# Tacha-S/perception

Hardware: AMD Instinct MI355X
Metric: candidate poses rendered+scored/sec @640x480 (higher is better)
Workload: dtype f32; 1 GPU; C2: 1 YCB mesh (12,288 tris), 10k 6-DoF poses/GPU render+score, 640x480, stride 8, no ICP; poses_per_gpu=10000, width=640, height=480, stride=8, parallelism=pose-shard x1, batches_in_flight=2, ranks=1, devices=1, exchange=none (one process)

## Files before the change

### include/pcore.h

```cpp
#ifndef PCORE_H_
#define PCORE_H_

#include <stdint.h>

#ifdef __cplusplus
extern "C" {
#endif

#define PCORE_ABI_VERSION 7

enum pcore_status {
    PCORE_OK = 0,
    PCORE_E_INVALID_ARG = 1,
    PCORE_E_HIP = 2,
    PCORE_E_OOM = 3,
    PCORE_E_STATE = 4
};

enum pcore_cost_type { PCORE_COST_DEPTH_3DOF = 0, PCORE_COST_RGBD_3DOF = 1, PCORE_COST_DEPTH_6DOF = 2 };

typedef struct pcore_ctx pcore_ctx;
typedef void* pcore_stream;

typedef struct pcore_camera {
    int32_t width, height;
    float fx, fy, cx, cy;
    float proj[16];
} pcore_camera;

typedef struct pcore_eval_params {
    int32_t cost_type;
    int32_t calc_obs_cost;
    int32_t stride;
    float depth_factor;
    float sensor_resolution;
    float occlusion_threshold;
    float color_distance_threshold;
} pcore_eval_params;

int pcore_create(int device, pcore_ctx** out_ctx);
void pcore_destroy(pcore_ctx* ctx);
const char* pcore_last_error(const pcore_ctx* ctx);
int pcore_abi_version(void);

uint64_t pcore_generation(const pcore_ctx* ctx);

int pcore_upload_meshes(pcore_ctx* ctx, const float* tri_xyz, const uint8_t* tri_rgb, int32_t num_tris,
                        const int32_t* tris_model_count, int32_t num_models);

int pcore_set_camera(pcore_ctx* ctx, const pcore_camera* cam);

int pcore_observed_cloud(pcore_ctx* ctx, const int32_t* d_depth, const uint8_t* d_label_mask, int32_t width,
                         int32_t height, int32_t stride, float depth_factor, float* d_out_xyz,
                         int32_t* d_out_label, int32_t cap, int32_t* out_count, pcore_stream stream);

int pcore_observed_cloud_bounded(pcore_ctx* ctx, const int32_t* d_depth, const uint8_t* d_rgb, int32_t width,
                                 int32_t height, int32_t stride, float depth_factor, const float* cam_to_world,
                                 const double* bounds, float* d_out_xyz, uint8_t* d_out_rgb, int32_t cap,
                                 int32_t* out_count, pcore_stream stream);

int pcore_set_observation(pcore_ctx* ctx, const int32_t* d_src_depth_cm, const uint8_t* d_src_mask,
                          const float* d_obs_xyz, const int32_t* d_obs_label, int32_t num_obs,
                          float sensor_resolution, pcore_stream stream);

int pcore_set_observation_colors(pcore_ctx* ctx, const uint8_t* d_obs_rgb, int32_t num_obs, pcore_stream stream);

int pcore_evaluate(pcore_ctx* ctx, const float* d_poses, const int32_t* d_pose_model,
                   const int32_t* d_pose_label, const float* d_pose_obs_total, int32_t num_poses,
                   const pcore_eval_params* params, float* d_out_rc, float* d_out_oc, float* d_out_diff,
                   int32_t* d_dbg_zs, pcore_stream stream);

#define PCORE_GICP_CYCLE_WINDOW 8
typedef struct pcore_icp_params {
    int32_t k_correspondences;
    int32_t max_iterations;
    double rotation_epsilon;
    double transformation_epsilon;
    int32_t cycle_exit_window;
} pcore_icp_params;

int pcore_evaluate_select(pcore_ctx* ctx, const float* d_poses, const int32_t* d_pose_model,
                          const int32_t* d_pose_label, const float* d_pose_obs_total, int32_t num_poses,
                          const pcore_eval_params* params, float* d_out_rc, float* d_out_oc, float* d_out_diff,
                          int64_t index_base, int32_t num_models, int64_t* d_keys, pcore_stream stream);

int pcore_evaluate_icp(pcore_ctx* ctx, const float* d_poses, const int32_t* d_pose_model,
                       const int32_t* d_pose_label, const float* d_pose_obs_total, int32_t num_poses,
                       const pcore_eval_params* params, const pcore_icp_params* icp, float* d_out_poses,
                       int32_t* d_out_iters, float* d_out_rc, float* d_out_oc, float* d_out_diff,
                       pcore_stream stream);

typedef struct pcore_planar_icp_params {
    int32_t max_iterations;
    float   max_correspondence;
    double  transformation_epsilon;
    double  fitness_epsilon;
} pcore_planar_icp_params;

int pcore_icp_planar(pcore_ctx* ctx, const float* d_poses, const int32_t* d_pose_model, int32_t num_poses,
                     const pcore_eval_params* params, const float* world_from_cam,
                     const pcore_planar_icp_params* icp, double* d_out_xform, int32_t* d_out_iters,
                     int32_t* d_out_status, double* d_out_mse, pcore_stream stream);

int pcore_debug_planar_step(const double* d_sums, double* d_out, int32_t n, pcore_stream stream);

typedef struct pcore_p2p_icp_params {
    int32_t max_iterations;
    float   relative_fitness;
    float   relative_rmse;
    float   max_dist_diff;
} pcore_p2p_icp_params;

int pcore_scene_projective(pcore_ctx* ctx, const int32_t* d_depth_cm, int32_t width, int32_t height, float fx, float fy,
                           float cx, float cy, float* d_out_pcd, float* d_out_normal, pcore_stream stream);

int pcore_icp_point2plane(pcore_ctx* ctx, const float* d_poses, const int32_t* d_pose_model,
                          const int32_t* d_pose_label, int32_t num_poses, const pcore_eval_params* params,
                          const pcore_p2p_icp_params* icp, float* d_out_T, float* d_out_fitness, float* d_out_rmse,
                          int32_t* d_out_iters, float* d_out_poses, pcore_stream stream);

int pcore_debug_p2p_clouds(const float* d_xyzw, const int32_t* d_seg_cnt, int32_t seg_stride, int32_t num_segs,
                           const float* d_scene_pcd4, const float* d_scene_normal4, int32_t width, int32_t height,
                           float fx, float fy, float cx, float cy, const pcore_p2p_icp_params* icp, float* d_out_T,
                           float* d_out_fitness, float* d_out_rmse, int32_t* d_out_iters, pcore_stream stream);

int pcore_render(pcore_ctx* ctx, const float* d_poses, const int32_t* d_pose_model, const int32_t* d_pose_label,
                 int32_t num_poses, float occlusion_threshold, int32_t* d_out_depth, uint8_t* d_out_color,
                 pcore_stream stream);

typedef struct pcore_gpu_stats {
    float icp_runtime;
    double peak_memory_usage;
    float gicp_ms;
    int32_t icp_chunks;
    int64_t gicp_iterations;
    int64_t gicp_iterations_run;
    int64_t gicp_cycle_exits;
} pcore_gpu_stats;
int pcore_get_stats(pcore_ctx* ctx, pcore_gpu_stats* out, int32_t reset);

#define PCORE_MAX_TILE_TIERS 8
typedef struct pcore_tile_info {
    int32_t num_tiers;
    int32_t tier;
    int32_t tcap;
    int32_t seq;
    int32_t edge[PCORE_MAX_TILE_TIERS];
    int32_t wgs_per_cu[PCORE_MAX_TILE_TIERS];
    int32_t hist[PCORE_MAX_TILE_TIERS + 1];
    int32_t chunked;
} pcore_tile_info;
int pcore_get_tile_info(pcore_ctx* ctx, pcore_tile_info* out);

int pcore_debug_lm_solve(const double* d_sys, const double* d_lambda, double* d_out, int32_t n, pcore_stream stream);

int pcore_debug_covariances(const float* d_xyzw, const int32_t* d_seg_off, const int32_t* d_seg_cnt, int32_t num_segs,
                            int32_t k, double* d_out_cov6, pcore_stream stream);
int pcore_debug_covariances_cloud(const float* d_xyzw, const int32_t* d_seg_cnt, int32_t seg_stride, int32_t num_segs,
                                  float fx, float fy, float cx, float cy, int32_t stride, double* d_out_cov6,
                                  pcore_stream stream);
int pcore_debug_gicp_help_stats(pcore_ctx* c, int64_t* out4);

int pcore_count_within(pcore_ctx* ctx, const float* d_queries, const int32_t* d_labels, const float* d_radius_sq,
                       int32_t n, int32_t* d_out_counts, pcore_stream stream);
int pcore_state_poses(pcore_ctx* ctx, const double* d_states, const int32_t* d_model, const double* cam_from_world,
                      const double* d_preprocess, int32_t num_models, int32_t n, float* d_out_poses,
                      pcore_stream stream);

int pcore_depth_to_cloud(pcore_ctx* ctx, const int32_t* d_depth, int32_t num_poses, int32_t width, int32_t height,
                         int32_t stride, float depth_factor, const uint8_t* d_label_mask,
                         const int32_t* d_pose_label, float* d_out_xyz, int32_t* d_out_pose, int32_t* d_out_label,
                         int32_t cap, int32_t* out_count, pcore_stream stream);

int pcore_depth_to_cloud_ex(pcore_ctx* ctx, const int32_t* d_depth, int32_t num_poses, int32_t width, int32_t height,
                            int32_t stride, float depth_factor, const uint8_t* d_label_mask, const int32_t* d_pose_label,
                            const uint8_t* d_color_planes, float* d_out_xyz, int32_t* d_out_pose, int32_t* d_out_label,
                            uint8_t* d_out_color, int32_t* d_out_dc_index, int32_t cap, int32_t* out_count,
                            pcore_stream stream);

#define PCORE_KEY_NONE ((int64_t)0x7fffffffffffffffLL)
int pcore_select(pcore_ctx* ctx, const float* d_rc, const float* d_oc, const int32_t* d_pose_model,
                 int32_t num_poses, int64_t index_base, int32_t num_models, int64_t* d_keys, pcore_stream stream);

int pcore_pose_distances(pcore_ctx* ctx, const float* d_pts, int32_t n, const double* d_T_gt, const double* d_T_est,
                         int32_t num_pairs, double* d_add, double* d_adds, pcore_stream stream);

#ifdef __cplusplus
}
#endif
#endif
```

### perception_amd/_native.py

```python
from __future__ import annotations

import ctypes
import os

import numpy as np

from . import build as _build

PCORE_OK = 0
PCORE_E_INVALID_ARG = 1
PCORE_E_HIP = 2
PCORE_E_OOM = 3
PCORE_E_STATE = 4
PCORE_KEY_NONE = 0x7FFFFFFFFFFFFFFF

COST_DEPTH_3DOF = 0
COST_RGBD_3DOF = 1
COST_DEPTH_6DOF = 2

EXPORTED_SYMBOLS = (
    "pcore_create", "pcore_destroy", "pcore_last_error", "pcore_abi_version", "pcore_upload_meshes",
    "pcore_set_camera", "pcore_observed_cloud", "pcore_set_observation", "pcore_evaluate", "pcore_evaluate_icp",
    "pcore_render",
    "pcore_depth_to_cloud", "pcore_select", "pcore_pose_distances",
    "pcore_observed_cloud_bounded", "pcore_set_observation_colors", "pcore_generation", "pcore_get_stats",
    "pcore_count_within", "pcore_state_poses", "pcore_evaluate_select", "pcore_get_tile_info", "pcore_debug_lm_solve",
    "pcore_debug_covariances", "pcore_debug_covariances_cloud", "pcore_debug_gicp_help_stats", "pcore_depth_to_cloud_ex",
    "pcore_icp_planar", "pcore_debug_planar_step",
    "pcore_scene_projective",
)
EXPORTED_SYMBOLS_WITH_DIGITS = ("pcore_icp_point2plane", "pcore_debug_p2p_clouds")


class PcoreError(RuntimeError):
    def __init__(self, code: int, msg: str):
        super().__init__(f"pcore error {code}: {msg}")
        self.code = code


class Camera(ctypes.Structure):
    _fields_ = [("width", ctypes.c_int32), ("height", ctypes.c_int32), ("fx", ctypes.c_float),
                ("fy", ctypes.c_float), ("cx", ctypes.c_float), ("cy", ctypes.c_float),
                ("proj", ctypes.c_float * 16)]


class EvalParams(ctypes.Structure):
    _fields_ = [("cost_type", ctypes.c_int32), ("calc_obs_cost", ctypes.c_int32), ("stride", ctypes.c_int32),
                ("depth_factor", ctypes.c_float), ("sensor_resolution", ctypes.c_float),
                ("occlusion_threshold", ctypes.c_float), ("color_distance_threshold", ctypes.c_float)]


class GpuStats(ctypes.Structure):
    _fields_ = [("icp_runtime", ctypes.c_float), ("peak_memory_usage", ctypes.c_double), ("gicp_ms", ctypes.c_float),
                ("icp_chunks", ctypes.c_int32), ("gicp_iterations", ctypes.c_int64),
                ("gicp_iterations_run", ctypes.c_int64), ("gicp_cycle_exits", ctypes.c_int64)]


MAX_TILE_TIERS = 8


class TileInfo(ctypes.Structure):
    _fields_ = [("num_tiers", ctypes.c_int32), ("tier", ctypes.c_int32), ("tcap", ctypes.c_int32),
                ("seq", ctypes.c_int32), ("edge", ctypes.c_int32 * MAX_TILE_TIERS),
                ("wgs_per_cu", ctypes.c_int32 * MAX_TILE_TIERS), ("hist", ctypes.c_int32 * (MAX_TILE_TIERS + 1)),
                ("chunked", ctypes.c_int32)]


class IcpParams(ctypes.Structure):
    _fields_ = [("k_correspondences", ctypes.c_int32), ("max_iterations", ctypes.c_int32),
                ("rotation_epsilon", ctypes.c_double), ("transformation_epsilon", ctypes.c_double),
                ("cycle_exit_window", ctypes.c_int32)]


class PlanarIcpParams(ctypes.Structure):
    _fields_ = [("max_iterations", ctypes.c_int32), ("max_correspondence", ctypes.c_float),
                ("transformation_epsilon", ctypes.c_double), ("fitness_epsilon", ctypes.c_double)]


class P2pIcpParams(ctypes.Structure):
    _fields_ = [("max_iterations", ctypes.c_int32), ("relative_fitness", ctypes.c_float),
                ("relative_rmse", ctypes.c_float), ("max_dist_diff", ctypes.c_float)]


P2P_MAX_ITER = 30
P2P_REL_FITNESS = 1e-5
P2P_REL_RMSE = 1e-5
P2P_MAX_DIST_DIFF = 0.1

PLANAR_MAX_ITER = 20
PLANAR_MAX_CORRESPONDENCE = 0.05
PLANAR_TRANS_EPS = 1e-8
PLANAR_FIT_EPS = 1e-5
PLANAR_ITERATION_CAP, PLANAR_TRANSFORM, PLANAR_ABS_MSE, PLANAR_REL_MSE, PLANAR_NO_CORRESPONDENCES, PLANAR_EMPTY_RENDER = \
    range(6)

ICP_K = 10
ICP_MAX_ITER = 150
ICP_ROT_EPS = float(np.float32(2e-3))
ICP_TRANS_EPS = float(np.float32(5e-4))
ICP_CYCLE_WINDOW = 8

_lib = None


def library_path() -> str:
    return _build.LIB


def load(auto_build: bool = True) -> ctypes.CDLL:
    global _lib
    if _lib is not None:
        return _lib
    override = os.environ.get("PCORE_LIB")
    if override:
        auto_build = False
    if auto_build:
        try:
            if _build.needs_build():
                _build.build()
        except (RuntimeError, OSError) as e:
            if not os.path.exists(_build.LIB):
                raise RuntimeError(f"libpcore.so is missing and cannot be built: {e}") from e
    path = override or _build.LIB
    if not os.path.exists(path):
        raise RuntimeError(f"libpcore.so not found at {path}; run `python -m perception_amd.build`")
    L = ctypes.CDLL(path)
    vp, i32, i64, f32 = ctypes.c_void_p, ctypes.c_int32, ctypes.c_int64, ctypes.c_float
    L.pcore_create.argtypes = [ctypes.c_int, ctypes.POINTER(vp)]
    L.pcore_destroy.argtypes = [vp]
    L.pcore_destroy.restype = None
    L.pcore_last_error.argtypes = [vp]
    L.pcore_last_error.restype = ctypes.c_char_p
    L.pcore_abi_version.argtypes = []
    L.pcore_upload_meshes.argtypes = [vp, vp, vp, i32, vp, i32]
    L.pcore_set_camera.argtypes = [vp, ctypes.POINTER(Camera)]
    L.pcore_observed_cloud.argtypes = [vp, vp, vp, i32, i32, i32, f32, vp, vp, i32, ctypes.POINTER(i32), vp]
    L.pcore_set_observation.argtypes = [vp, vp, vp, vp, vp, i32, f32, vp]
    L.pcore_evaluate.argtypes = [vp, vp, vp, vp, vp, i32, ctypes.POINTER(EvalParams), vp, vp, vp, vp, vp]
    L.pcore_evaluate_icp.argtypes = [vp, vp, vp, vp, vp, i32, ctypes.POINTER(EvalParams), ctypes.POINTER(IcpParams),
                                     vp, vp, vp, vp, vp, vp]
    L.pcore_render.argtypes = [vp, vp, vp, vp, i32, f32, vp, vp, vp]
    L.pcore_get_stats.argtypes = [vp, ctypes.POINTER(GpuStats), i32]
    if hasattr(L, "pcore_get_tile_info"):
        L.pcore_get_tile_info.argtypes = [vp, ctypes.POINTER(TileInfo)]
    if hasattr(L, "pcore_debug_lm_solve"):
        L.pcore_debug_lm_solve.argtypes = [vp, vp, vp, i32, vp]
    if hasattr(L, "pcore_debug_covariances"):
        L.pcore_debug_covariances.argtypes = [vp, vp, vp, i32, i32, vp, vp]
    if hasattr(L, "pcore_debug_gicp_help_stats"):
        L.pcore_debug_gicp_help_stats.argtypes = [vp, vp]
    if hasattr(L, "pcore_debug_covariances_cloud"):
        f32 = ctypes.c_float
        L.pcore_debug_covariances_cloud.argtypes = [vp, vp, i32, i32, f32, f32, f32, f32, i32, vp, vp]
    if hasattr(L, "pcore_depth_to_cloud_ex"):
        L.pcore_depth_to_cloud_ex.argtypes = [vp, vp, i32, i32, i32, i32, f32, vp, vp, vp, vp, vp, vp, vp, vp, i32,
                                              ctypes.POINTER(i32), vp]
    L.pcore_depth_to_cloud.argtypes = [vp, vp, i32, i32, i32, i32, f32, vp, vp, vp, vp, vp, i32,
                                       ctypes.POINTER(i32), vp]
    if hasattr(L, "pcore_icp_planar"):
        L.pcore_icp_planar.argtypes = [vp, vp, vp, i32, ctypes.POINTER(EvalParams), ctypes.POINTER(ctypes.c_float),
                                       ctypes.POINTER(PlanarIcpParams), vp, vp, vp, vp, vp]
    if hasattr(L, "pcore_debug_planar_step"):
        L.pcore_debug_planar_step.argtypes = [vp, vp, i32, vp]
    if hasattr(L, "pcore_icp_point2plane"):
        L.pcore_scene_projective.argtypes = [vp, vp, i32, i32, f32, f32, f32, f32, vp, vp, vp]
        L.pcore_icp_point2plane.argtypes = [vp, vp, vp, vp, i32, ctypes.POINTER(EvalParams),
                                            ctypes.POINTER(P2pIcpParams), vp, vp, vp, vp, vp, vp]
        L.pcore_debug_p2p_clouds.argtypes = [vp, vp, i32, i32, vp, vp, i32, i32, f32, f32, f32, f32,
                                             ctypes.POINTER(P2pIcpParams), vp, vp, vp, vp, vp]
    L.pcore_select.argtypes = [vp, vp, vp, vp, i32, i64, i32, vp, vp]
    L.pcore_pose_distances.argtypes = [vp, vp, i32, vp, vp, i32, vp, vp, vp]
    L.pcore_set_observation_colors.argtypes = [vp, vp, i32, vp]
    L.pcore_observed_cloud_bounded.argtypes = [vp, vp, vp, i32, i32, i32, f32, vp, vp, vp, vp, i32,
                                               ctypes.POINTER(i32), vp]
    L.pcore_generation.argtypes = [vp]
    L.pcore_evaluate_select.argtypes = [vp, vp, vp, vp, vp, i32, ctypes.POINTER(EvalParams), vp, vp, vp, i64, i32,
                                        vp, vp]
    L.pcore_count_within.argtypes = [vp, vp, vp, vp, i32, vp, vp]
    L.pcore_state_poses.argtypes = [vp, vp, vp, ctypes.POINTER(ctypes.c_double), vp, i32, i32, vp, vp]
    for name in EXPORTED_SYMBOLS + EXPORTED_SYMBOLS_WITH_DIGITS:
        if name not in ("pcore_destroy", "pcore_last_error", "pcore_generation") and hasattr(L, name):
            getattr(L, name).restype = ctypes.c_int
    L.pcore_generation.restype = ctypes.c_uint64
    _lib = L
    return L
```

### perception_amd/build.py

```python
from __future__ import annotations

import os
import shutil
import subprocess
import sys

HERE = os.path.dirname(os.path.abspath(__file__))
CSRC = os.path.join(HERE, "csrc")
LIB = os.path.join(HERE, "libpcore.so")
SOURCES = ["pcore_kernels.hip", "pcore_gicp.hip", "pcore_metrics.hip", "pcore_states.hip", "pcore_icp2d.hip", "pcore_p2p.hip",
           "pcore_api.hip"]
HEADERS = ["pcore_internal.h", "pcore_cov.h", "pcore_gicp_math.h", "pcore_icp2d_math.h", "pcore_p2p_math.h", "pcore_dmath.h", "pcore_colour.h", "pcore_fdiv.h", "pcore_streams.h", os.path.join("..", "..", "include", "pcore.h")]
ARCH = os.environ.get("PCORE_OFFLOAD_ARCH", "gfx950")


def hipcc() -> str:
    for cand in (os.environ.get("HIPCC"), shutil.which("hipcc"), "/opt/rocm/bin/hipcc"):
        if cand and os.path.exists(cand):
            return cand
    raise RuntimeError("hipcc not found: cannot build libpcore.so")


def flags() -> list:
    return [f"--offload-arch={ARCH}", "-O2", "-std=c++17", "-fPIC", "-shared", "-ffp-contract=off",
            "-fno-fast-math", "-fno-slp-vectorize", "-Wall", "-Wno-unused-function"]


def kernel_source_digest() -> str:
    import hashlib

    h = hashlib.sha256(" ".join(flags()).encode())
    for f in ("pcore_kernels.hip", "pcore_internal.h", "pcore_cov.h", "pcore_colour.h", "pcore_fdiv.h", "pcore_streams.h"):
        with open(os.path.join(CSRC, f), "rb") as fh:
            h.update(fh.read())
    return h.hexdigest()[:16]


def gicp_source_digest() -> str:
    import hashlib

    h = hashlib.sha256(" ".join(flags()).encode())
    for f in ("pcore_gicp.hip", "pcore_cov.h", "pcore_gicp_math.h", "pcore_icp2d_math.h", "pcore_dmath.h", "pcore_internal.h"):
        with open(os.path.join(CSRC, f), "rb") as fh:
            h.update(fh.read())
    return h.hexdigest()[:16]


def needs_build() -> bool:
    if not os.path.exists(LIB):
        return True
    t = os.path.getmtime(LIB)
    deps = [os.path.join(CSRC, f) for f in SOURCES + HEADERS] + [os.path.abspath(__file__)]
    return any(os.path.getmtime(d) > t for d in deps if os.path.exists(d))


def build(force: bool = False, verbose: bool = False) -> str:
    if not force and not needs_build():
        return LIB
    cmd = [hipcc()] + flags() + [os.path.join(CSRC, f) for f in SOURCES] + ["-o", LIB + ".tmp"]
    if verbose:
        print(" ".join(cmd), file=sys.stderr)
    subprocess.run(cmd, check=True, cwd=CSRC)
    os.replace(LIB + ".tmp", LIB)
    return LIB


def build_checkers(verbose: bool = False) -> list:
    root = os.path.dirname(HERE)
    out_dir = os.path.join(root, "tools", "bin")
    os.makedirs(out_dir, exist_ok=True)
    built = []
    for name in ("fdiv_check",):
        src = os.path.join(root, "tools", name + ".hip")
        out = os.path.join(out_dir, name)
        cmd = [hipcc(), f"--offload-arch={ARCH}", "-O3", "-std=c++17", "-ffp-contract=off", "-fno-fast-math", src,
               "-o", out]
        if verbose:
            print(" ".join(cmd), file=sys.stderr)
        subprocess.run(cmd, check=True, cwd=root)
        built.append(out)
    return built


if __name__ == "__main__":
    print(build(force="--force" in sys.argv, verbose=True))
```

### perception_amd/core.py

```python
from __future__ import annotations

import ctypes
from typing import Optional, Sequence, Tuple

import numpy as np
import torch

from . import _native
from ._native import Camera, EvalParams, IcpParams, P2pIcpParams, PcoreError, PlanarIcpParams


def _ptr(t: Optional[torch.Tensor], dtype: torch.dtype, name: str):
    if t is None:
        return None
    if not isinstance(t, torch.Tensor) or not t.is_cuda:
        raise TypeError(f"{name}: expected a GPU torch tensor")
    if t.dtype != dtype:
        raise TypeError(f"{name}: expected {dtype}, got {t.dtype}")
    if not t.is_contiguous():
        raise ValueError(f"{name}: tensor must be contiguous")
    return ctypes.c_void_p(t.data_ptr())


def _stream(stream: Optional[torch.cuda.Stream]):
    s = stream if stream is not None else torch.cuda.current_stream()
    return ctypes.c_void_p(s.cuda_stream)


class PoseCore:

    def __init__(self, device: int = 0):
        self.lib = _native.load()
        self.device = int(device)
        h = ctypes.c_void_p()
        rc = self.lib.pcore_create(self.device, ctypes.byref(h))
        if rc != _native.PCORE_OK:
            raise PcoreError(rc, f"pcore_create(device={device}) failed")
        self._h = h
        self.width = self.height = 0
        self.num_models = 0

    def close(self):
        if getattr(self, "_h", None) is not None and self._h.value:
            self.lib.pcore_destroy(self._h)
            self._h = None

    def __del__(self):
        try:
            self.close()
        except Exception:
            pass

    def _check(self, rc: int):
        if rc != _native.PCORE_OK:
            msg = self.lib.pcore_last_error(self._h)
            raise PcoreError(rc, msg.decode() if msg else "")

    def upload_meshes(self, tris: np.ndarray, tris_model_count, colors: Optional[np.ndarray] = None):
        tris = np.ascontiguousarray(tris, dtype=np.float32).reshape(-1, 9)
        cnt = np.ascontiguousarray(tris_model_count, dtype=np.int32)
        col = None if colors is None else np.ascontiguousarray(colors, dtype=np.uint8).reshape(-1, 3)
        self._check(self.lib.pcore_upload_meshes(
            self._h, tris.ctypes.data_as(ctypes.c_void_p),
            None if col is None else col.ctypes.data_as(ctypes.c_void_p), tris.shape[0],
            cnt.ctypes.data_as(ctypes.c_void_p), cnt.shape[0]))
        self.num_models = int(cnt.shape[0])

    def set_camera(self, width: int, height: int, fx: float, fy: float, cx: float, cy: float, proj: np.ndarray):
        cam = Camera()
        cam.width, cam.height = int(width), int(height)
        cam.fx, cam.fy, cam.cx, cam.cy = float(fx), float(fy), float(cx), float(cy)
        pj = np.asarray(proj, dtype=np.float32).reshape(16)
        for i in range(16):
            cam.proj[i] = float(pj[i])
        self._check(self.lib.pcore_set_camera(self._h, ctypes.byref(cam)))
        self.width, self.height = int(width), int(height)

    def observed_cloud(self, depth: torch.Tensor, label_mask: Optional[torch.Tensor], stride: int,
                       depth_factor: float, stream=None) -> Tuple[torch.Tensor, torch.Tensor]:
        h, w = depth.shape[-2:]
        cap = ((w + stride - 1) // stride) * ((h + stride - 1) // stride)
        xyz = torch.empty((max(cap, 1), 3), dtype=torch.float32, device=depth.device)
        lab = torch.empty((max(cap, 1),), dtype=torch.int32, device=depth.device)
        cnt = ctypes.c_int32(0)
        self._check(self.lib.pcore_observed_cloud(
            self._h, _ptr(depth, torch.int32, "depth"), _ptr(label_mask, torch.uint8, "label_mask"), w, h, stride,
            float(depth_factor), _ptr(xyz, torch.float32, "xyz"), _ptr(lab, torch.int32, "label"), cap,
            ctypes.byref(cnt), _stream(stream)))
        n = cnt.value
        return xyz[:n], lab[:n]

    def observed_cloud_bounded(self, depth: torch.Tensor, stride: int, depth_factor: float,
                               cam_to_world: Optional[np.ndarray] = None, bounds: Optional[Sequence[float]] = None,
                               rgb: Optional[torch.Tensor] = None, stream=None
                               ) -> Tuple[torch.Tensor, Optional[torch.Tensor]]:
        h, w = depth.shape[-2:]
        cap = ((w + stride - 1) // stride) * ((h + stride - 1) // stride)
        xyz = torch.empty((max(cap, 1), 3), dtype=torch.float32, device=depth.device)
        out_rgb = torch.empty((max(cap, 1), 3), dtype=torch.uint8, device=depth.device) if rgb is not None else None
        M = None if cam_to_world is None else (ctypes.c_float * 16)(*np.asarray(cam_to_world, np.float32).reshape(16))
        B = None if bounds is None else (ctypes.c_double * 6)(*np.asarray(bounds, np.float64).reshape(6))
        cnt = ctypes.c_int32(0)
        self._check(self.lib.pcore_observed_cloud_bounded(
            self._h, _ptr(depth, torch.int32, "depth"), _ptr(None if rgb is None else rgb.contiguous(), torch.uint8, "rgb"),
            w, h, stride, float(depth_factor), M, B, _ptr(xyz, torch.float32, "xyz"),
            _ptr(out_rgb, torch.uint8, "out_rgb"), cap, ctypes.byref(cnt), _stream(stream)))
        n = cnt.value
        return xyz[:n], (out_rgb[:n] if out_rgb is not None else None)

    def set_observation(self, src_depth_cm: torch.Tensor, src_mask: Optional[torch.Tensor],
                        obs_xyz: torch.Tensor, obs_label: Optional[torch.Tensor], sensor_resolution: float,
                        stream=None):
        obs_xyz = obs_xyz.contiguous()
        n = int(obs_xyz.shape[0])
        self._check(self.lib.pcore_set_observation(
            self._h, _ptr(src_depth_cm.contiguous(), torch.int32, "src_depth"),
            _ptr(None if src_mask is None else src_mask.contiguous(), torch.uint8, "src_mask"),
            _ptr(obs_xyz, torch.float32, "obs_xyz") if n else None,
            _ptr(None if obs_label is None else obs_label.contiguous(), torch.int32, "obs_label") if n else None,
            n, float(sensor_resolution), _stream(stream)))

    def set_observation_colors(self, obs_rgb: torch.Tensor, stream=None):
        rgb = obs_rgb.contiguous()
        n = int(rgb.shape[0])
        self._check(self.lib.pcore_set_observation_colors(
            self._h, _ptr(rgb, torch.uint8, "obs_rgb") if n else None, n, _stream(stream)))

    def evaluate(self, poses: torch.Tensor, pose_model: torch.Tensor, pose_label: Optional[torch.Tensor],
                 pose_obs_total: Optional[torch.Tensor], cost_type: int = _native.COST_DEPTH_6DOF,
                 calc_obs_cost: bool = True, stride: int = 8, depth_factor: float = 100.0,
                 sensor_resolution: float = 0.01, occlusion_threshold: float = 1.0,
                 out: Optional[Tuple[torch.Tensor, torch.Tensor, torch.Tensor]] = None,
                 dbg_zs: Optional[torch.Tensor] = None, color_distance_threshold: float = 15.0, stream=None,
                 select: Optional[Tuple[torch.Tensor, int, int]] = None):
        n = int(poses.shape[0])
        dev = poses.device
        if out is None:
            out = tuple(torch.empty(n, dtype=torch.float32, device=dev) for _ in range(3))
        rc, oc, df = out
        p = EvalParams(int(cost_type), int(bool(calc_obs_cost)), int(stride), float(depth_factor),
                       float(sensor_resolution), float(occlusion_threshold), float(color_distance_threshold))
        if select is not None:
            keys, index_base, num_models = select
            if dbg_zs is not None:
                raise ValueError("evaluate: dbg_zs and select are exclusive")
            self._check(self.lib.pcore_evaluate_select(
                self._h, _ptr(poses, torch.float32, "poses"), _ptr(pose_model, torch.int32, "pose_model"),
                _ptr(pose_label, torch.int32, "pose_label"), _ptr(pose_obs_total, torch.float32, "pose_obs_total"),
                n, ctypes.byref(p), _ptr(rc, torch.float32, "rc"), _ptr(oc, torch.float32, "oc"),
                _ptr(df, torch.float32, "diff"), int(index_base), int(num_models), _ptr(keys, torch.int64, "keys"),
                _stream(stream)))
            return rc, oc, df
        self._check(self.lib.pcore_evaluate(
            self._h, _ptr(poses, torch.float32, "poses"), _ptr(pose_model, torch.int32, "pose_model"),
            _ptr(pose_label, torch.int32, "pose_label"), _ptr(pose_obs_total, torch.float32, "pose_obs_total"),
            n, ctypes.byref(p), _ptr(rc, torch.float32, "rc"), _ptr(oc, torch.float32, "oc"),
            _ptr(df, torch.float32, "diff"), _ptr(dbg_zs, torch.int32, "dbg_zs"), _stream(stream)))
        return rc, oc, df

    def capture_evaluate(self, poses: torch.Tensor, pose_model: torch.Tensor, pose_label: Optional[torch.Tensor],
                         pose_obs_total: Optional[torch.Tensor], **kw):
        n = int(poses.shape[0])
        out = tuple(torch.empty(n, dtype=torch.float32, device=poses.device) for _ in range(3))
        self.evaluate(poses, pose_model, pose_label, pose_obs_total, out=out, **kw)
        torch.cuda.synchronize()
        graph = torch.cuda.CUDAGraph()
        with torch.cuda.graph(graph):
            self.evaluate(poses, pose_model, pose_label, pose_obs_total, out=out, **kw)
        gen = self.generation()

        def replay():
            if self.generation() != gen:
                raise PcoreError(_native.PCORE_E_STATE, "captured evaluate graph is stale: the context changed "
                                 "(setup call, new stride or scratch reallocation) since the capture")
            graph.replay()

        return replay, out

    def generation(self) -> int:
        return int(self.lib.pcore_generation(self._h))

    def evaluate_icp(self, poses: torch.Tensor, pose_model: torch.Tensor, pose_label: Optional[torch.Tensor],
                     pose_obs_total: Optional[torch.Tensor], cost_type: int = _native.COST_DEPTH_6DOF,
                     calc_obs_cost: bool = True, stride: int = 8, depth_factor: float = 100.0,
                     sensor_resolution: float = 0.01, occlusion_threshold: float = 1.0,
                     k: int = _native.ICP_K, max_iterations: int = _native.ICP_MAX_ITER,
                     rotation_epsilon: float = _native.ICP_ROT_EPS,
                     transformation_epsilon: float = _native.ICP_TRANS_EPS, out=None,
                     color_distance_threshold: float = 15.0, stream=None,
                     cycle_exit_window: int = _native.ICP_CYCLE_WINDOW):
        n = int(poses.shape[0])
        dev = poses.device
        if out is None:
            out = (torch.empty((n, 16), dtype=torch.float32, device=dev), torch.empty(n, dtype=torch.int32, device=dev),
                   *(torch.empty(n, dtype=torch.float32, device=dev) for _ in range(3)))
        adj, iters, rc, oc, df = out
        p = EvalParams(int(cost_type), int(bool(calc_obs_cost)), int(stride), float(depth_factor),
                       float(sensor_resolution), float(occlusion_threshold), float(color_distance_threshold))
        ip = IcpParams(int(k), int(max_iterations), float(rotation_epsilon), float(transformation_epsilon),
                       int(cycle_exit_window))
        self._check(self.lib.pcore_evaluate_icp(
            self._h, _ptr(poses, torch.float32, "poses"), _ptr(pose_model, torch.int32, "pose_model"),
            _ptr(pose_label, torch.int32, "pose_label"), _ptr(pose_obs_total, torch.float32, "pose_obs_total"),
            n, ctypes.byref(p), ctypes.byref(ip), _ptr(adj, torch.float32, "adjusted_poses"),
            _ptr(iters, torch.int32, "iterations"), _ptr(rc, torch.float32, "rc"), _ptr(oc, torch.float32, "oc"),
            _ptr(df, torch.float32, "diff"), _stream(stream)))
        return adj, iters, rc, oc, df

    def icp_planar(self, poses: torch.Tensor, pose_model: torch.Tensor, world_from_cam: np.ndarray,
                   cost_type: int = _native.COST_DEPTH_3DOF, stride: int = 4, depth_factor: float = 100.0,
                   occlusion_threshold: float = 1.0, max_iterations: int = _native.PLANAR_MAX_ITER,
                   max_correspondence: float = _native.PLANAR_MAX_CORRESPONDENCE,
                   transformation_epsilon: float = _native.PLANAR_TRANS_EPS,
                   fitness_epsilon: float = _native.PLANAR_FIT_EPS, out=None, stream=None):
        n = int(poses.shape[0])
        dev = poses.device
        if out is None:
            out = (torch.empty((n, 4), dtype=torch.float64, device=dev), torch.empty(n, dtype=torch.int32, device=dev),
                   torch.empty(n, dtype=torch.int32, device=dev), torch.empty(n, dtype=torch.float64, device=dev))
        xform, iters, status, mse = out
        p = EvalParams(int(cost_type), 0, int(stride), float(depth_factor), 0.0, float(occlusion_threshold), 0.0)
        pp = PlanarIcpParams(int(max_iterations), float(max_correspondence), float(transformation_epsilon),
                             float(fitness_epsilon))
        M = (ctypes.c_float * 16)(*np.asarray(world_from_cam, np.float32).reshape(16))
        self._check(self.lib.pcore_icp_planar(
            self._h, _ptr(poses, torch.float32, "poses"), _ptr(pose_model, torch.int32, "pose_model"), n,
            ctypes.byref(p), M, ctypes.byref(pp), _ptr(xform, torch.float64, "xform"),
            _ptr(iters, torch.int32, "iterations"), _ptr(status, torch.int32, "status"),
            _ptr(mse, torch.float64, "mse"), _stream(stream)))
        return xform, iters, status, mse

    def planar_step(self, sums: torch.Tensor, stream=None) -> torch.Tensor:
        sums = sums.contiguous()
        n = int(sums.shape[0])
        out = torch.empty((n, 4), dtype=torch.float64, device=sums.device)
        rc = self.lib.pcore_debug_planar_step(_ptr(sums, torch.float64, "sums"), _ptr(out, torch.float64, "out"), n,
                                              _stream(stream))
        if rc != _native.PCORE_OK:
            raise PcoreError(rc, "pcore_debug_planar_step failed")
        return out

    def scene_projective(self, depth_cm: torch.Tensor, fx: float, fy: float, cx: float, cy: float, stream=None
                         ) -> Tuple[torch.Tensor, torch.Tensor]:
        h, w = depth_cm.shape[-2:]
        pcd = torch.empty((h, w, 3), dtype=torch.float32, device=depth_cm.device)
        nrm = torch.empty((h, w, 3), dtype=torch.float32, device=depth_cm.device)
        self._check(self.lib.pcore_scene_projective(
            self._h, _ptr(depth_cm, torch.int32, "depth_cm"), int(w), int(h), float(fx), float(fy), float(cx),
            float(cy), _ptr(pcd, torch.float32, "pcd"), _ptr(nrm, torch.float32, "normal"), _stream(stream)))
        return pcd, nrm

    def icp_point2plane(self, poses: torch.Tensor, pose_model: torch.Tensor, pose_label: Optional[torch.Tensor] = None,
                        cost_type: int = _native.COST_DEPTH_6DOF, stride: int = 8, depth_factor: float = 100.0,
                        occlusion_threshold: float = 1.0, max_iterations: int = _native.P2P_MAX_ITER,
                        relative_fitness: float = _native.P2P_REL_FITNESS,
                        relative_rmse: float = _native.P2P_REL_RMSE, max_dist_diff: float = _native.P2P_MAX_DIST_DIFF,
                        out=None, out_poses: Optional[torch.Tensor] = None, stream=None):
        n = int(poses.shape[0])
        dev = poses.device
        if out is None:
            out = (torch.empty((n, 16), dtype=torch.float32, device=dev), torch.empty(n, dtype=torch.float32, device=dev),
                   torch.empty(n, dtype=torch.float32, device=dev), torch.empty(n, dtype=torch.int32, device=dev))
        T, fitness, rmse, iters = out
        p = EvalParams(int(cost_type), 0, int(stride), float(depth_factor), 0.0, float(occlusion_threshold), 0.0)
        ip = P2pIcpParams(int(max_iterations), float(relative_fitness), float(relative_rmse), float(max_dist_diff))
        self._check(self.lib.pcore_icp_point2plane(
            self._h, _ptr(poses, torch.float32, "poses"), _ptr(pose_model, torch.int32, "pose_model"),
            _ptr(pose_label, torch.int32, "pose_label"), n, ctypes.byref(p), ctypes.byref(ip),
            _ptr(T, torch.float32, "T"), _ptr(fitness, torch.float32, "fitness"), _ptr(rmse, torch.float32, "rmse"),
            _ptr(iters, torch.int32, "iterations"), _ptr(out_poses, torch.float32, "out_poses"), _stream(stream)))
        return T, fitness, rmse, iters

    def p2p_clouds(self, xyzw: torch.Tensor, seg_cnt: torch.Tensor, scene_pcd4: torch.Tensor,
                   scene_normal4: torch.Tensor, fx: float, fy: float, cx: float, cy: float,
                   max_iterations: int = _native.P2P_MAX_ITER, relative_fitness: float = _native.P2P_REL_FITNESS,
                   relative_rmse: float = _native.P2P_REL_RMSE, max_dist_diff: float = _native.P2P_MAX_DIST_DIFF,
                   stream=None):
        s, cap = int(xyzw.shape[0]), int(xyzw.shape[1])
        h, w = int(scene_pcd4.shape[0]), int(scene_pcd4.shape[1])
        dev = xyzw.device
        T = torch.empty((s, 16), dtype=torch.float32, device=dev)
        fitness = torch.empty(s, dtype=torch.float32, device=dev)
        rmse = torch.empty(s, dtype=torch.float32, device=dev)
        iters = torch.empty(s, dtype=torch.int32, device=dev)
        ip = P2pIcpParams(int(max_iterations), float(relative_fitness), float(relative_rmse), float(max_dist_diff))
        rc = self.lib.pcore_debug_p2p_clouds(
            _ptr(xyzw, torch.float32, "xyzw"), _ptr(seg_cnt, torch.int32, "seg_cnt"), cap, s,
            _ptr(scene_pcd4, torch.float32, "scene_pcd4"), _ptr(scene_normal4, torch.float32, "scene_normal4"), w, h,
            float(fx), float(fy), float(cx), float(cy), ctypes.byref(ip), _ptr(T, torch.float32, "T"),
            _ptr(fitness, torch.float32, "fitness"), _ptr(rmse, torch.float32, "rmse"),
            _ptr(iters, torch.int32, "iterations"), _stream(stream))
        if rc != _native.PCORE_OK:
            raise PcoreError(rc, "pcore_debug_p2p_clouds failed")
        return T, fitness, rmse, iters

    def evaluate_p2p(self, poses: torch.Tensor, pose_model: torch.Tensor, pose_label: Optional[torch.Tensor],
                     pose_obs_total: Optional[torch.Tensor], cost_type: int = _native.COST_DEPTH_6DOF,
                     calc_obs_cost: bool = True, stride: int = 8, depth_factor: float = 100.0,
                     sensor_resolution: float = 0.01, occlusion_threshold: float = 1.0,
                     max_iterations: int = _native.P2P_MAX_ITER, relative_fitness: float = _native.P2P_REL_FITNESS,
                     relative_rmse: float = _native.P2P_REL_RMSE, max_dist_diff: float = _native.P2P_MAX_DIST_DIFF,
                     color_distance_threshold: float = 15.0, stream=None):
        n = int(poses.shape[0])
        adj = torch.empty((n, 16), dtype=torch.float32, device=poses.device)
        label = pose_label if cost_type == _native.COST_DEPTH_6DOF else None
        _, fitness, rmse, iters = self.icp_point2plane(
            poses, pose_model, label, cost_type=cost_type, stride=stride, depth_factor=depth_factor,
            occlusion_threshold=occlusion_threshold, max_iterations=max_iterations,
            relative_fitness=relative_fitness, relative_rmse=relative_rmse, max_dist_diff=max_dist_diff,
            out_poses=adj, stream=stream)
        rc, oc, df = self.evaluate(adj, pose_model, pose_label, pose_obs_total, cost_type=cost_type,
                                   calc_obs_cost=calc_obs_cost, stride=stride, depth_factor=depth_factor,
                                   sensor_resolution=sensor_resolution, occlusion_threshold=occlusion_threshold,
                                   color_distance_threshold=color_distance_threshold, stream=stream)
        return adj, iters, rc, oc, df, fitness, rmse

    def render(self, poses: torch.Tensor, pose_model: torch.Tensor, pose_label: Optional[torch.Tensor],
               occlusion_threshold: float = 1.0, out: Optional[torch.Tensor] = None, color: bool = False,
               out_color: Optional[torch.Tensor] = None, stream=None):
        n = int(poses.shape[0])
        if out is None:
            out = torch.empty((n, self.height, self.width), dtype=torch.int32, device=poses.device)
        if color and out_color is None:
            out_color = torch.empty((3, n, self.height, self.width), dtype=torch.uint8, device=poses.device)
        self._check(self.lib.pcore_render(
            self._h, _ptr(poses, torch.float32, "poses"), _ptr(pose_model, torch.int32, "pose_model"),
            _ptr(pose_label, torch.int32, "pose_label"), n, float(occlusion_threshold),
            _ptr(out, torch.int32, "out"), _ptr(out_color, torch.uint8, "out_color") if color else None,
            _stream(stream)))
        return (out, out_color) if color else out

    def stats(self, reset: bool = False) -> dict:
        st = _native.GpuStats()
        self._check(self.lib.pcore_get_stats(self._h, ctypes.byref(st), int(bool(reset))))
        return {"icp_runtime": st.icp_runtime, "peak_memory_usage": st.peak_memory_usage, "gicp_ms": st.gicp_ms,
                "icp_chunks": st.icp_chunks, "gicp_iterations": st.gicp_iterations,
                "gicp_iterations_run": st.gicp_iterations_run, "gicp_cycle_exits": st.gicp_cycle_exits}

    def gicp_help_stats(self) -> dict:
        out = (ctypes.c_int64 * 4)()
        self._check(self.lib.pcore_debug_gicp_help_stats(self._h, out))
        return {"helper_rounds": int(out[0]), "owner_timeouts": int(out[1]), "helper_giveups": int(out[2]),
                "poses_enlisted": int(out[3])}

    def tile_info(self) -> dict:
        ti = _native.TileInfo()
        self._check(self.lib.pcore_get_tile_info(self._h, ctypes.byref(ti)))
        n = ti.num_tiers
        return {"tier": ti.tier, "tcap": ti.tcap, "seq": ti.seq, "edge": list(ti.edge[:n]),
                "wgs_per_cu": list(ti.wgs_per_cu[:n]), "hist": list(ti.hist[:n + 1]), "chunked": ti.chunked}

    def depth_to_cloud(self, depth: torch.Tensor, stride: int, depth_factor: float,
                       label_mask: Optional[torch.Tensor] = None, pose_label: Optional[torch.Tensor] = None,
                       stream=None, color_planes: Optional[torch.Tensor] = None, dc_index: bool = False):
        if depth.dim() == 2:
            depth = depth.unsqueeze(0)
        n, h, w = depth.shape
        cap = n * ((w + stride - 1) // stride) * ((h + stride - 1) // stride)
        dev = depth.device
        xyz = torch.empty((max(cap, 1), 3), dtype=torch.float32, device=dev)
        pose = torch.empty((max(cap, 1),), dtype=torch.int32, device=dev)
        lab = torch.empty((max(cap, 1),), dtype=torch.int32, device=dev)
        cnt = ctypes.c_int32(0)
        extra = color_planes is not None or dc_index
        if not extra:
            self._check(self.lib.pcore_depth_to_cloud(
                self._h, _ptr(depth.contiguous(), torch.int32, "depth"), n, w, h, stride, float(depth_factor),
                _ptr(label_mask, torch.uint8, "label_mask"), _ptr(pose_label, torch.int32, "pose_label"),
                _ptr(xyz, torch.float32, "xyz"), _ptr(pose, torch.int32, "pose"), _ptr(lab, torch.int32, "label"),
                cap, ctypes.byref(cnt), _stream(stream)))
            k = cnt.value
            return xyz[:k], pose[:k], lab[:k]
        planes = None
        col = None
        if color_planes is not None:
            planes = color_planes.contiguous()
            if tuple(planes.shape) != (3, n, h, w):
                raise ValueError(f"color_planes must be (3, {n}, {h}, {w}), got {tuple(planes.shape)}")
            col = torch.empty((3, max(cap, 1)), dtype=torch.uint8, device=dev)
        dc = torch.empty((n, h, w), dtype=torch.int32, device=dev) if dc_index else None
        self._check(self.lib.pcore_depth_to_cloud_ex(
            self._h, _ptr(depth.contiguous(), torch.int32, "depth"), n, w, h, stride, float(depth_factor),
            _ptr(label_mask, torch.uint8, "label_mask"), _ptr(pose_label, torch.int32, "pose_label"),
            _ptr(planes, torch.uint8, "color_planes"), _ptr(xyz, torch.float32, "xyz"), _ptr(pose, torch.int32, "pose"),
            _ptr(lab, torch.int32, "label"), _ptr(col, torch.uint8, "color"), _ptr(dc, torch.int32, "dc_index"),
            max(cap, 1) if col is not None else cap, ctypes.byref(cnt), _stream(stream)))
        k = cnt.value
        out = [xyz[:k], pose[:k], lab[:k]]
        if col is not None:
            out.append(col[:, :k])
        if dc is not None:
            out.append(dc)
        return tuple(out)

    def select(self, rc: torch.Tensor, oc: torch.Tensor, pose_model: torch.Tensor, num_models: int,
               index_base: int = 0, keys: Optional[torch.Tensor] = None, stream=None) -> torch.Tensor:
        if keys is None:
            keys = torch.full((num_models,), _native.PCORE_KEY_NONE, dtype=torch.int64, device=rc.device)
        self._check(self.lib.pcore_select(
            self._h, _ptr(rc, torch.float32, "rc"), _ptr(oc, torch.float32, "oc"),
            _ptr(pose_model, torch.int32, "pose_model"), int(rc.shape[0]), int(index_base), int(num_models),
            _ptr(keys, torch.int64, "keys"), _stream(stream)))
        return keys

    def count_within(self, queries: torch.Tensor, labels: torch.Tensor, radius_sq: torch.Tensor,
                     out: Optional[torch.Tensor] = None, stream=None) -> torch.Tensor:
        n = int(queries.shape[0])
        if out is None:
            out = torch.empty(n, dtype=torch.int32, device=queries.device)
        self._check(self.lib.pcore_count_within(
            self._h, _ptr(queries.contiguous(), torch.float32, "queries"), _ptr(labels.contiguous(), torch.int32, "labels"),
            _ptr(radius_sq.contiguous(), torch.float32, "radius_sq"), n, _ptr(out, torch.int32, "counts"),
            _stream(stream)))
        return out

    def state_poses(self, states: torch.Tensor, model: torch.Tensor, cam_from_world, preprocess: torch.Tensor,
                    out: Optional[torch.Tensor] = None, stream=None) -> torch.Tensor:
        n = int(states.shape[0])
        if out is None:
            out = torch.empty((n, 16), dtype=torch.float32, device=states.device)
        cam = (ctypes.c_double * 16)(*[float(v) for v in np.asarray(cam_from_world, np.float64).reshape(16)])
        k = int(preprocess.shape[0])
        self._check(self.lib.pcore_state_poses(
            self._h, _ptr(states.contiguous(), torch.float64, "states"), _ptr(model.contiguous(), torch.int32, "model"),
            cam, _ptr(preprocess.contiguous(), torch.float64, "preprocess"), k, n, _ptr(out, torch.float32, "poses"),
            _stream(stream)))
        return out


class PoseLanes:

    def __init__(self, device: int = 0, lanes: int = 2):
        if lanes < 1:
            raise ValueError("lanes must be >= 1")
        self.cores = [PoseCore(device) for _ in range(lanes)]
        dev = torch.device("cuda", int(device))
        self.streams = [torch.cuda.Stream(device=dev) for _ in range(lanes)]

    def __len__(self):
        return len(self.cores)

    def __getitem__(self, i: int) -> Tuple[PoseCore, torch.cuda.Stream]:
        return self.cores[i], self.streams[i]

    def upload_meshes(self, *a, **kw):
        for c in self.cores:
            c.upload_meshes(*a, **kw)

    def set_camera(self, *a, **kw):
        for c in self.cores:
            c.set_camera(*a, **kw)

    def set_observation(self, *a, **kw):
        for c in self.cores:
            c.set_observation(*a, **kw)

    def set_observation_colors(self, *a, **kw):
        for c in self.cores:
            c.set_observation_colors(*a, **kw)

    @classmethod
    def replicate(cls, core: "PoseCore", scene_setup, lanes: int = 2) -> "PoseLanes":
        if lanes < 1:
            raise ValueError("lanes must be >= 1")
        self = cls.__new__(cls)
        self.cores = [core] + [PoseCore(core.device) for _ in range(lanes - 1)]
        dev = torch.device("cuda", core.device)
        self.streams = [torch.cuda.Stream(device=dev) for _ in range(lanes)]
        for c in self.cores[1:]:
            scene_setup(c)
        return self


def decode_keys(keys) -> Tuple[np.ndarray, np.ndarray]:
    k = np.asarray(keys.cpu() if isinstance(keys, torch.Tensor) else keys, dtype=np.int64)
    none = k == _native.PCORE_KEY_NONE
    hi = (k >> 31).astype(np.uint64).astype(np.uint32)
    cost = (hi ^ np.uint32(0x80000000)).view(np.int32).astype(np.int32)
    idx = (k & 0x7FFFFFFF).astype(np.int64)
    cost = np.where(none, np.int32(2**31 - 1), cost)
    idx = np.where(none, -1, idx)
    return cost, idx


def encode_key(cost: int, index: int) -> int:
    if cost == 2**31 - 1 and index < 0:
        return _native.PCORE_KEY_NONE
    hi = (int(cost) & 0xFFFFFFFF) ^ 0x80000000
    return (hi << 31) | (int(index) & 0x7FFFFFFF)
```

### perception_amd/csrc/pcore_api.hip

```cpp
#include "../../include/pcore.h"
#include "pcore_internal.h"
#include "pcore_streams.h"
#include "pcore_gicp_math.h"
#include "pcore_icp2d_math.h"
#include "pcore_p2p_math.h"

#include <algorithm>
#include <climits>
#include <cmath>
#include <cstdio>
#include <cstdlib>
#include <cstring>
#include <string>
#include <unordered_map>
#include <vector>

using namespace pcore;

namespace {

template <typename T>
struct DevBuf {
    T* p = nullptr;
    size_t n = 0;
// ... 1051 lines not shown
            HIPC(c, hipMemcpyAsync(c->icp_iter_stats_host, c->icp_iter_stats.p, 8 * sizeof(unsigned long long),
                                   hipMemcpyDeviceToHost, s));
        if (ev) {
            HIPC(c, hipEventRecord(ev[2], s));
            c->icp_ev_used++;
        }
    }
    return pcore_evaluate(c, d_out_poses, d_pose_model, d_pose_label, d_pose_obs_total, num_poses, p, d_out_rc,
                          d_out_oc, d_out_diff, nullptr, stream);
}

int pcore_icp_planar(pcore_ctx* c, const float* d_poses, const int32_t* d_pose_model, int32_t num_poses,
                     const pcore_eval_params* p, const float* world_from_cam, const pcore_planar_icp_params* pp,
                     double* d_out_xform, int32_t* d_out_iters, int32_t* d_out_status, double* d_out_mse,
                     pcore_stream stream) {
    if (!c) return PCORE_E_INVALID_ARG;
    if (!p || !pp || !world_from_cam) return fail(c, PCORE_E_INVALID_ARG, "icp_planar: null parameters");
    if (!c->have_mesh || !c->have_cam || !c->have_obs)
        return fail(c, PCORE_E_STATE, "icp_planar: meshes, camera and observation must be set first");
    if (p->cost_type != PCORE_COST_DEPTH_3DOF && p->cost_type != PCORE_COST_RGBD_3DOF)
        return fail(c, PCORE_E_INVALID_ARG, "icp_planar: cost_type must be a 3-DoF one (0 or 1)");
    if (pp->max_iterations < 0) return fail(c, PCORE_E_INVALID_ARG, "icp_planar: max_iterations must be >= 0");
    if (!std::isfinite(pp->max_correspondence) || pp->max_correspondence < 0.0f)
        return fail(c, PCORE_E_INVALID_ARG, "icp_planar: max_correspondence must be finite and >= 0");
    if (std::isnan(pp->transformation_epsilon) || std::isnan(pp->fitness_epsilon))
        return fail(c, PCORE_E_INVALID_ARG, "icp_planar: NaN epsilon");
    for (int i = 0; i < 16; i++)
        if (!std::isfinite(world_from_cam[i])) return fail(c, PCORE_E_INVALID_ARG, "icp_planar: non-finite world_from_cam");
    if (num_poses < 0 || (num_poses > 0 && (!d_poses || !d_pose_model || !d_out_xform || !d_out_iters || !d_out_status)))
        return fail(c, PCORE_E_INVALID_ARG, "icp_planar: null pose / output pointer");
    const int W = c->cam.width, H = c->cam.height;
    if (p->stride <= 0 || W % p->stride != 0)
        return fail(c, PCORE_E_INVALID_ARG, "icp_planar: width must be a multiple of stride");
    const int ws = W / p->stride, hs = (H + p->stride - 1) / p->stride;
    if (ws > 4095 || hs > 4095) return fail(c, PCORE_E_INVALID_ARG, "icp_planar: sampled image too large");
    if (fused_lds_bytes(ws * hs, c->bitmap_words, false) > (size_t)c->prop.sharedMemPerBlock)
        return fail(c, PCORE_E_INVALID_ARG, "icp_planar: sampled z-buffer does not fit in LDS (use a larger stride)");
    if (num_poses == 0) return PCORE_OK;
    HIPC(c, hipSetDevice(c->device));
    hipStream_t s = (hipStream_t)stream;
    const int nsamp = ws * hs;
    const size_t per_pose = (size_t)nsamp * sizeof(float4) + sizeof(int32_t);
    size_t budget = (size_t)32 << 30;
    {
        size_t free_b = 0, total_b = 0;
        if (hipMemGetInfo(&free_b, &total_b) == hipSuccess && free_b > 0)
            budget = std::min(budget, std::max<size_t>((size_t)1 << 30, free_b / 5 * 2));
    }
    if (const char* e = getenv("PCORE_ICP2D_SCRATCH_BYTES")) budget = (size_t)std::max(1LL, atoll(e));
    const int max_chunk = (int)std::min<size_t>(std::max<size_t>(1, budget / per_pose), 0x7fffffff);
    const int nchunks = (num_poses + max_chunk - 1) / max_chunk;
    const int chunk = (num_poses + nchunks - 1) / nchunks;
    const bool grid_stale = c->planar_obs_serial != c->obs_serial ||
                            std::memcmp(c->planar_m, world_from_cam, sizeof(c->planar_m)) != 0 ||
                            std::memcmp(&c->planar_radius, &pp->max_correspondence, sizeof(float)) != 0;
    const bool setup = grid_stale || c->sampled_stride != p->stride || !c->icp_cloud.p || !c->icp_count.p ||
                       c->icp_cloud.n < (size_t)chunk * nsamp || c->icp_count.n < (size_t)chunk;
    hipStreamCaptureStatus cap_status = hipStreamCaptureStatusNone;
    if (hipStreamIsCapturing(s, &cap_status) != hipSuccess) {
        (void)hipGetLastError();
        cap_status = hipStreamCaptureStatusActive;
    }
    if (setup && cap_status != hipStreamCaptureStatusNone)
        return fail(c, PCORE_E_STATE, "icp_planar: the world-frame grid or the scratch would have to be built while the "
                                      "stream captures; run the call once before the capture");
    if (grid_stale) {
        const int n = (int)(c->obs_xyz_h.size() / 3);
        std::vector<float4> wp((size_t)n);
        for (int i = 0; i < n; i++) {
            float4 q;
            icp2d::to_world(world_from_cam, c->obs_xyz_h[3 * (size_t)i], c->obs_xyz_h[3 * (size_t)i + 1],
                            c->obs_xyz_h[3 * (size_t)i + 2], q.x, q.y, q.z);
            std::memcpy(&q.w, &i, 4);
            wp[i] = q;
        }
        std::vector<int32_t> cell_start;
        std::vector<float4> gpts;
        LabelGrid g;
        build_grid(wp, pp->max_correspondence, g, cell_start, gpts);
        if (gpts.empty()) gpts.push_back(make_float4(0.0f, 0.0f, 0.0f, 0.0f));
        HIPC(c, hipStreamSynchronize(s));
        c->planar_obs_serial = 0;
        c->generation++;
        HIPC(c, dev_upload(c->planar_cell_start, cell_start));
        HIPC(c, dev_upload(c->planar_pts, gpts));
        c->planar_grid = g;
        std::memcpy(c->planar_m, world_from_cam, sizeof(c->planar_m));
        c->planar_radius = pp->max_correspondence;
        c->planar_obs_serial = c->obs_serial;
    }
    int rc = ensure_sampled(c, p->stride, s);
    if (rc != PCORE_OK) return rc;
    HIPC(c, reserve_gen(c, c->icp_cloud, (size_t)chunk * nsamp));
    HIPC(c, reserve_gen(c, c->icp_count, (size_t)chunk));
    FusedArgs a{};
    fill_fused_args(c, p, a);
    PlanarArgs g{};
    g.src = c->icp_cloud.p;
    g.src_count = c->icp_count.p;
    g.src_cap = nsamp;
    for (int i = 0; i < 12; i++) g.m[i] = world_from_cam[i];
    g.grid = c->planar_grid;
    g.cell_start = c->planar_cell_start.p;
    g.grid_pts = c->planar_pts.p;
    g.r = pp->max_correspondence;
    g.r2 = pp->max_correspondence * pp->max_correspondence;
    g.max_iter = pp->max_iterations;
    g.eps_t = pp->transformation_epsilon;
    g.eps_fit = pp->fitness_epsilon;
    g.out_xform = d_out_xform;
    g.out_iters = d_out_iters;
    g.out_status = d_out_status;
    g.out_mse = d_out_mse;
    for (int base = 0; base < num_poses; base += chunk) {
        const int n = std::min(chunk, num_poses - base);
        a.poses = d_poses + (size_t)16 * base;
        a.pose_model = d_pose_model + base;
        a.pose_label = nullptr;
        a.num_poses = n;
        a.cloud_out = c->icp_cloud.p;
        a.cloud_count = c->icp_count.p;
        a.cloud_cap = nsamp;
        a.tcap = fused_tier_samples(0, a.ws, a.hs, 0, false, c->dinfo);
        if (const char* e = getenv("PCORE_FUSED_TCAP")) a.tcap = std::min(std::max(atoi(e), 1), a.ws * a.hs);
        if (a.tcap <= 0) a.tcap = a.ws * a.hs;
        HIPC(c, launch_render_cloud(a, s));
        g.pose_base = base;
        HIPC(c, launch_planar_icp(g, n, s));
    }
    return PCORE_OK;
}

int pcore_debug_planar_step(const double* d_sums, double* d_out, int32_t n, pcore_stream stream) {
    if (n < 0 || (n > 0 && (!d_sums || !d_out))) return PCORE_E_INVALID_ARG;
    return launch_planar_step_test(d_sums, d_out, n, (hipStream_t)stream) == hipSuccess ? PCORE_OK : PCORE_E_HIP;
}

int pcore_scene_projective(pcore_ctx* c, const int32_t* d_depth_cm, int32_t width, int32_t height, float fx, float fy,
                           float cx, float cy, float* d_out_pcd, float* d_out_normal, pcore_stream stream) {
    if (!c) return PCORE_E_INVALID_ARG;
    if (width <= 0 || height <= 0 || width > 16384 || height > 16384)
        return fail(c, PCORE_E_INVALID_ARG, "scene_projective: bad image size");
    if (!d_depth_cm || !d_out_pcd || !d_out_normal)
        return fail(c, PCORE_E_INVALID_ARG, "scene_projective: null pointer");
    HIPC(c, hipSetDevice(c->device));
    HIPC(c, launch_p2p_scene(d_depth_cm, width, height, fx, fy, cx, cy, nullptr, nullptr, d_out_pcd, d_out_normal,
                             (hipStream_t)stream));
    return PCORE_OK;
}

namespace {

const char* p2p_params_error(const pcore_p2p_icp_params* ip) {
    if (ip->max_iterations < 0) return "max_iterations must be >= 0";
    if (std::isnan(ip->relative_fitness) || ip->relative_fitness < 0.0f) return "relative_fitness must be >= 0";
    if (std::isnan(ip->relative_rmse) || ip->relative_rmse < 0.0f) return "relative_rmse must be >= 0";
    if (std::isnan(ip->max_dist_diff) || ip->max_dist_diff < 0.0f) return "max_dist_diff must be >= 0";
    return nullptr;
}

}

int pcore_icp_point2plane(pcore_ctx* c, const float* d_poses, const int32_t* d_pose_model, const int32_t* d_pose_label,
                          int32_t num_poses, const pcore_eval_params* p, const pcore_p2p_icp_params* ip,
                          float* d_out_T, float* d_out_fitness, float* d_out_rmse, int32_t* d_out_iters,
                          float* d_out_poses, pcore_stream stream) {
    if (!c) return PCORE_E_INVALID_ARG;
    if (!p || !ip) return fail(c, PCORE_E_INVALID_ARG, "icp_point2plane: null parameters");
    if (!c->have_mesh || !c->have_cam || !c->have_obs)
        return fail(c, PCORE_E_STATE, "icp_point2plane: meshes, camera and observation must be set first");
    if (p->cost_type != PCORE_COST_DEPTH_3DOF && p->cost_type != PCORE_COST_DEPTH_6DOF &&
        p->cost_type != PCORE_COST_RGBD_3DOF)
        return fail(c, PCORE_E_INVALID_ARG, "icp_point2plane: unknown cost_type");
    if (const char* e = p2p_params_error(ip)) return fail(c, PCORE_E_INVALID_ARG, std::string("icp_point2plane: ") + e);
    if (num_poses < 0 || (num_poses > 0 && (!d_poses || !d_pose_model || !d_out_T || !d_out_fitness || !d_out_rmse ||
                                            !d_out_iters)))
        return fail(c, PCORE_E_INVALID_ARG, "icp_point2plane: null pose / output pointer");
    if (d_pose_label && !c->obs_has_mask)
        return fail(c, PCORE_E_INVALID_ARG, "icp_point2plane: pose labels need a source mask");
    const int W = c->cam.width, H = c->cam.height;
    if (p->stride <= 0 || W % p->stride != 0)
        return fail(c, PCORE_E_INVALID_ARG, "icp_point2plane: width must be a multiple of stride");
    const int ws = W / p->stride, hs = (H + p->stride - 1) / p->stride;
    if (ws > 4095 || hs > 4095) return fail(c, PCORE_E_INVALID_ARG, "icp_point2plane: sampled image too large");
    if (fused_lds_bytes(ws * hs, c->bitmap_words, false) > (size_t)c->prop.sharedMemPerBlock)
        return fail(c, PCORE_E_INVALID_ARG,
                    "icp_point2plane: sampled z-buffer does not fit in LDS (use a larger stride)");
    if (num_poses == 0) return PCORE_OK;
    HIPC(c, hipSetDevice(c->device));
    hipStream_t s = (hipStream_t)stream;
    const int nsamp = ws * hs;
    const size_t per_pose = (size_t)nsamp * sizeof(float4) + sizeof(int32_t);
    size_t budget = (size_t)32 << 30;
    {
        size_t free_b = 0, total_b = 0;
        if (hipMemGetInfo(&free_b, &total_b) == hipSuccess && free_b > 0)
            budget = std::min(budget, std::max<size_t>((size_t)1 << 30, free_b / 5 * 2));
    }
    if (const char* e = getenv("PCORE_P2P_SCRATCH_BYTES")) budget = (size_t)std::max(1LL, atoll(e));
    const int max_chunk = (int)std::min<size_t>(std::max<size_t>(1, budget / per_pose), 0x7fffffff);
    const int nchunks = (num_poses + max_chunk - 1) / max_chunk;
    const int chunk = (num_poses + nchunks - 1) / nchunks;
    const pcore_camera& cam = c->cam;
    const bool scene_stale = c->p2p_obs_serial != c->obs_serial || c->p2p_cam.width != W || c->p2p_cam.height != H ||
                             std::memcmp(&c->p2p_cam.fx, &cam.fx, sizeof(float)) != 0 ||
                             std::memcmp(&c->p2p_cam.fy, &cam.fy, sizeof(float)) != 0 ||
                             std::memcmp(&c->p2p_cam.cx, &cam.cx, sizeof(float)) != 0 ||
                             std::memcmp(&c->p2p_cam.cy, &cam.cy, sizeof(float)) != 0;
    const bool setup = scene_stale || c->sampled_stride != p->stride || !c->icp_cloud.p || !c->icp_count.p ||
                       c->icp_cloud.n < (size_t)chunk * nsamp || c->icp_count.n < (size_t)chunk;
    hipStreamCaptureStatus cap_status = hipStreamCaptureStatusNone;
    if (hipStreamIsCapturing(s, &cap_status) != hipSuccess) {
        (void)hipGetLastError();
        cap_status = hipStreamCaptureStatusActive;
    }
    if (setup && cap_status != hipStreamCaptureStatusNone)
        return fail(c, PCORE_E_STATE, "icp_point2plane: the scene or the scratch would have to be built while the "
                                      "stream captures; run the call once before the capture");
    if (scene_stale) {
        const size_t npx = (size_t)W * H;
        HIPC(c, hipStreamSynchronize(s));
        c->p2p_obs_serial = 0;
        c->generation++;
        HIPC(c, dev_reserve(c->p2p_pcd, npx));
        HIPC(c, dev_reserve(c->p2p_normal, npx));
        HIPC(c, launch_p2p_scene(c->src_depth.p, W, H, cam.fx, cam.fy, cam.cx, cam.cy, c->p2p_pcd.p, c->p2p_normal.p,
                                 nullptr, nullptr, s));
        c->p2p_cam = cam;
        c->p2p_obs_serial = c->obs_serial;
    }
    int rc = ensure_sampled(c, p->stride, s);
    if (rc != PCORE_OK) return rc;
    HIPC(c, reserve_gen(c, c->icp_cloud, (size_t)chunk * nsamp));
    HIPC(c, reserve_gen(c, c->icp_count, (size_t)chunk));
    FusedArgs a{};
    fill_fused_args(c, p, a);
    P2pArgs g{};
    g.src = c->icp_cloud.p;
    g.src_count = c->icp_count.p;
    g.src_cap = nsamp;
    g.scene_pcd = c->p2p_pcd.p;
    g.scene_normal = c->p2p_normal.p;
    g.width = W;
    g.height = H;
    g.fx = cam.fx; g.fy = cam.fy; g.cx = cam.cx; g.cy = cam.cy;
    g.max_dist_diff = ip->max_dist_diff;
    g.rel_fitness = ip->relative_fitness;
    g.rel_rmse = ip->relative_rmse;
    g.max_iter = ip->max_iterations;
    g.poses_in = d_poses;
    g.poses_out = d_out_poses;
    g.out_T = d_out_T;
    g.out_fitness = d_out_fitness;
    g.out_rmse = d_out_rmse;
    g.out_iters = d_out_iters;
    for (int base = 0; base < num_poses; base += chunk) {
        const int n = std::min(chunk, num_poses - base);
        a.poses = d_poses + (size_t)16 * base;
        a.pose_model = d_pose_model + base;
        a.pose_label = d_pose_label ? d_pose_label + base : nullptr;
        a.num_poses = n;
        a.cloud_out = c->icp_cloud.p;
        a.cloud_count = c->icp_count.p;
        a.cloud_cap = nsamp;
        a.tcap = fused_tier_samples(0, a.ws, a.hs, 0, false, c->dinfo);
        if (const char* e = getenv("PCORE_FUSED_TCAP")) a.tcap = std::min(std::max(atoi(e), 1), a.ws * a.hs);
        if (a.tcap <= 0) a.tcap = a.ws * a.hs;
        HIPC(c, launch_render_cloud(a, s));
        g.pose_base = base;
        HIPC(c, launch_p2p_icp(g, n, s));
    }
    return PCORE_OK;
}

int pcore_debug_p2p_clouds(const float* d_xyzw, const int32_t* d_seg_cnt, int32_t seg_stride, int32_t num_segs,
                           const float* d_scene_pcd4, const float* d_scene_normal4, int32_t width, int32_t height,
                           float fx, float fy, float cx, float cy, const pcore_p2p_icp_params* ip, float* d_out_T,
                           float* d_out_fitness, float* d_out_rmse, int32_t* d_out_iters, pcore_stream stream) {
    if (!ip || p2p_params_error(ip) || num_segs < 0 || seg_stride < 0 || width <= 0 || height <= 0 || width > 16384 ||
        height > 16384 || !d_scene_pcd4 || !d_scene_normal4)
        return PCORE_E_INVALID_ARG;
    if (num_segs > 0 && (!d_xyzw || !d_seg_cnt || !d_out_T || !d_out_fitness || !d_out_rmse || !d_out_iters))
        return PCORE_E_INVALID_ARG;
    P2pArgs g{};
    g.src = (float4*)d_xyzw;
    g.src_count = d_seg_cnt;
    g.src_cap = seg_stride;
    g.scene_pcd = (const float4*)d_scene_pcd4;
    g.scene_normal = (const float4*)d_scene_normal4;
    g.width = width;
    g.height = height;
    g.fx = fx; g.fy = fy; g.cx = cx; g.cy = cy;
    g.max_dist_diff = ip->max_dist_diff;
    g.rel_fitness = ip->relative_fitness;
    g.rel_rmse = ip->relative_rmse;
    g.max_iter = ip->max_iterations;
    g.out_T = d_out_T;
    g.out_fitness = d_out_fitness;
    g.out_rmse = d_out_rmse;
    g.out_iters = d_out_iters;
    return launch_p2p_icp(g, num_segs, (hipStream_t)stream) == hipSuccess ? PCORE_OK : PCORE_E_HIP;
}

int pcore_render(pcore_ctx* c, const float* d_poses, const int32_t* d_pose_model, const int32_t* d_pose_label,
                 int32_t num_poses, float occlusion_threshold, int32_t* d_out_depth, uint8_t* d_out_color,
                 pcore_stream stream) {
    if (!c) return PCORE_E_INVALID_ARG;
    if (!c->have_mesh || !c->have_cam || !c->have_obs)
        return fail(c, PCORE_E_STATE, "render: meshes, camera and observation must be set first");
    if (num_poses < 0 || (num_poses > 0 && (!d_poses || !d_pose_model || !d_out_depth)))
        return fail(c, PCORE_E_INVALID_ARG, "render: null pointer");
    if (d_pose_label && !c->obs_has_mask)
        return fail(c, PCORE_E_INVALID_ARG, "render: pose labels need a source mask");
    if (num_poses == 0) return PCORE_OK;
    HIPC(c, hipSetDevice(c->device));
    hipStream_t s = (hipStream_t)stream;
    const int W = c->cam.width, H = c->cam.height;
    HIPC(c, launch_fill_i32(d_out_depth, INT_MAX, (size_t)num_poses * W * H, s));
    HIPC(c, launch_render_full(c->tris.p, c->num_tris, c->tri_lo.p, c->tri_hi.p, d_poses, d_pose_model, num_poses, W,
                               H, c->proj.p, d_out_depth, s));
    int32_t* tri_min = nullptr;
    if (d_out_color) {
        const size_t npx = (size_t)num_poses * W * H;
        HIPC(c, dev_reserve(c->render_tri, npx));
        tri_min = c->render_tri.p;
        HIPC(c, launch_fill_i32(tri_min, INT_MAX, npx, s));
        HIPC(c, launch_render_full_tri(c->tris.p, c->num_tris, c->tri_lo.p, c->tri_hi.p, d_poses, d_pose_model,
                                       num_poses, W, H, c->proj.p, d_out_depth, tri_min, s));
    }
    HIPC(c, launch_render_finalize(d_out_depth, c->src_depth.p, c->src_mask.p, d_pose_label, num_poses, W, H,
                                   occlusion_threshold, s, tri_min, d_out_color ? c->tri_rgb.p : nullptr, d_out_color));
    return PCORE_OK;
}

int pcore_get_stats(pcore_ctx* c, pcore_gpu_stats* out, int32_t reset) {
    if (!c || !out) return PCORE_E_INVALID_ARG;
    HIPC(c, hipSetDevice(c->device));
    double icp_ms = 0.0, gicp_ms = 0.0;
    for (int i = 0; i < c->icp_ev_used; i++) {
        hipEvent_t* ev = c->icp_ev.data() + 3 * i;
        HIPC(c, hipEventSynchronize(ev[2]));
        float a = 0.0f, b = 0.0f;
        HIPC(c, hipEventElapsedTime(&a, ev[0], ev[2]));
        HIPC(c, hipEventElapsedTime(&b, ev[1], ev[2]));
        icp_ms += a;
        gicp_ms += b;
    }
    out->icp_runtime = (float)(icp_ms * 1e-3);
    out->peak_memory_usage = c->peak_mem_mb;
    out->gicp_ms = (float)gicp_ms;
    out->icp_chunks = c->icp_ev_used;
    unsigned long long it[4] = {0ull, 0ull, 0ull, 0ull};
    if (c->icp_ev_used > 0 && c->icp_iter_stats_host)
        for (int i = 0; i < 4; i++) it[i] = c->icp_iter_stats_host[i];
    if (it[3] != 0)
        return fail(c, PCORE_E_HIP, "evaluate_icp: " + std::to_string(it[3]) +
                                        " poses needed the grid search in the GICP instance without it");
    out->gicp_iterations = (int64_t)it[0];
    out->gicp_iterations_run = (int64_t)it[1];
    out->gicp_cycle_exits = (int64_t)it[2];
    if (reset) c->peak_mem_mb = 0.0;
    return PCORE_OK;
}

int pcore_debug_gicp_help_stats(pcore_ctx* c, int64_t* out4) {
    if (!c || !out4) return PCORE_E_INVALID_ARG;
    HIPC(c, hipSetDevice(c->device));
    for (int i = 0; i < 4; i++) out4[i] = 0;
    if (c->icp_ev_used <= 0 || !c->icp_iter_stats_host) return PCORE_OK;
    HIPC(c, hipEventSynchronize(c->icp_ev[3 * (c->icp_ev_used - 1) + 2]));
    for (int i = 0; i < 4; i++) out4[i] = (int64_t)c->icp_iter_stats_host[4 + i];
    return PCORE_OK;
}

int pcore_get_tile_info(pcore_ctx* c, pcore_tile_info* out) {
    if (!c || !out) return PCORE_E_INVALID_ARG;
    static_assert(kTileTiers <= PCORE_MAX_TILE_TIERS, "pcore_tile_info holds the tiers");
    std::memset(out, 0, sizeof(*out));
    out->num_tiers = kTileTiers;
    out->tier = c->tile_tier;
    out->tcap = c->tile_tcap;
    out->seq = -1;
    for (int t = 0; t < kTileTiers; t++) {
        out->edge[t] = c->tile_edge[t];
        out->wgs_per_cu[t] = tier_wgs(t);
    }
    if (c->fb_host) {
        const volatile int32_t* fb = c->fb_host;
        for (int b = 0; b <= kTileTiers; b++) out->hist[b] = fb[b];
        out->chunked = fb[kTileTiers + 1];
        out->seq = fb[kTileTiers + 2];
    }
    return PCORE_OK;
}

int pcore_debug_lm_solve(const double* d_sys, const double* d_lambda, double* d_out, int32_t n, pcore_stream stream) {
    if (n < 0 || (n > 0 && (!d_sys || !d_lambda || !d_out))) return PCORE_E_INVALID_ARG;
    return launch_lm_solve_test(d_sys, d_lambda, d_out, n, (hipStream_t)stream) == hipSuccess ? PCORE_OK : PCORE_E_HIP;
}

int pcore_debug_covariances(const float* d_xyzw, const int32_t* d_seg_off, const int32_t* d_seg_cnt, int32_t num_segs,
                            int32_t k, double* d_out_cov6, pcore_stream stream) {
    if (num_segs < 0 || k <= 0 || k > 16 || (num_segs > 0 && (!d_xyzw || !d_seg_off || !d_seg_cnt || !d_out_cov6)))
        return PCORE_E_INVALID_ARG;
    return launch_covariances(reinterpret_cast<const float4*>(d_xyzw), d_seg_off, d_seg_cnt, 0, num_segs, k, d_out_cov6,
                              (hipStream_t)stream, INT_MAX) == hipSuccess ? PCORE_OK : PCORE_E_HIP;
}

int pcore_debug_covariances_cloud(const float* d_xyzw, const int32_t* d_seg_cnt, int32_t seg_stride, int32_t num_segs,
                                  float fx, float fy, float cx, float cy, int32_t stride, double* d_out_cov6,
                                  pcore_stream stream) {
    if (num_segs < 0 || seg_stride < 0 || stride <= 0 || (num_segs > 0 && (!d_xyzw || !d_seg_cnt || !d_out_cov6)))
        return PCORE_E_INVALID_ARG;
    return launch_covariances_cloud(reinterpret_cast<const float4*>(d_xyzw), d_seg_cnt, seg_stride, num_segs, fx, fy, cx,
                                    cy, stride, d_out_cov6, (hipStream_t)stream) == hipSuccess ? PCORE_OK : PCORE_E_HIP;
}

int pcore_depth_to_cloud(pcore_ctx* c, const int32_t* d_depth, int32_t num_poses, int32_t width, int32_t height,
                         int32_t stride, float depth_factor, const uint8_t* d_label_mask, const int32_t* d_pose_label,
                         float* d_out_xyz, int32_t* d_out_pose, int32_t* d_out_label, int32_t cap, int32_t* out_count,
                         pcore_stream stream) {
    return pcore_depth_to_cloud_ex(c, d_depth, num_poses, width, height, stride, depth_factor, d_label_mask,
                                   d_pose_label, nullptr, d_out_xyz, d_out_pose, d_out_label, nullptr, nullptr, cap,
                                   out_count, stream);
}

int pcore_depth_to_cloud_ex(pcore_ctx* c, const int32_t* d_depth, int32_t num_poses, int32_t width, int32_t height,
                            int32_t stride, float depth_factor, const uint8_t* d_label_mask, const int32_t* d_pose_label,
                            const uint8_t* d_color_planes, float* d_out_xyz, int32_t* d_out_pose, int32_t* d_out_label,
                            uint8_t* d_out_color, int32_t* d_out_dc_index, int32_t cap, int32_t* out_count,
                            pcore_stream stream) {
    if (!c) return PCORE_E_INVALID_ARG;
    if (!c->have_cam) return fail(c, PCORE_E_STATE, "depth_to_cloud: camera not set");
    if (num_poses < 0 || width <= 0 || height <= 0 || stride <= 0 || !d_depth || cap < 0 ||
        (cap > 0 && !d_out_xyz) || !out_count || (d_out_color && !d_color_planes))
        return fail(c, PCORE_E_INVALID_ARG, "depth_to_cloud: bad arguments");
    if (width % stride != 0) return fail(c, PCORE_E_INVALID_ARG, "depth_to_cloud: width % stride != 0");
    if (d_label_mask && num_poses != 1)
        return fail(c, PCORE_E_INVALID_ARG, "depth_to_cloud: label mask needs num_poses == 1");
    *out_count = 0;
    if (num_poses == 0) return PCORE_OK;
    HIPC(c, hipSetDevice(c->device));
    hipStream_t s = (hipStream_t)stream;
    HIPC(c, dev_reserve(c->scratch_counts, num_poses));
    HIPC(c, dev_reserve(c->scratch_offsets, num_poses));
    HIPC(c, dev_reserve(c->scratch_total, 1));
    const CloudBounds no_bounds{};
    HIPC(c, launch_cloud_count(d_depth, num_poses, width, height, stride, d_label_mask, no_bounds,
                               c->scratch_counts.p, s));
    HIPC(c, launch_exclusive_scan(c->scratch_counts.p, c->scratch_offsets.p, num_poses, c->scratch_total.p, s));
    HIPC(c, launch_cloud_write(d_depth, num_poses, width, height, stride, c->cam.cx, c->cam.cy, c->cam.fx, c->cam.fy,
                               depth_factor, d_label_mask, d_pose_label, c->scratch_offsets.p, d_out_xyz, d_out_pose,
                               d_out_label, cap, no_bounds, nullptr, nullptr, s, d_out_color ? d_color_planes : nullptr,
                               d_out_color));
    if (d_out_dc_index) {
        const size_t samples = (size_t)((width + stride - 1) / stride) * ((height + stride - 1) / stride);
        HIPC(c, dev_reserve(c->scratch_dc_pre, (size_t)num_poses * (samples + 1)));
        HIPC(c, launch_cloud_dc_index(d_depth, num_poses, width, height, stride, d_label_mask, c->scratch_offsets.p,
                                      c->scratch_dc_pre.p, d_out_dc_index, s));
    }
    int32_t total = 0;
    HIPC(c, hipMemcpyAsync(&total, c->scratch_total.p, 4, hipMemcpyDeviceToHost, s));
    HIPC(c, hipStreamSynchronize(s));
    *out_count = total;
    return PCORE_OK;
}

int pcore_select(pcore_ctx* c, const float* d_rc, const float* d_oc, const int32_t* d_pose_model, int32_t num_poses,
                 int64_t index_base, int32_t num_models, int64_t* d_keys, pcore_stream stream) {
    if (!c) return PCORE_E_INVALID_ARG;
    if (num_poses < 0 || num_models <= 0 || index_base < 0 || index_base + num_poses > 0x7fffffffLL ||
        (num_poses > 0 && (!d_rc || !d_oc || !d_pose_model || !d_keys)))
        return fail(c, PCORE_E_INVALID_ARG, "select: bad arguments");
    if (num_poses == 0) return PCORE_OK;
    HIPC(c, hipSetDevice(c->device));
    HIPC(c, launch_select(d_rc, d_oc, d_pose_model, num_poses, index_base, num_models, d_keys, (hipStream_t)stream));
    return PCORE_OK;
}

int pcore_count_within(pcore_ctx* c, const float* d_queries, const int32_t* d_labels, const float* d_radius_sq,
                       int32_t n, int32_t* d_out_counts, pcore_stream stream) {
    if (!c) return PCORE_E_INVALID_ARG;
    if (n < 0 || (n > 0 && (!d_queries || !d_labels || !d_radius_sq || !d_out_counts)))
        return fail(c, PCORE_E_INVALID_ARG, "count_within: null pointer");
    if (!c->have_obs) return fail(c, PCORE_E_STATE, "count_within: the observation must be set first");
    if (n == 0) return PCORE_OK;
    HIPC(c, hipSetDevice(c->device));
    HIPC(c, launch_count_within(d_queries, d_labels, d_radius_sq, n, c->tgt.p, c->seg_lo.p, c->seg_hi.p,
                                c->num_obs > 0 ? c->num_grids : 0, d_out_counts, (hipStream_t)stream));
    return PCORE_OK;
}

int pcore_state_poses(pcore_ctx* c, const double* d_states, const int32_t* d_model, const double* cam_from_world,
                      const double* d_preprocess, int32_t num_models, int32_t n, float* d_out_poses,
                      pcore_stream stream) {
    if (!c) return PCORE_E_INVALID_ARG;
    if (n < 0 || !cam_from_world || num_models <= 0 ||
        (n > 0 && (!d_states || !d_model || !d_preprocess || !d_out_poses)))
        return fail(c, PCORE_E_INVALID_ARG, "state_poses: bad arguments");
    if (n == 0) return PCORE_OK;
    HIPC(c, hipSetDevice(c->device));
    HIPC(c, launch_state_poses(d_states, d_model, d_preprocess, cam_from_world, num_models, n, d_out_poses,
                               (hipStream_t)stream));
    return PCORE_OK;
}

int pcore_pose_distances(pcore_ctx* c, const float* d_pts, int32_t n, const double* d_T_gt, const double* d_T_est,
                         int32_t num_pairs, double* d_add, double* d_adds, pcore_stream stream) {
    if (!c) return PCORE_E_INVALID_ARG;
    if (n <= 0 || num_pairs < 0 || (num_pairs > 0 && (!d_pts || !d_T_gt || !d_T_est)))
        return fail(c, PCORE_E_INVALID_ARG, "pose_distances: need n > 0 points and pose pointers");
    if (num_pairs == 0 || (!d_add && !d_adds)) return PCORE_OK;
    if (num_pairs > 65535) return fail(c, PCORE_E_INVALID_ARG, "pose_distances: at most 65535 pairs per call");
    HIPC(c, hipSetDevice(c->device));
    HIPC(c, dev_reserve(c->metric_part, (size_t)2 * num_pairs * pose_dist_blocks(n)));
    HIPC(c, launch_pose_distances(d_pts, n, d_T_gt, d_T_est, num_pairs, c->metric_part.p, d_add, d_adds,
                                  (hipStream_t)stream));
    return PCORE_OK;
}

}
```

### perception_amd/csrc/pcore_fdiv.h

```cpp
#pragma once
#include <hip/hip_runtime.h>
#include <stdint.h>

namespace pcore {

__device__ __forceinline__ float recip_refined(float b) {
    const float r = __builtin_amdgcn_rcpf(b);
    const float e = __builtin_fmaf(-b, r, 1.0f);
    return __builtin_fmaf(e, r, r);
}

__device__ __forceinline__ float quot_refined(float a, float b, float r1) {
    const float q0 = a * r1;
    const float e1 = __builtin_fmaf(-b, q0, a);
    const float q1 = __builtin_fmaf(e1, r1, q0);
    const float e2 = __builtin_fmaf(-b, q1, a);
    return __builtin_fmaf(e2, r1, q1);
}

__device__ __forceinline__ uint32_t fexp_bits(float x) { return (__float_as_uint(x) >> 23) & 0xffu; }

__device__ __forceinline__ bool fdiv_range_ok(uint32_t emin, uint32_t emax) { return emin >= 87u && emax <= 167u; }

__device__ __forceinline__ float fdiv_exact(float a, float b) {
    const uint32_t ea = fexp_bits(a), eb = fexp_bits(b);
    float q = quot_refined(a, b, recip_refined(b));
    if (!fdiv_range_ok(min(ea, eb), max(ea, eb))) {
        asm volatile("");
        q = a / b;
    }
    return q;
}

__device__ __forceinline__ int32_t cvt_i32_rz_sat(float f) {
    int32_t r;
    asm("v_cvt_i32_f32 %0, %1" : "=v"(r) : "v"(f));
    return r;
}

__device__ __forceinline__ uint32_t absbits_zero_as_one(float x) {
    const uint32_t u = __float_as_uint(x) & 0x7fffffffu;
    return u == 0u ? 0x3f800000u : u;
}
__device__ __forceinline__ bool absbits_range_ok(uint32_t umin, uint32_t umax) {
    return umin >= (87u << 23) && umax < (168u << 23);
}

__device__ __forceinline__ int32_t frag_depth_ieee(float alpha, float beta, float gamma, float z0, float z1, float z2) {
    const float ox = alpha / z0, oy = beta / z1, oz = gamma / z2;
    return cvt_i32_rz_sat((alpha + beta + gamma) / (ox + oy + oz) + 0.5f);
}

__device__ __forceinline__ int32_t frag_depth_certified(float alpha, float beta, float gamma, float z0, float z1,
                                                        float z2, bool z_known_ok = false, bool active = true) {
    const float num = alpha + beta + gamma;
    const float oxa = alpha * __builtin_amdgcn_rcpf(z0), oya = beta * __builtin_amdgcn_rcpf(z1),
                oza = gamma * __builtin_amdgcn_rcpf(z2);
    const float f = num * __builtin_amdgcn_rcpf(oxa + oya + oza);
    const float e = fabsf(f) * 0x1p-19f;
    int32_t d = cvt_i32_rz_sat((f - e) + 0.5f);
    const int32_t dh = cvt_i32_rz_sat((f + e) + 0.5f);
    bool z_ok = z_known_ok;
    if (!z_known_ok) {
        const float zmin = fminf(fminf(z0, z1), z2), zmax = fmaxf(fmaxf(z0, z1), z2), zs = z0 + z1 + z2;
        z_ok = zmin >= 0x1p-100f && zmax <= 0x1p100f && zs == zs;
    }
    if (active && (!z_ok || num != num || d != dh)) {
        asm volatile("");
        d = frag_depth_ieee(alpha, beta, gamma, z0, z1, z2);
    }
    return d;
}

__device__ __forceinline__ void fdiv2_exact(float a0, float a1, float b, float& q0, float& q1) {
    const uint32_t e0 = fexp_bits(a0), e1 = fexp_bits(a1), eb = fexp_bits(b);
    const uint32_t emin = min(min(e0, e1), eb), emax = max(max(e0, e1), eb);
    const float r1 = recip_refined(b);
    q0 = quot_refined(a0, b, r1);
    q1 = quot_refined(a1, b, r1);
    if (!fdiv_range_ok(emin, emax)) {
        asm volatile("");
        q0 = a0 / b;
        q1 = a1 / b;
    }
}

}
```

### perception_amd/csrc/pcore_kernels.hip

```cpp
#include "pcore_internal.h"
#include "pcore_colour.h"
#include "pcore_cov.h"
#include "pcore_fdiv.h"

#include <algorithm>
#include <climits>
#include <cfloat>
#include <cstdlib>

#pragma clang fp contract(off)

#ifndef PCORE_FRAG_FDIV
#define PCORE_FRAG_FDIV 3
#endif
#ifndef PCORE_STEP_UNROLL
#define PCORE_STEP_UNROLL 1
#endif

namespace pcore {

constexpr int kWave = 64;
constexpr int kWaves = kFusedWaves;
constexpr int kThreads = kWaves * kWave;
constexpr int kRecCap = 128;
constexpr int kRecStride = kRecCap + 2;
constexpr int64_t PCORE_KEY_NONE_DEV = 0x7fffffffffffffffLL;
constexpr int kSmallK = 4;


__device__ __forceinline__ int32_t cvt_i32_x86(float f) {
    if (!(f == f) || f >= 2147483648.0f || f < -2147483648.0f) return INT_MIN;
    return (int32_t)f;
}

__device__ __forceinline__ int32_t iabs_wrap(int32_t a, int32_t b) {
    int32_t d = (int32_t)((uint32_t)a - (uint32_t)b);
    return d < 0 ? (int32_t)(0u - (uint32_t)d) : d;
}

__device__ __forceinline__ float ref_max(float a, float b) { return (a > b) ? a : b; }
__device__ __forceinline__ float ref_min(float a, float b) { return (a < b) ? a : b; }

__device__ __forceinline__ float row4(float m0, float m1, float m2, float m3, float x, float y, float z) {
    return m0 * x + m1 * y + m2 * z + m3;
}

__device__ __forceinline__ int32_t occlusion_rule(int32_t z, int32_t src, int lab, bool use_seg, int32_t pl,
                                                  float occlusion_threshold) {
    if (z == INT_MAX) return 0;
    bool cond;
    if (use_seg) cond = (pl != lab - 1) && ((float)iabs_wrap(z, src) > 0.5f);
    else cond = (float)iabs_wrap(z, src) > occlusion_threshold;
    if (cond && z > src && src > 0) return 0;
    return z;
}

__device__ __forceinline__ void bbox_ref(const float (&p)[3][2], float cmax0, float cmax1, float (&bmin)[2],
                                         float (&bmax)[2]) {
    bmin[0] = FLT_MAX; bmin[1] = FLT_MAX;
    bmax[0] = -FLT_MAX; bmax[1] = -FLT_MAX;
    const float cmax[2] = {cmax0, cmax1};
#pragma unroll
    for (int i = 0; i < 3; i++)
#pragma unroll
        for (int j = 0; j < 2; j++) {
            bmin[j] = ref_max(0.0f, ref_min(bmin[j], p[i][j]));
            bmax[j] = ref_min(cmax[j], ref_max(bmax[j], p[i][j]));
        }
}

__device__ __forceinline__ bool loop_bounds(float bmin, float bmax, int& lo, int& hi) {
    if (!(bmax >= 0.0f)) return false;
    const float st = bmin + 0.5f;
    int start;
    if (!(st > 0.0f)) start = 0;
    else if (st >= 1.0e9f) return false;
    else start = (int)st;
    hi = (int)floorf(bmax);
    lo = start;
    return lo <= hi;
}

__device__ __forceinline__ bool fragment(float A0, float A1, float B0, float B1, float C0, float C1, float z0,
                                         float z1, float z2, float P0, float P1, int32_t& depth, bool z_ok = false) {
    const float area = 0.5f * ((C0 - A0) * (B1 - A1) - (B0 - A0) * (C1 - A1));
    const float base_inv = 1.0f / area;
    const float beta = 0.5f * ((C0 - A0) * (P1 - A1) - (P0 - A0) * (C1 - A1)) * base_inv;
    const float gamma = 0.5f * ((P0 - A0) * (B1 - A1) - (B0 - A0) * (P1 - A1)) * base_inv;
    const float alpha = 1.0f - beta - gamma;
    float mn, mx;
    asm("v_min3_f32 %0, %1, %2, %3" : "=v"(mn) : "v"(alpha), "v"(beta), "v"(gamma));
    asm("v_max3_f32 %0, %1, %2, %3" : "=v"(mx) : "v"(alpha), "v"(beta), "v"(gamma));
    const bool inside = !(mn < -0.0f) && !(mx > 1.0f);
#if PCORE_FRAG_FDIV == 3
    depth = frag_depth_certified(alpha, beta, gamma, z0, z1, z2, z_ok, inside);
#else
    (void)z_ok;
    depth = 0;
    if (inside) {
        const float ox = alpha / z0, oy = beta / z1, oz = gamma / z2;
        depth = cvt_i32_rz_sat((alpha + beta + gamma) / (ox + oy + oz) + 0.5f);
    }
#endif
    return inside;
}

__device__ __forceinline__ void wave_sync() {
    __builtin_amdgcn_fence(__ATOMIC_RELEASE, "wavefront");
    __builtin_amdgcn_wave_barrier();
    __builtin_amdgcn_fence(__ATOMIC_ACQUIRE, "wavefront");
}

__device__ __forceinline__ int lane_id() { return __builtin_amdgcn_mbcnt_hi(~0u, __builtin_amdgcn_mbcnt_lo(~0u, 0)); }

__device__ __forceinline__ int mbcnt64(uint64_t mask) {
    return __builtin_amdgcn_mbcnt_hi((uint32_t)(mask >> 32), __builtin_amdgcn_mbcnt_lo((uint32_t)mask, 0));
}


struct TriRec {
    float a0, a1, b0, b1, c0, c1, z0, z1, z2;
};

template <int STRIDE>
__device__ __forceinline__ int sdiv(int v, int s) {
    if constexpr (STRIDE > 0) return v / STRIDE;
    else return v / s;
}

template <int STRIDE>
__device__ __forceinline__ int sample_window(const float (&bmin)[2], const float (&bmax)[2], int s, int H, int& kx0,
                                             int& ky0, int& nx, int& ny) {
    int lo0, hi0, lo1, hi1;
    if (!loop_bounds(bmin[0], bmax[0], lo0, hi0)) return 0;
    if (!loop_bounds(bmin[1], bmax[1], lo1, hi1)) return 0;
    const int ss = STRIDE > 0 ? STRIDE : s;
    kx0 = sdiv<STRIDE>(lo0 + ss - 1, s);
    const int kx1 = sdiv<STRIDE>(hi0, s);
    ky0 = sdiv<STRIDE>(H - 1 - hi1 + ss - 1, s);
    const int ky1 = sdiv<STRIDE>(H - 1 - lo1, s);
    nx = kx1 - kx0 + 1;
    ny = ky1 - ky0 + 1;
    if (nx <= 0 || ny <= 0) return 0;
    return nx * ny;
}

struct FusedSmem {
    int32_t* zbuf;
    float2* vxy;
    float* vz;
    uint2* vbd;
    uint2* ring;
    uint32_t* ring_id;
    uint32_t* bitmap;
    int32_t* counters;
};
constexpr int kRingSlots = kVRing * kWave;
static_assert(kRingSlots <= (1 << kRingSlotBits), "vertex ring slots must fit the 9-bit triangle indices");
static_assert(kVRing > kRefPasses, "the ring must hold the referenced passes and the one being written");
static_assert(kRecCap >= 128 && (kRecCap & (kRecCap - 1)) == 0, "record ring: >= 128 records, a power of two");

struct SampleWin {
    int x0, y0, nx, ny;
    int fastdiv;
};

template <bool IDPASS = false>
__device__ __forceinline__ void raster_sample(const TriRec& r, int kx, int ky, int s, int H, const SampleWin& w,
                                              int32_t* zbuf, int32_t* cid = nullptr, uint32_t id = 0) {
    const float P0 = (float)(kx * s);
    const float P1 = (float)(H - 1 - ky * s);
    int32_t d;
    const bool in = fragment(r.a0, r.a1, r.b0, r.b1, r.c0, r.c1, r.z0, r.z1, r.z2, P0, P1, d, w.fastdiv != 0);
    const int k = (int)__umul24((uint32_t)(ky - w.y0), (uint32_t)w.nx) + (kx - w.x0);
    if constexpr (IDPASS) {
        if (in && d == zbuf[k]) atomicMin(&cid[k], (int32_t)id);
    } else {
        if (in) atomicMin(&zbuf[k], d);
    }
}

size_t fused_lds_bytes(int tile_samples, int bitmap_words, bool colour) {
    auto al = [](size_t b) { return (b + 15) & ~size_t(15); };
    size_t b = al((size_t)tile_samples * 4);
    b += al((size_t)kWaves * kRingSlots * 8);
    b += al((size_t)kWaves * kRingSlots * 4);
    b += al((size_t)kWaves * 2 * kWave * 8);
    b += al((size_t)kWaves * kRecStride * 8);
    if (colour) b += al((size_t)kWaves * kRecStride * 4);
    b += al((size_t)bitmap_words * 4);
    b += 48;
    return b;
}

__device__ __forceinline__ FusedSmem carve_smem(unsigned char* smem_raw, int nsamp, int bitmap_words,
                                                bool colour = false) {
    auto al = [](size_t b) { return (b + 15) & ~size_t(15); };
    FusedSmem sm;
    unsigned char* p = smem_raw;
    sm.zbuf = (int32_t*)p; p += al((size_t)nsamp * 4);
    sm.vxy = (float2*)p; p += al((size_t)kWaves * kRingSlots * 8);
    sm.vz = (float*)p; p += al((size_t)kWaves * kRingSlots * 4);
    sm.vbd = (uint2*)p; p += al((size_t)kWaves * 2 * kWave * 8);
    sm.ring = (uint2*)p; p += al((size_t)kWaves * kRecStride * 8);
    sm.ring_id = nullptr;
    if (colour) { sm.ring_id = (uint32_t*)p; p += al((size_t)kWaves * kRecStride * 4); }
    sm.bitmap = (uint32_t*)p; p += al((size_t)bitmap_words * 4);
    sm.counters = (int32_t*)p;
    return sm;
}

template <int STRIDE>
__device__ __forceinline__ int floor_div(int v, int s) {
    if constexpr (STRIDE == 8) return v >> 3;
    else {
        const int q = v / s;
        return (v % s != 0 && v < 0) ? q - 1 : q;
    }
}

__device__ __forceinline__ int cvt_rpi(float v) {
    int r;
    asm("v_cvt_rpi_i32_f32 %0, %1" : "=v"(r) : "v"(v));
    return r;
}
__device__ __forceinline__ int cvt_flr(float v) {
    int r;
    asm("v_cvt_flr_i32_f32 %0, %1" : "=v"(r) : "v"(v));
    return r;
}

typedef short short2v __attribute__((ext_vector_type(2)));
__device__ __forceinline__ short2v as_s2(uint32_t v) { return __builtin_bit_cast(short2v, v); }
constexpr uint32_t kNanBounds = 0x80008000u;

template <int STRIDE>
__device__ __forceinline__ uint2 vertex_bounds(float sx, float sy, int s, float cmax0, float cmax1, int H,
                                              bool finite = false) {
    if (!finite && __builtin_isunordered(sx, sy)) return make_uint2(kNanBounds, 0u);
    const int ss = STRIDE > 0 ? STRIDE : s;
    const int lo0 = cvt_rpi(__builtin_amdgcn_fmed3f(sx, 0.0f, 65536.0f));
    const int lo1 = cvt_rpi(__builtin_amdgcn_fmed3f(sy, 0.0f, 65536.0f));
    const int hi0 = cvt_flr(__builtin_amdgcn_fmed3f(sx, -65536.0f, cmax0));
    const int hi1 = cvt_flr(__builtin_amdgcn_fmed3f(sy, -65536.0f, cmax1));
    int A0 = floor_div<STRIDE>(lo0 + ss - 1, s), A1 = floor_div<STRIDE>(hi0, s);
    int B0 = floor_div<STRIDE>(H - 1 - hi1 + ss - 1, s), B1 = floor_div<STRIDE>(H - 1 - lo1, s);
    if constexpr (STRIDE == 0) {
        A0 = min(A0, 32767);
        B0 = min(B0, 32767);
        A1 = max(A1, -32767);
        B1 = max(B1, -32767);
    }
    return make_uint2(((uint32_t)A0 & 0xffffu) | ((uint32_t)B0 << 16), ((uint32_t)A1 & 0xffffu) | ((uint32_t)B1 << 16));
}

#ifdef PCORE_FUSED_PROFILE
__device__ unsigned long long g_fprof[8];
extern "C" int pcore_debug_fused_profile(unsigned long long* out, int reset) {
    hipError_t e = hipMemcpyFromSymbol(out, HIP_SYMBOL(g_fprof), sizeof(unsigned long long) * 8);
    if (e == hipSuccess && reset) {
        const unsigned long long z[8] = {0, 0, 0, 0, 0, 0, 0, 0};
        e = hipMemcpyToSymbol(HIP_SYMBOL(g_fprof), z, sizeof(z));
    }
    return e == hipSuccess ? 0 : 1;
}
struct FProf {
    unsigned long long acc[8] = {0, 0, 0, 0, 0, 0, 0, 0};
    unsigned long long last = __builtin_amdgcn_s_memtime();
    __device__ __forceinline__ void mark(int k) {
        const unsigned long long t = __builtin_amdgcn_s_memtime();
        acc[k] += t - last;
        last = t;
    }
    __device__ __forceinline__ void flush() {
        if ((threadIdx.x & 63) == 0)
            for (int k = 0; k < 8; k++) atomicAdd(&g_fprof[k], acc[k]);
    }
};
#else
struct FProf {
    __device__ __forceinline__ void mark(int) {}
    __device__ __forceinline__ void flush() {}
};
#endif

#ifdef PCORE_FLUSH_STATS
__device__ unsigned long long pcore_flush_stats[9];
extern "C" int pcore_debug_flush_stats(unsigned long long* host) {
    return (int)hipMemcpyFromSymbol(host, HIP_SYMBOL(pcore_flush_stats), sizeof(unsigned long long) * 9);
}
#endif

template <int STRIDE, bool IDPASS = false, int FD = -1>
__device__ __forceinline__ void raster_phase(const FusedArgs& a, const FusedSmem& sm, int pose, const SampleWin& sw_in,
                                             int32_t* cid, FProf& fp) {
    SampleWin sw = sw_in;
    if constexpr (FD >= 0) sw.fastdiv = FD;
    const int tid = threadIdx.x;
    const int wave = __builtin_amdgcn_readfirstlane(tid >> 6);
    const int lane = tid & 63;
    const int s = STRIDE > 0 ? STRIDE : a.stride;
    const int W = a.width, H = a.height;
    const float* P = a.poses + (size_t)16 * pose;
    const float m00 = P[0], m01 = P[1], m02 = P[2], m03 = P[3];
    const float m10 = P[4], m11 = P[5], m12 = P[6], m13 = P[7];
    const float m20 = P[8], m21 = P[9], m22 = P[10], m23 = P[11];
    const int model = a.pose_model[pose];
    bool proj_sparse = false;
    if (a.proj_sparse && model >= 0 && model < a.num_models) {
        const float4 lo = a.model_box[2 * model], hi = a.model_box[2 * model + 1];
        const float ax = fmaxf(fabsf(lo.x), fabsf(hi.x)), ay = fmaxf(fabsf(lo.y), fabsf(hi.y));
        const float az = fmaxf(fabsf(lo.z), fabsf(hi.z));
        const float Bx = fabsf(m00) * ax + fabsf(m01) * ay + fabsf(m02) * az + fabsf(m03);
        const float By = fabsf(m10) * ax + fabsf(m11) * ay + fabsf(m12) * az + fabsf(m13);
        proj_sparse = lo.w != 0.0f && Bx < 1.0e30f && By < 1.0e30f;
    }
    __syncthreads();

    const float Wf = (float)W, Hf = (float)H;
    const float hw = Wf / 2.0f, hh = Hf / 2.0f;
    const float cmax0 = (float)(W - 1), cmax1 = (float)(H - 1);
    float2* vxy = sm.vxy + wave * kRingSlots;
    float* vz = sm.vz + wave * kRingSlots;
    uint2* vbd = sm.vbd + wave * 2 * kWave;
    const short2v wfirst = {(short)sw.x0, (short)sw.y0};
    const short2v wlast = {(short)(sw.x0 + sw.nx - 1), (short)(sw.y0 + sw.ny - 1)};
    uint2* ring = sm.ring + wave * kRecStride;
    uint32_t* ring_id = IDPASS ? sm.ring_id + wave * kRecStride : nullptr;
    int rec_total = 0, rec_done = 0;

#if PCORE_DEBUG_SKIP_RT
    const int dbg = a.dbg_skip;
#else
    constexpr int dbg = 0;
#endif
    auto flush = [&](int count) {
        fp.mark(2);
        wave_sync();
        if (!(dbg & 1)) {
            for (int base = 0; base < count; base += kWave) {
#ifdef PCORE_FLUSH_STATS
                if (lane == 0) {
                    atomicAdd(&pcore_flush_stats[0], 1ull);
                    atomicAdd(&pcore_flush_stats[1], (unsigned long long)min(count - base, kWave));
                }
#endif
                if (base + lane < count) {
                    const int j = (rec_done + base + lane) & (kRecCap - 1);
                    const uint2 rec = ring[j];
                    const uint32_t id = IDPASS ? ring_id[j] : 0u;
                    const int i0 = rec.x & 511, i1 = (rec.x >> 9) & 511, i2 = (rec.x >> 18) & 511;
                    const float2 q0 = vxy[i0], q1 = vxy[i1], q2 = vxy[i2];
                    TriRec r;
                    r.a0 = q0.x; r.a1 = q0.y;
                    r.b0 = q1.x; r.b1 = q1.y;
                    r.c0 = q2.x; r.c1 = q2.y;
                    r.z0 = vz[i0]; r.z1 = vz[i1]; r.z2 = vz[i2];
                    asm volatile("" : "+v"(r.z0), "+v"(r.z1), "+v"(r.z2));
#ifdef PCORE_FLUSH_STATS
                    atomicAdd(&pcore_flush_stats[2], 1ull);
#endif
                    raster_sample<IDPASS>(r, (int)(rec.y & 0xffffu), (int)(rec.y >> 16), s, H, sw, sm.zbuf, cid, id);
                }
            }
        }
        rec_done += count;
        wave_sync();
        fp.mark(3);
    };

    if (model < 0 || model >= a.num_models) return;
    const int st_lo = a.model_st_lo[model], st_hi = a.model_st_hi[model];
    fp.mark(0);
    for (int st = st_lo + wave; st < st_hi; st += kWaves) {
        const int4 sd = a.streams[st];
        if (rec_total > rec_done) {
#ifdef PCORE_FLUSH_STATS
            if (lane == 0) atomicAdd(&pcore_flush_stats[3], 1ull);
#endif
            flush(rec_total - rec_done);
        }
        int hist[kVRing - kRefPasses];
#pragma unroll
        for (int k = 0; k < kVRing - kRefPasses; k++) hist[k] = rec_total;
        int buf = 0;
        const uint32_t* tp = a.stris + (size_t)sd.x * kStepSlots;
        const uint32_t* op = IDPASS ? a.stri_orig + (size_t)sd.x * kStepSlots : nullptr;
        const float4* vq = a.sverts + (size_t)sd.z * kStepSlots;
        auto run_step = [&](int step, const float4& cv, const uint32_t ct, const uint32_t cidt, float4& ncv,
                            uint32_t& nct, uint32_t& ncid) {
            (void)step;
            tp += kStepSlots;
            nct = tp[lane];
            if constexpr (IDPASS) {
                op += kStepSlots;
                ncid = op[lane];
            } else {
                ncid = 0u;
            }
            const bool vpass = (__builtin_amdgcn_readfirstlane((int)ct) >> 30) & 1;
            if (vpass) vq += kStepSlots;
            ncv = vq[lane];
            if (vpass) {
                if (rec_done < hist[kVRing - kRefPasses - 1]) {
#ifdef PCORE_FLUSH_STATS
                    if (lane == 0) atomicAdd(&pcore_flush_stats[3], 1ull);
#endif
                    flush(rec_total - rec_done);
                }
                if (!(dbg & 8)) {
                    const float lx = row4(m00, m01, m02, m03, cv.x, cv.y, cv.z);
                    const float ly = row4(m10, m11, m12, m13, cv.x, cv.y, cv.z);
                    const float lz = row4(m20, m21, m22, m23, cv.x, cv.y, cv.z);
                    float px, py;
                    if (proj_sparse) {
                        px = a.p00 * lx + a.p02 * lz;
                        py = a.p11 * ly + a.p12 * lz;
                    } else {
                        px = row4(a.p00, a.p01, a.p02, a.p03, lx, ly, lz);
                        py = row4(a.p10, a.p11, a.p12, a.p13, lx, ly, lz);
                    }
                    const float r1 = recip_refined(lz);
                    float qx = quot_refined(px, lz, r1), qy = quot_refined(py, lz, r1);
                    float sx = qx * hw + hw, sy = qy * hh + hh;
                    if (!sw.fastdiv) {
                        const uint32_t ex = fexp_bits(px), ey = fexp_bits(py), ez = fexp_bits(lz);
                        if (!fdiv_range_ok(min(min(ex, ey), ez), max(max(ex, ey), ez))) {
                            asm volatile("");
                            qx = px / lz;
                            qy = py / lz;
                            sx = qx * Wf / 2.0f + Wf / 2.0f;
                            sy = qy * Hf / 2.0f + Hf / 2.0f;
                        }
                    }
                    vxy[buf * kWave + lane] = make_float2(sx, sy);
                    vz[buf * kWave + lane] = lz;
                    uint2 vb;
                    if (sw.fastdiv) vb = vertex_bounds<STRIDE>(sx, sy, s, cmax0, cmax1, H, true);
                    else vb = vertex_bounds<STRIDE>(sx, sy, s, cmax0, cmax1, H, false);
                    vbd[(buf & 1) * kWave + lane] = vb;
                }
#pragma unroll
                for (int k = kVRing - kRefPasses - 1; k > 0; k--) hist[k] = hist[k - 1];
                hist[0] = rec_total;
                buf = buf + 1 == kVRing ? 0 : buf + 1;
#ifdef PCORE_FLUSH_STATS
                if (lane == 0) atomicAdd(&pcore_flush_stats[8], 1ull);
#endif
                wave_sync();
            }
            fp.mark(1);
            if (!(dbg & 2)) {
                uint32_t pos = 0u, nxy = 0u;
                int nk = 0;
                auto slot_of = [ct](int k) { return (int)((ct >> (9 * k)) & 511u); };
                const bool pad = ct >> 31;
                {
                    uint32_t i1, i2;
                    asm("v_bfe_u32 %0, %1, 9, 7" : "=v"(i1) : "v"(ct));
                    asm("v_bfe_u32 %0, %1, 18, 7" : "=v"(i2) : "v"(ct));
                    const uint2 w0 = vbd[ct & 127u], w1 = vbd[i1], w2 = vbd[i2];
                    short2v lo = __builtin_elementwise_min(__builtin_elementwise_min(as_s2(w0.x), as_s2(w1.x)), as_s2(w2.x));
                    short2v hi = __builtin_elementwise_max(__builtin_elementwise_max(as_s2(w0.y), as_s2(w1.y)), as_s2(w2.y));
                    const bool nan_tri = !sw.fastdiv && lo.x < 0 && !pad;
                    lo = __builtin_elementwise_max(lo, wfirst);
                    hi = __builtin_elementwise_min(hi, wlast);
                    const short2v d = hi - lo;
                    const short2v one = {1, 1};
                    pos = __builtin_bit_cast(uint32_t, lo);
                    nxy = __builtin_bit_cast(uint32_t, d + one);
                    const bool nonempty = (__builtin_bit_cast(uint32_t, d) & 0x80008000u) == 0u && !pad;
                    nk = nonempty ? (int)__umul24(nxy & 0xffffu, nxy >> 16) : 0;
                    if (nan_tri) {
                        const float2 q0 = vxy[slot_of(0)], q1 = vxy[slot_of(1)], q2 = vxy[slot_of(2)];
                        const float p[3][2] = {{q0.x, q0.y}, {q1.x, q1.y}, {q2.x, q2.y}};
                        float bmin[2], bmax[2];
                        bbox_ref(p, cmax0, cmax1, bmin, bmax);
                        int kx0 = 0, ky0 = 0, nx = 0, ny = 0;
                        nk = sample_window<STRIDE>(bmin, bmax, s, H, kx0, ky0, nx, ny);
                        if (nk > 0) {
                            const int kx1 = min(kx0 + nx, sw.x0 + sw.nx), ky1 = min(ky0 + ny, sw.y0 + sw.ny);
                            kx0 = max(kx0, sw.x0);
                            ky0 = max(ky0, sw.y0);
                            nx = kx1 - kx0;
                            ny = ky1 - ky0;
                            nk = (nx > 0 && ny > 0) ? nx * ny : 0;
                        }
                        pos = (uint32_t)kx0 | ((uint32_t)ky0 << 16);
                        nxy = (uint32_t)nx | ((uint32_t)ny << 16);
                    }
                }
                uint64_t big = __ballot(nk > kSmallK);
#ifdef PCORE_FLUSH_STATS
                {
                    const uint64_t btouch = __ballot(nk > 0), blanes = __ballot(!(ct >> 31));
                    if (lane == 0) {
                        atomicAdd(&pcore_flush_stats[4], (unsigned long long)__popcll(big));
                        atomicAdd(&pcore_flush_stats[5], (unsigned long long)__popcll(btouch));
                        atomicAdd(&pcore_flush_stats[6], (unsigned long long)__popcll(blanes));
                        atomicAdd(&pcore_flush_stats[7], 1ull);
                    }
                }
#endif
                if (big) {
                    float2 q0 = make_float2(0.f, 0.f), q1 = q0, q2 = q0;
                    float z0 = 0.0f, z1 = 0.0f, z2 = 0.0f;
                    if (nk > kSmallK) {
                        const int i0 = slot_of(0), i1 = slot_of(1), i2 = slot_of(2);
                        q0 = vxy[i0];
                        q1 = vxy[i1];
                        q2 = vxy[i2];
                        z0 = vz[i0];
                        z1 = vz[i1];
                        z2 = vz[i2];
                    }
                    do {
                        const int j = __ffsll((unsigned long long)big) - 1;
                        big &= big - 1;
                        auto rl = [&](float x) { return __int_as_float(__builtin_amdgcn_readlane(__float_as_int(x), j)); };
                        TriRec rb;
                        rb.a0 = rl(q0.x); rb.a1 = rl(q0.y);
                        rb.b0 = rl(q1.x); rb.b1 = rl(q1.y);
                        rb.c0 = rl(q2.x); rb.c1 = rl(q2.y);
                        rb.z0 = rl(z0); rb.z1 = rl(z1); rb.z2 = rl(z2);
                        const uint32_t bpos = (uint32_t)__builtin_amdgcn_readlane((int)pos, j);
                        const int bkx0 = (int)(bpos & 0xffffu), bky0 = (int)(bpos >> 16);
                        const int bnx = (int)((uint32_t)__builtin_amdgcn_readlane((int)nxy, j) & 0xffffu);
                        const int bnk = __builtin_amdgcn_readlane(nk, j);
                        const uint32_t bid = IDPASS ? (uint32_t)__builtin_amdgcn_readlane((int)cidt, j) : 0u;
                        const float inv_nx = 1.0f / (float)bnx;
                        for (int q = lane; q < bnk; q += kWave) {
                            int iy = (int)(((float)q + 0.5f) * inv_nx), ix = q - iy * bnx;
                            if (ix < 0) { iy--; ix += bnx; } else if (ix >= bnx) { iy++; ix -= bnx; }
                            raster_sample<IDPASS>(rb, bkx0 + ix, bky0 + iy, s, H, sw, sm.zbuf, cid, bid);
                        }
                    } while (big);
                }
                const bool qd = nk > 0 && nk <= kSmallK;
                const uint64_t bq = __ballot(qd);
#if PCORE_RING_DISCARD
                {
                    const int slot = qd ? (rec_total + mbcnt64(bq)) & (kRecCap - 1) : kRecCap;
                    ring[slot] = make_uint2(ct, pos);
                    if (IDPASS) ring_id[slot] = cidt;
                }
#else
                if (qd) {
                    const int slot = (rec_total + mbcnt64(bq)) & (kRecCap - 1);
                    ring[slot] = make_uint2(ct, pos);
                    if (IDPASS) ring_id[slot] = cidt;
                }
#endif
                rec_total += __popcll(bq);
                while (rec_total - rec_done >= kWave) flush(kWave);
                if (__ballot(qd && nk > 1)) {
                    for (int q = 1; q < kSmallK; q++) {
                        const bool qr = qd && nk > q;
                        const uint64_t br = __ballot(qr);
                        if (!br) break;
                        if (qr) {
                            const int nx = (int)(nxy & 0xffffu);
                            const int iy = nx == 1 ? q : (nx == 2 ? q >> 1 : 0), ix = q - iy * nx;
                            const int slot = (rec_total + mbcnt64(br)) & (kRecCap - 1);
                            ring[slot] = make_uint2(ct, pos + (uint32_t)ix + ((uint32_t)iy << 16));
                            if (IDPASS) ring_id[slot] = cidt;
                        }
                        rec_total += __popcll(br);
                        while (rec_total - rec_done >= kWave) flush(kWave);
                    }
                }
            }
            fp.mark(2);
        };
        float4 cvA = vq[lane], cvB;
        uint32_t ctA = tp[lane], ctB, cidA, cidB;
        cidA = IDPASS ? op[lane] : 0u;
#if PCORE_STEP_UNROLL
        for (int step = sd.x; step < sd.y; step += 2) {
            run_step(step, cvA, ctA, cidA, cvB, ctB, cidB);
            if (step + 1 < sd.y) run_step(step + 1, cvB, ctB, cidB, cvA, ctA, cidA);
        }
#else
        for (int step = sd.x; step < sd.y; step++) {
            run_step(step, cvA, ctA, cidA, cvB, ctB, cidB);
            cvA = cvB; ctA = ctB; cidA = cidB;
        }
#endif
    }
    if (rec_total > rec_done) flush(rec_total - rec_done);
}

__device__ SampleWin pose_window(const FusedArgs& a, int model, const float (&m)[12], int s) {
    const SampleWin whole = {0, 0, a.ws, a.hs, 0};
    const float4 lo = a.model_box[2 * model], hi = a.model_box[2 * model + 1];
    const int c = lane_id() & 7;
    const float x = (c & 1) ? hi.x : lo.x, y = (c & 2) ? hi.y : lo.y, z = (c & 4) ? hi.z : lo.z;
    const float Wf = (float)a.width, Hf = (float)a.height;
    const float lx = row4(m[0], m[1], m[2], m[3], x, y, z);
    const float ly = row4(m[4], m[5], m[6], m[7], x, y, z);
    const float lz = row4(m[8], m[9], m[10], m[11], x, y, z);
    const float px = row4(a.p00, a.p01, a.p02, a.p03, lx, ly, lz);
    const float py = row4(a.p10, a.p11, a.p12, a.p13, lx, ly, lz);
    const float sx = px / lz * Wf / 2.0f + Wf / 2.0f;
    const float sy = py / lz * Hf / 2.0f + Hf / 2.0f;
    const bool bad = !(fabsf(sx) < 1.0e7f) || !(fabsf(sy) < 1.0e7f) || !(lz > 0.0f);
    float lzmin = lz, sx0 = sx, sx1 = sx, sy0 = sy, sy1 = sy;
#pragma unroll
    for (int off = 1; off < 8; off <<= 1) {
        lzmin = fminf(lzmin, __shfl_xor(lzmin, off));
        sx0 = fminf(sx0, __shfl_xor(sx0, off));
        sx1 = fmaxf(sx1, __shfl_xor(sx1, off));
        sy0 = fminf(sy0, __shfl_xor(sy0, off));
        sy1 = fmaxf(sy1, __shfl_xor(sy1, off));
    }
    auto uni = [](float v) { return __int_as_float(__builtin_amdgcn_readfirstlane(__float_as_int(v))); };
    lzmin = uni(lzmin); sx0 = uni(sx0); sx1 = uni(sx1); sy0 = uni(sy0); sy1 = uni(sy1);
    if ((__ballot(bad) & 0xffull) || lo.w == 0.0f) return whole;
    const float ax = fmaxf(fabsf(lo.x), fabsf(hi.x)), ay = fmaxf(fabsf(lo.y), fabsf(hi.y));
    const float az = fmaxf(fabsf(lo.z), fabsf(hi.z));
    const float Bx = fabsf(m[0]) * ax + fabsf(m[1]) * ay + fabsf(m[2]) * az + fabsf(m[3]);
    const float By = fabsf(m[4]) * ax + fabsf(m[5]) * ay + fabsf(m[6]) * az + fabsf(m[7]);
    const float Bz = fabsf(m[8]) * ax + fabsf(m[9]) * ay + fabsf(m[10]) * az + fabsf(m[11]);
    if (!(lzmin > 0.05f * Bz)) return whole;
    const float eps = 5.9604645e-8f;
    const float Pbx = fabsf(a.p00) * Bx + fabsf(a.p01) * By + fabsf(a.p02) * Bz + fabsf(a.p03);
    const float Pby = fabsf(a.p10) * Bx + fabsf(a.p11) * By + fabsf(a.p12) * Bz + fabsf(a.p13);
    const float mgx = 2.0f + 256.0f * eps * (0.5f * Wf) * Pbx / lzmin + 8.0f * eps * (fmaxf(fabsf(sx0), fabsf(sx1)) + Wf);
    const float mgy = 2.0f + 256.0f * eps * (0.5f * Hf) * Pby / lzmin + 8.0f * eps * (fmaxf(fabsf(sy0), fabsf(sy1)) + Hf);
    if (!(mgx < 1.0e6f) || !(mgy < 1.0e6f)) return whole;
    const float xlo = sx0 - mgx, xhi = sx1 + mgx, ylo = sy0 - mgy, yhi = sy1 + mgy;
    const float sf = (float)s;
    const int X0 = max(0, (int)floorf((xlo - 1.0f) / sf)), X1 = min(a.ws - 1, (int)floorf(xhi / sf));
    const int Y0 = max(0, (int)floorf((Hf - 1.0f - yhi) / sf)), Y1 = min(a.hs - 1, (int)floorf((Hf - ylo) / sf));
    const bool fastdiv = lzmin - 1.0e-5f * Bz >= 1.0f && Bz < 0x1p40f && Pbx < 0x1p40f && Pby < 0x1p40f;
    return SampleWin{X0, Y0, max(0, X1 - X0 + 1), max(0, Y1 - Y0 + 1), fastdiv ? 1 : 0};
}

__device__ __forceinline__ int64_t select_key(float rc, float oc, int m, int num_models, int64_t gidx) {
    const int32_t target = cvt_i32_x86(rc);
    const int32_t source = cvt_i32_x86(oc);
    const int32_t cost = (target < 0) ? -1 : cvt_i32_x86(rc + oc);
    const int32_t adiff = iabs_wrap(target, source);
    const bool ok = !(cost == -1 || cost == -2) && adiff < 30 && cost != INT_MAX && m >= 0 && m < num_models;
    if (!ok) return PCORE_KEY_NONE_DEV;
    const uint64_t hi = (uint64_t)((uint32_t)cost ^ 0x80000000u);
    return (int64_t)((hi << 31) | ((uint64_t)gidx & 0x7fffffffull));
}

template <int STRIDE, bool COLOUR>
__device__ __forceinline__ void fused_pose(const FusedArgs& a, const FusedSmem& sm, int pose, const SampleWin& pw,
                                           int cap) {
    const int tid = threadIdx.x;
    const int wave = __builtin_amdgcn_readfirstlane(tid >> 6);
    const int lane = tid & 63;
    const int s = STRIDE > 0 ? STRIDE : a.stride;
    const int ws = a.ws, nsamp = a.ws * a.hs;

    for (int i = tid; i < a.bitmap_words; i += kThreads) sm.bitmap[i] = 0u;
    if (tid < 4) sm.counters[tid] = 0;
    if (a.dbg_zs)
        for (int i = tid; i < nsamp; i += kThreads) a.dbg_zs[(size_t)pose * nsamp + i] = 0;

    const bool use_seg = a.pose_label != nullptr;
    const int32_t pl = use_seg ? a.pose_label[pose] : 0;
    FProf fp;
    int wave_bad = 0, wave_pts = 0;
    int32_t* cid = nullptr;
    if constexpr (COLOUR) cid = a.cid + (size_t)pose * nsamp;
    auto chunk = [&](const SampleWin& sw) __attribute__((always_inline)) {
    const int tn = sw.nx * sw.ny;
    for (int i = tid; i < tn; i += kThreads) sm.zbuf[i] = INT_MAX;
    if (sw.fastdiv) raster_phase<STRIDE, false, 1>(a, sm, pose, sw, nullptr, fp);
    else raster_phase<STRIDE, false, 0>(a, sm, pose, sw, nullptr, fp);
    fp.mark(2);
    __syncthreads();
    fp.mark(4);
    if constexpr (COLOUR) {
        for (int i = tid; i < tn; i += kThreads) cid[i] = INT_MAX;
        __syncthreads();
        raster_phase<STRIDE, true>(a, sm, pose, sw, cid, fp);
        __syncthreads();
    }

    int32_t* queue = reinterpret_cast<int32_t*>(sm.ring + wave * kRecStride);
    int qcount = 0;
    const int grid_id = use_seg ? pl : a.num_grids;
    const bool grid_ok = use_seg ? (pl >= 0 && pl < a.num_grids) : true;
    LabelGrid g;
    if (grid_ok) g = a.grids[grid_id];
    const float r_eff = sqrtf(a.r2) * 1.0001f + 1e-7f;
    int my_bad = 0;

    auto process_points = [&](int count) {
        wave_sync();
        for (int base = 0; base < count; base += kWave) {
            const int j = base + lane;
            bool is_bad = false;
            if (j < count) {
                const int k = queue[2 * j];
                const int kxy = queue[2 * j + 1];
                const int32_t Z = sm.zbuf[k];
                const int kx = kxy & 0xffff, ky = kxy >> 16;
                const float zp = (float)Z / a.depth_factor;
                const float xp = ((float)(kx * s) - a.cx) / a.fx * zp;
                const float yp = ((float)(ky * s) - a.cy) / a.fy * zp;
                float best = INFINITY;
                int bidx = 0x7fffffff;
                if (grid_ok) {
                    const float rc = r_eff * g.inv_c;
                    const float fx0 = (xp - g.ox) * g.inv_c, fy0 = (yp - g.oy) * g.inv_c, fz0 = (zp - g.oz) * g.inv_c;
                    const float lx = fx0 - rc, hx = fx0 + rc, ly = fy0 - rc, hy = fy0 + rc, lz = fz0 - rc, hz = fz0 + rc;
                    if (hx >= 0.0f && lx < (float)g.nx && hy >= 0.0f && ly < (float)g.ny && hz >= 0.0f && lz < (float)g.nz) {
                        const int ix0 = (int)floorf(fmaxf(lx, 0.0f)), ix1 = min(g.nx - 1, (int)floorf(hx));
                        const int iy0 = (int)floorf(fmaxf(ly, 0.0f)), iy1 = min(g.ny - 1, (int)floorf(hy));
                        const int iz0 = (int)floorf(fmaxf(lz, 0.0f)), iz1 = min(g.nz - 1, (int)floorf(hz));
                        int cb[4], ce[4];
#pragma unroll
                        for (int q = 0; q < 4; q++) {
                            const int iy = iy0 + (q & 1), iz = iz0 + (q >> 1);
                            const bool ok = iy <= iy1 && iz <= iz1;
                            const int c = g.cell_base + (iz * g.ny + iy) * g.nx + ix0;
                            cb[q] = ok ? a.cell_start[c] : 0;
                            ce[q] = ok ? a.cell_start[c + 1 + (ix1 - ix0)] : 0;
                        }
                        const int l0 = ce[0] - cb[0], l1 = l0 + (ce[1] - cb[1]), l2 = l1 + (ce[2] - cb[2]);
                        const int ltot = l2 + (ce[3] - cb[3]);
                        for (int k0 = 0; k0 < ltot; k0 += 4) {
                            float4 o[4];
#pragma unroll
                            for (int u = 0; u < 4; u++) {
                                const int k = min(k0 + u, ltot - 1);
                                const int pi = k < l0 ? cb[0] + k : k < l1 ? cb[1] + (k - l0)
                                             : k < l2 ? cb[2] + (k - l1) : cb[3] + (k - l2);
                                o[u] = a.grid_pts[pi];
                            }
#pragma unroll
                            for (int u = 0; u < 4; u++) {
                                const float dx = xp - o[u].x, dy = yp - o[u].y, dz = zp - o[u].z;
                                const float d = dx * dx + dy * dy + dz * dz;
                                const int oi = __float_as_int(o[u].w);
                                const bool take = k0 + u < ltot && (d < best || (d == best && oi < bidx));
                                best = take ? d : best;
                                bidx = take ? oi : bidx;
                            }
                        }
                    }
                }
                if (best > a.r2) {
                    is_bad = true;
                } else if (bidx != 0x7fffffff) {
                    bool expl = true;
                    if constexpr (COLOUR) {
                        const int id = cid[k];
                        const float4 lr = a.tri_lab[id == INT_MAX ? 0 : id];
                        const float4 lo = a.obs_lab[bidx];
                        const double cd = colour::colour_distance(lo.x, lo.y, lo.z, lr.x, lr.y, lr.z);
                        expl = !(cd > (double)a.colour_thr);
                    }
                    if (expl) atomicOr(&sm.bitmap[bidx >> 5], 1u << (bidx & 31));
                    else is_bad = true;
                }
            }
            my_bad += is_bad ? 1 : 0;
        }
        wave_sync();
    };

    const float inv_nx = tn > 0 ? 1.0f / (float)sw.nx : 0.0f;
    for (int base = wave * kWave; base < tn; base += kThreads) {
        const int k = base + lane;
        bool valid = false;
        int kx = 0, ky = 0;
#if PCORE_DEBUG_SKIP_RT
        if (k < tn && !(a.dbg_skip & 4)) {
#else
        if (k < tn) {
#endif
            int iy = (int)(((float)k + 0.5f) * inv_nx), ix = k - iy * sw.nx;
            if (ix < 0) { iy--; ix += sw.nx; } else if (ix >= sw.nx) { iy++; ix -= sw.nx; }
            kx = sw.x0 + ix;
            ky = sw.y0 + iy;
            const int gk = ky * ws + kx;
            const int32_t z = sm.zbuf[k];
            const int32_t zf = z == INT_MAX ? 0
                                            : occlusion_rule(z, a.src_s[gk], use_seg ? (int)a.lab_s[gk] : 0, use_seg,
                                                             pl, a.occlusion_threshold);
            if (zf != z) sm.zbuf[k] = zf;
            if (a.dbg_zs) a.dbg_zs[(size_t)pose * nsamp + gk] = zf;
            valid = zf > 0;
        }
        const uint64_t bv = __ballot(valid);
        if (valid) {
            const int q = qcount + mbcnt64(bv);
            queue[2 * q] = k;
            queue[2 * q + 1] = kx | (ky << 16);
        }
        qcount += __popcll(bv);
        wave_pts += __popcll(bv);
        if (qcount >= kWave) {
            process_points(qcount);
            qcount = 0;
        }
    }
    if (qcount > 0) process_points(qcount);
    fp.mark(5);
    for (int off = 32; off > 0; off >>= 1) my_bad += __shfl_xor(my_bad, off);
    wave_bad += __builtin_amdgcn_readfirstlane(my_bad);
    };
    if (pw.nx * pw.ny <= cap) {
        chunk(pw);
    } else {
        const int cw = min(pw.nx, cap), ch = max(1, cap / max(cw, 1));
        for (int r0 = 0; r0 < pw.ny; r0 += ch)
            for (int c0 = 0; c0 < pw.nx; c0 += cw) {
                if (r0 > 0 || c0 > 0) __syncthreads();
                chunk(SampleWin{pw.x0 + c0, pw.y0 + r0, min(cw, pw.nx - c0), min(ch, pw.ny - r0), pw.fastdiv});
            }
    }
    __syncthreads();
    if (lane == 0) atomicAdd(&sm.counters[0], wave_bad);
    int my_expl = 0;
    for (int w = tid; w < a.bitmap_words; w += kThreads) my_expl += __popc(sm.bitmap[w]);
    for (int off = 32; off > 0; off >>= 1) my_expl += __shfl_xor(my_expl, off);
    if (lane == 0) {
        atomicAdd(&sm.counters[1], my_expl);
        atomicAdd(&sm.counters[2], wave_pts);
    }
    __syncthreads();

    if (tid == 0) {
        const float num = (float)sm.counters[2];
        const float badf = (float)sm.counters[0];
        const float rendered_explained = num - badf;
        float rc = (num == 0.0f) ? -1.0f : badf / num;
        rc = (rc == -1.0f) ? -1.0f : rc * 100.0f;
        a.out_rc[pose] = rc;
        float ocw = 0.0f;
        if (a.calc_obs) {
            const float expl = (float)sm.counters[1];
            const float tot = a.pose_obs_total[pose];
            a.out_diff[pose] = rendered_explained - expl;
            float oc = tot - expl;
            oc = oc / tot;
            ocw = oc * 100.0f;
            a.out_oc[pose] = ocw;
        } else {
            if (a.out_oc) a.out_oc[pose] = 0.0f;
            if (a.out_diff) a.out_diff[pose] = 0.0f;
        }
        if (a.sel_keys) {
            const int m = a.pose_model[pose];
            const int64_t key = select_key(rc, ocw, m, a.sel_models, a.sel_base + pose);
            if (key != PCORE_KEY_NONE_DEV) atomicMin((unsigned long long*)&a.sel_keys[m], (unsigned long long)key);
        }
    }
    fp.mark(6);
    fp.flush();
}

__device__ __forceinline__ void load_pose_rows(const float* poses, int pose, float (&m)[12]) {
    const float* P = poses + (size_t)16 * pose;
#pragma unroll
    for (int i = 0; i < 12; i++) m[i] = P[i];
}

#ifdef PCORE_WG_TIMING
__device__ unsigned long long pcore_wg_clock[2 * 1048576];
extern "C" int pcore_debug_wg_clock(unsigned long long* host, int n) {
    return (int)hipMemcpyFromSymbol(host, HIP_SYMBOL(pcore_wg_clock), sizeof(unsigned long long) * 2 * (size_t)n);
}
#endif

#ifndef PCORE_FUSED_WAVES_PER_EU
#define PCORE_FUSED_WAVES_PER_EU PCORE_TIER_MAX
#endif
template <int STRIDE, bool COLOUR = false>
__global__ void __launch_bounds__(kThreads) __attribute__((amdgpu_waves_per_eu(COLOUR ? 1 : PCORE_FUSED_WAVES_PER_EU)))
fused_cost_kernel(FusedArgs a) {
    extern __shared__ __attribute__((aligned(16))) unsigned char smem_raw[];
    const int pose = blockIdx.x;
#ifdef PCORE_WG_TIMING
    if (threadIdx.x == 0) pcore_wg_clock[2 * pose] = wall_clock64();
    struct End {
        int pose;
        __device__ ~End() {
            __syncthreads();
            if (threadIdx.x == 0) pcore_wg_clock[2 * pose + 1] = wall_clock64();
        }
    } end_clock{pose};
#endif
    const FusedSmem sm = carve_smem(smem_raw, a.tcap, a.bitmap_words, COLOUR);
    if (threadIdx.x < kWave) {
        const int model = a.pose_model[pose];
        SampleWin w = {0, 0, 0, 0, 0};
        if (model >= 0 && model < a.num_models) {
            float m[12];
            load_pose_rows(a.poses, pose, m);
            w = pose_window(a, model, m, STRIDE > 0 ? STRIDE : a.stride);
        }
        if (threadIdx.x == 0) {
            sm.counters[4] = w.x0;
            sm.counters[5] = w.y0;
            sm.counters[6] = w.nx;
            sm.counters[7] = w.ny;
            sm.counters[8] = w.fastdiv;
        }
    }
    __syncthreads();
    const SampleWin sw = {__builtin_amdgcn_readfirstlane(sm.counters[4]), __builtin_amdgcn_readfirstlane(sm.counters[5]),
                          __builtin_amdgcn_readfirstlane(sm.counters[6]), __builtin_amdgcn_readfirstlane(sm.counters[7]),
                          __builtin_amdgcn_readfirstlane(sm.counters[8])};
    const int tn = sw.nx * sw.ny;
    if (threadIdx.x == 0) {
        const int par = a.fb_par;
        int b = 0;
#pragma unroll
        for (int t = 0; t < kTileTiers; t++) b += tn > a.hist_edge[t] ? 1 : 0;
        atomicAdd(&a.win_hist[par * (kTileTiers + 1) + b], 1);
        if (tn > a.tcap) atomicAdd(&a.fb_ctr[par], 1);
        if (blockIdx.x == 0 && a.fb_host) {
            const int o = (1 - par) * (kTileTiers + 1);
            for (int k = 0; k <= kTileTiers; k++) a.fb_host[k] = atomicExch(&a.win_hist[o + k], 0);
            a.fb_host[kTileTiers + 1] = atomicExch(&a.fb_ctr[1 - par], 0);
            a.fb_host[kTileTiers + 2] = a.fb_seq - 1;
        }
    }
    fused_pose<STRIDE, COLOUR>(a, sm, pose, sw, a.tcap);
}

constexpr int kProbeBlocks = 2048;
__global__ void __launch_bounds__(kThreads) window_probe_kernel(FusedArgs a, int32_t* hist) {
    constexpr int kWaves = kThreads / kWave;
    int cnt[kTileTiers + 1] = {};
    for (int pose = blockIdx.x * kWaves + (int)(threadIdx.x / kWave); pose < a.num_poses;
         pose += gridDim.x * kWaves) {
        const int model = a.pose_model[pose];
        int tn = 0;
        if (model >= 0 && model < a.num_models) {
            float m[12];
            load_pose_rows(a.poses, pose, m);
            const SampleWin w = pose_window(a, model, m, a.stride);
            tn = w.nx * w.ny;
        }
        int b = 0;
#pragma unroll
        for (int t = 0; t < kTileTiers; t++) b += tn > a.hist_edge[t] ? 1 : 0;
#pragma unroll
        for (int k = 0; k <= kTileTiers; k++) cnt[k] += b == k ? 1 : 0;
    }
    __shared__ int32_t wg_cnt[kTileTiers + 1];
    if (threadIdx.x <= kTileTiers) wg_cnt[threadIdx.x] = 0;
    __syncthreads();
    if (lane_id() == 0) {
#pragma unroll
        for (int k = 0; k <= kTileTiers; k++)
            if (cnt[k]) atomicAdd(&wg_cnt[k], cnt[k]);
    }
    __syncthreads();
    if (threadIdx.x <= kTileTiers && wg_cnt[threadIdx.x]) atomicAdd(&hist[threadIdx.x], wg_cnt[threadIdx.x]);
}

hipError_t launch_window_probe(const FusedArgs& a, int32_t* hist, hipStream_t s) {
    if (a.num_poses <= 0) return hipSuccess;
    const int per_wg = kThreads / kWave;
    const int blocks = std::min(kProbeBlocks, (a.num_poses + per_wg - 1) / per_wg);
    hipLaunchKernelGGL(window_probe_kernel, dim3(blocks), dim3(kThreads), 0, s, a, hist);
    return hipGetLastError();
}

template <int STRIDE>
__global__ void __launch_bounds__(kThreads) render_cloud_kernel(FusedArgs a) {
    extern __shared__ __attribute__((aligned(16))) unsigned char smem_raw[];
    __shared__ int wsum[kWaves];
    __shared__ int carry_s;
    const int pose = blockIdx.x;
    const int tid = threadIdx.x, wave = tid >> 6, lane = tid & 63;
    const int s = STRIDE > 0 ? STRIDE : a.stride;
    const int ws = a.ws, nsamp = a.ws * a.hs;
    const int cap = a.tcap > 0 && a.tcap < nsamp ? a.tcap : nsamp;
    const FusedSmem sm = carve_smem(smem_raw, cap, 0);
    const int model = a.pose_model[pose];
    SampleWin sw = {0, 0, 0, 0, 0};
    if (model >= 0 && model < a.num_models) {
        float m[12];
        load_pose_rows(a.poses, pose, m);
        sw = pose_window(a, model, m, s);
    }
    if (tid == 0) carry_s = 0;
    const bool use_seg = a.pose_label != nullptr;
    const int32_t pl = use_seg ? a.pose_label[pose] : 0;
    FProf fp;
    float4* out = a.cloud_out + (size_t)pose * a.cloud_cap;
    auto chunk = [&](const SampleWin& cw) __attribute__((always_inline)) {
        const int tn = cw.nx * cw.ny;
        for (int i = tid; i < tn; i += kThreads) sm.zbuf[i] = INT_MAX;
        if (cw.fastdiv) raster_phase<STRIDE, false, 1>(a, sm, pose, cw, nullptr, fp);
        else raster_phase<STRIDE, false, 0>(a, sm, pose, cw, nullptr, fp);
        __syncthreads();
        const float inv_nx = tn > 0 ? 1.0f / (float)cw.nx : 0.0f;
        for (int base = 0; base < tn; base += kThreads) {
            const int k = base + tid;
            int32_t zf = 0;
            int kx = 0, ky = 0;
            if (k < tn) {
                int iy = (int)(((float)k + 0.5f) * inv_nx), ix = k - iy * cw.nx;
                if (ix < 0) { iy--; ix += cw.nx; } else if (ix >= cw.nx) { iy++; ix -= cw.nx; }
                kx = cw.x0 + ix;
                ky = cw.y0 + iy;
                const int gk = ky * ws + kx;
                zf = occlusion_rule(sm.zbuf[k], a.src_s[gk], use_seg ? (int)a.lab_s[gk] : 0, use_seg, pl,
                                    a.occlusion_threshold);
            }
            const bool valid = zf > 0;
            const uint64_t b = __ballot(valid);
            if (lane == 0) wsum[wave] = __popcll(b);
            __syncthreads();
            int woff = 0, tot = 0;
            for (int w = 0; w < kWaves; w++) {
                if (w < wave) woff += wsum[w];
                tot += wsum[w];
            }
            const int carry = carry_s;
            if (valid) {
                const int o = carry + woff + mbcnt64(b);
                const float zp = (float)zf / a.depth_factor;
                const float xp = ((float)(kx * s) - a.cx) / a.fx * zp;
                const float yp = ((float)(ky * s) - a.cy) / a.fy * zp;
                if (o < a.cloud_cap) out[o] = make_float4(xp, yp, zp, 0.0f);
            }
            __syncthreads();
            if (tid == 0) carry_s = carry + tot;
            __syncthreads();
        }
    };
    if (sw.nx * sw.ny <= cap) {
        chunk(sw);
    } else {
        const int cw = min(sw.nx, cap), ch = max(1, cap / max(cw, 1));
        for (int r0 = 0; r0 < sw.ny; r0 += ch)
            for (int c0 = 0; c0 < sw.nx; c0 += cw)
                chunk(SampleWin{sw.x0 + c0, sw.y0 + r0, min(cw, sw.nx - c0), min(ch, sw.ny - r0), sw.fastdiv});
    }
    if (tid == 0) a.cloud_count[pose] = carry_s < a.cloud_cap ? carry_s : a.cloud_cap;
    if (a.cloud_cov) {
        __syncthreads();
        const int n = carry_s < a.cloud_cap ? carry_s : a.cloud_cap;
        float4* tile = reinterpret_cast<float4*>(sm.vxy) + wave * kCovLanes;
        double* C = a.cloud_cov + (size_t)6 * pose * a.cloud_cap;
        for (int i0 = wave * kCovLanes; i0 < n; i0 += kThreads)
            cov_knn_round<10, true>(out, n, 10, i0, lane, tile, C);
    }
}

hipError_t launch_render_cloud(const FusedArgs& a, hipStream_t s) {
    const int nsamp = a.ws * a.hs;
    const size_t lds = fused_lds_bytes(a.tcap > 0 && a.tcap < nsamp ? a.tcap : nsamp, 0);
    if (a.num_poses <= 0) return hipSuccess;
    if (a.stride == 8)
        hipLaunchKernelGGL(render_cloud_kernel<8>, dim3(a.num_poses), dim3(kThreads), lds, s, a);
    else
        hipLaunchKernelGGL(render_cloud_kernel<0>, dim3(a.num_poses), dim3(kThreads), lds, s, a);
    return hipGetLastError();
}

int fused_tier_samples(int t, int ws, int hs, int bitmap_words, bool colour, const DeviceInfo& d) {
    const int nsamp = ws * hs;
    const size_t granule = d.lds_granule;
    const size_t per_wg = (d.lds_per_cu / tier_wgs(t)) / granule * granule;
    const size_t fixed = fused_lds_bytes(0, bitmap_words, colour);
    if (per_wg <= fixed + 64) return 0;
    const int cap = (int)((per_wg - fixed) / 4) & ~3;
    return cap >= nsamp ? nsamp : cap;
}

hipError_t launch_fused_cost(const FusedArgs& a0, hipStream_t s) {
    if (a0.num_poses <= 0) return hipSuccess;
    const bool colour = a0.cid != nullptr;
    const int nsamp = a0.ws * a0.hs;
    FusedArgs a = a0;
    if (a.tcap <= 0 || a.tcap > nsamp) a.tcap = nsamp;
    const size_t lds = fused_lds_bytes(a.tcap, a.bitmap_words, colour);
    if (colour)
        hipLaunchKernelGGL((fused_cost_kernel<0, true>), dim3(a.num_poses), dim3(kThreads), lds, s, a);
    else if (a.stride == 8)
        hipLaunchKernelGGL(fused_cost_kernel<8>, dim3(a.num_poses), dim3(kThreads), lds, s, a);
    else
        hipLaunchKernelGGL(fused_cost_kernel<0>, dim3(a.num_poses), dim3(kThreads), lds, s, a);
    return hipGetLastError();
}


__global__ void __launch_bounds__(256) render_full_kernel(const float* tris, int num_tris, const int32_t* tri_lo,
                                                          const int32_t* tri_hi, const float* poses,
                                                          const int32_t* pose_model, int width, int height,
                                                          const float* proj, int32_t* depth) {
    const int pose = blockIdx.y;
    const int t = blockIdx.x * blockDim.x + threadIdx.x;
    if (t >= num_tris) return;
    const int m = pose_model[pose];
    if (!(t >= tri_lo[m] && t < tri_hi[m])) return;
    const float* M = poses + (size_t)16 * pose;
    const float* tp = tris + (size_t)9 * t;
    const float Wf = (float)width, Hf = (float)height;
    float p[3][2], z[3];
#pragma unroll
    for (int k = 0; k < 3; k++) {
        const float x = tp[3 * k], y = tp[3 * k + 1], zz = tp[3 * k + 2];
        const float lx = row4(M[0], M[1], M[2], M[3], x, y, zz);
        const float ly = row4(M[4], M[5], M[6], M[7], x, y, zz);
        const float lz = row4(M[8], M[9], M[10], M[11], x, y, zz);
        const float px = row4(proj[0], proj[1], proj[2], proj[3], lx, ly, lz);
        const float py = row4(proj[4], proj[5], proj[6], proj[7], lx, ly, lz);
        p[k][0] = px / lz * Wf / 2.0f + Wf / 2.0f;
        p[k][1] = py / lz * Hf / 2.0f + Hf / 2.0f;
        z[k] = lz;
    }
    float bmin[2], bmax[2];
    bbox_ref(p, (float)(width - 1), (float)(height - 1), bmin, bmax);
    int lo0, hi0, lo1, hi1;
    if (!loop_bounds(bmin[0], bmax[0], lo0, hi0) || !loop_bounds(bmin[1], bmax[1], lo1, hi1)) return;
    int32_t* img = depth + (size_t)pose * width * height;
    for (int P1 = lo1; P1 <= hi1; P1++)
        for (int P0 = lo0; P0 <= hi0; P0++) {
            int32_t d;
            if (fragment(p[0][0], p[0][1], p[1][0], p[1][1], p[2][0], p[2][1], z[0], z[1], z[2], (float)P0, (float)P1, d))
                atomicMin(&img[P0 + (size_t)(height - 1 - P1) * width], d);
        }
}

__global__ void __launch_bounds__(256) render_full_tri_kernel(const float* tris, int num_tris, const int32_t* tri_lo,
                                                              const int32_t* tri_hi, const float* poses,
                                                              const int32_t* pose_model, int width, int height,
                                                              const float* proj, const int32_t* depth,
                                                              int32_t* tri_min) {
    const int pose = blockIdx.y;
    const int t = blockIdx.x * blockDim.x + threadIdx.x;
    if (t >= num_tris) return;
    const int m = pose_model[pose];
    if (!(t >= tri_lo[m] && t < tri_hi[m])) return;
    const float* M = poses + (size_t)16 * pose;
    const float* tp = tris + (size_t)9 * t;
    const float Wf = (float)width, Hf = (float)height;
    float p[3][2], z[3];
#pragma unroll
    for (int k = 0; k < 3; k++) {
        const float x = tp[3 * k], y = tp[3 * k + 1], zz = tp[3 * k + 2];
        const float lx = row4(M[0], M[1], M[2], M[3], x, y, zz);
        const float ly = row4(M[4], M[5], M[6], M[7], x, y, zz);
        const float lz = row4(M[8], M[9], M[10], M[11], x, y, zz);
        const float px = row4(proj[0], proj[1], proj[2], proj[3], lx, ly, lz);
        const float py = row4(proj[4], proj[5], proj[6], proj[7], lx, ly, lz);
        p[k][0] = px / lz * Wf / 2.0f + Wf / 2.0f;
        p[k][1] = py / lz * Hf / 2.0f + Hf / 2.0f;
        z[k] = lz;
    }
    float bmin[2], bmax[2];
    bbox_ref(p, (float)(width - 1), (float)(height - 1), bmin, bmax);
    int lo0, hi0, lo1, hi1;
    if (!loop_bounds(bmin[0], bmax[0], lo0, hi0) || !loop_bounds(bmin[1], bmax[1], lo1, hi1)) return;
    const size_t base = (size_t)pose * width * height;
    for (int P1 = lo1; P1 <= hi1; P1++)
        for (int P0 = lo0; P0 <= hi0; P0++) {
            int32_t d;
            if (fragment(p[0][0], p[0][1], p[1][0], p[1][1], p[2][0], p[2][1], z[0], z[1], z[2], (float)P0, (float)P1, d)) {
                const size_t i = base + P0 + (size_t)(height - 1 - P1) * width;
                if (d == depth[i]) atomicMin(&tri_min[i], t);
            }
        }
}

__global__ void render_finalize_kernel(int32_t* depth, const int32_t* src_depth, const uint8_t* src_mask,
                                       const int32_t* pose_label, int width, int height, float occlusion_threshold,
                                       const int32_t* tri_min, const uint32_t* rgb, uint8_t* color, int num_poses) {
    const int pose = blockIdx.y;
    const size_t npx = (size_t)width * height;
    const bool use_seg = pose_label != nullptr;
    const int32_t pl = use_seg ? pose_label[pose] : 0;
    int32_t* img = depth + npx * pose;
    const size_t plane = npx * (size_t)num_poses;
    for (size_t i = (size_t)blockIdx.x * blockDim.x + threadIdx.x; i < npx; i += (size_t)gridDim.x * blockDim.x) {
        const int32_t dmin = img[i];
        const int32_t z = occlusion_rule(dmin, src_depth[i], use_seg ? (int)src_mask[i] : 0, use_seg, pl, occlusion_threshold);
        img[i] = z;
        if (color) {
            const bool shown = dmin != INT_MAX && z == dmin;
            const uint32_t c = shown ? rgb[tri_min[npx * pose + i]] : 0u;
            uint8_t* px = color + npx * pose + i;
            px[0] = (uint8_t)(c & 0xff);
            px[plane] = (uint8_t)((c >> 8) & 0xff);
            px[2 * plane] = (uint8_t)((c >> 16) & 0xff);
        }
    }
}

__global__ void fill_i32_kernel(int32_t* p, int32_t v, size_t n) {
    for (size_t i = (size_t)blockIdx.x * blockDim.x + threadIdx.x; i < n; i += (size_t)gridDim.x * blockDim.x) p[i] = v;
}

hipError_t launch_fill_i32(int32_t* p, int32_t v, size_t n, hipStream_t s) {
    if (n == 0) return hipSuccess;
    size_t blocks = (n + 255) / 256;
    if (blocks > 4096) blocks = 4096;
    hipLaunchKernelGGL(fill_i32_kernel, dim3((unsigned)blocks), dim3(256), 0, s, p, v, n);
    return hipGetLastError();
}

hipError_t launch_render_full(const float* tris, int num_tris, const int32_t* tri_lo, const int32_t* tri_hi,
                              const float* poses, const int32_t* pose_model, int num_poses, int width, int height,
                              const float* proj, int32_t* depth, hipStream_t s) {
    if (num_poses <= 0 || num_tris <= 0) return hipSuccess;
    dim3 grid((num_tris + 255) / 256, num_poses);
    hipLaunchKernelGGL(render_full_kernel, grid, dim3(256), 0, s, tris, num_tris, tri_lo, tri_hi, poses, pose_model,
                       width, height, proj, depth);
    return hipGetLastError();
}

hipError_t launch_render_full_tri(const float* tris, int num_tris, const int32_t* tri_lo, const int32_t* tri_hi,
                                  const float* poses, const int32_t* pose_model, int num_poses, int width, int height,
                                  const float* proj, const int32_t* depth, int32_t* tri_min, hipStream_t s) {
    if (num_poses <= 0 || num_tris <= 0) return hipSuccess;
    dim3 grid((num_tris + 255) / 256, num_poses);
    hipLaunchKernelGGL(render_full_tri_kernel, grid, dim3(256), 0, s, tris, num_tris, tri_lo, tri_hi, poses,
                       pose_model, width, height, proj, depth, tri_min);
    return hipGetLastError();
}

hipError_t launch_render_finalize(int32_t* depth, const int32_t* src_depth, const uint8_t* src_mask,
                                  const int32_t* pose_label, int num_poses, int width, int height,
                                  float occlusion_threshold, hipStream_t s, const int32_t* tri_min,
                                  const uint32_t* rgb, uint8_t* color) {
    if (num_poses <= 0) return hipSuccess;
    const size_t npx = (size_t)width * height;
    unsigned bx = (unsigned)((npx + 255) / 256);
    if (bx > 256) bx = 256;
    hipLaunchKernelGGL(render_finalize_kernel, dim3(bx, num_poses), dim3(256), 0, s, depth, src_depth, src_mask,
                       pose_label, width, height, occlusion_threshold, tri_min, rgb, color, num_poses);
    return hipGetLastError();
}


__device__ __forceinline__ bool cloud_valid(const int32_t* depth, const uint8_t* label_mask, size_t idx, int x, int y,
                                            const CloudBounds& cb) {
    if (depth[idx] <= 0) return false;
    if (label_mask != nullptr && label_mask[idx] <= 0) return false;
    if (cb.on) {
        const float zc = (float)depth[idx] / cb.depth_factor;
        const float xc = ((float)x - cb.cx) / cb.fx * zc;
        const float yc = ((float)y - cb.cy) / cb.fy * zc;
        float w[3];
#pragma unroll
        for (int r = 0; r < 3; r++) {
            w[r] = cb.m[4 * r] * xc + cb.m[4 * r + 1] * yc + cb.m[4 * r + 2] * zc;
            w[r] = w[r] + cb.m[4 * r + 3];
        }
        if (w[0] > cb.b[0] || w[0] < cb.b[1]) return false;
        if (w[1] > cb.b[2] || w[1] < cb.b[3]) return false;
        if (w[2] > cb.b[4] || w[2] < cb.b[5]) return false;
    }
    return true;
}

__global__ void cloud_count_kernel(const int32_t* depth, int width, int height, int stride, const uint8_t* label_mask,
                                   CloudBounds cb, int32_t* counts) {
    const int n = blockIdx.x;
    const int ws = (width + stride - 1) / stride, hs = (height + stride - 1) / stride;
    const size_t npx = (size_t)width * height;
    int c = 0;
    for (int k = threadIdx.x; k < ws * hs; k += blockDim.x) {
        const int ky = k / ws, kx = k - ky * ws;
        c += cloud_valid(depth, label_mask, npx * n + (size_t)(kx * stride) + (size_t)(ky * stride) * width,
                         kx * stride, ky * stride, cb) ? 1 : 0;
    }
    for (int off = 32; off > 0; off >>= 1) c += __shfl_xor(c, off);
    __shared__ int part[16];
    if ((threadIdx.x & 63) == 0) part[threadIdx.x >> 6] = c;
    __syncthreads();
    if (threadIdx.x == 0) {
        int t = 0;
        for (int w = 0; w < (int)(blockDim.x >> 6); w++) t += part[w];
        counts[n] = t;
    }
}

__global__ void exclusive_scan_kernel(const int32_t* in, int32_t* out, int n, int32_t* total) {
    __shared__ int wsum[16];
    __shared__ int carry_s;
    const int lane = threadIdx.x & 63, wave = threadIdx.x >> 6, nw = blockDim.x >> 6;
    if (threadIdx.x == 0) carry_s = 0;
    __syncthreads();
    for (int base = 0; base < n; base += blockDim.x) {
        const int i = base + threadIdx.x;
        const int v = i < n ? in[i] : 0;
        int incl = v;
        for (int off = 1; off < 64; off <<= 1) {
            const int y = __shfl_up(incl, off);
            if (lane >= off) incl += y;
        }
        if (lane == 63) wsum[wave] = incl;
        __syncthreads();
        int woff = 0;
        for (int w = 0; w < wave; w++) woff += wsum[w];
        int chunk_total = 0;
        for (int w = 0; w < nw; w++) chunk_total += wsum[w];
        const int carry = carry_s;
        if (i < n) out[i] = carry + woff + incl - v;
        __syncthreads();
        if (threadIdx.x == 0) carry_s = carry + chunk_total;
        __syncthreads();
    }
    if (threadIdx.x == 0 && total) *total = carry_s;
}

__global__ void cloud_write_kernel(const int32_t* depth, int width, int height, int stride, float cx, float cy,
                                   float fx, float fy, float depth_factor, const uint8_t* label_mask,
                                   const int32_t* pose_label, const int32_t* offsets, float* xyz, int32_t* pose_out,
                                   int32_t* label_out, int cap, CloudBounds cb, const uint8_t* rgb_in,
                                   uint8_t* rgb_out, const uint8_t* planes_in, uint8_t* planes_out, int num_poses) {
    __shared__ int wsum[16];
    __shared__ int carry_s;
    const int n = blockIdx.x;
    const int lane = threadIdx.x & 63, wave = threadIdx.x >> 6, nw = blockDim.x >> 6;
    const int ws = (width + stride - 1) / stride, hs = (height + stride - 1) / stride;
    const size_t npx = (size_t)width * height;
    if (threadIdx.x == 0) carry_s = offsets[n];
    __syncthreads();
    for (int base = 0; base < ws * hs; base += blockDim.x) {
        const int k = base + threadIdx.x;
        bool v = false;
        int kx = 0, ky = 0;
        size_t idx = 0;
        if (k < ws * hs) {
            ky = k / ws; kx = k - ky * ws;
            idx = npx * n + (size_t)(kx * stride) + (size_t)(ky * stride) * width;
            v = cloud_valid(depth, label_mask, idx, kx * stride, ky * stride, cb);
        }
        const uint64_t b = __ballot(v);
        if (lane == 0) wsum[wave] = __popcll(b);
        __syncthreads();
        int woff = 0, tot = 0;
        for (int w = 0; w < nw; w++) {
            if (w < wave) woff += wsum[w];
            tot += wsum[w];
        }
        const int carry = carry_s;
// ... 176 lines not shown
```

### perception_amd/csrc/pcore_streams.h

```cpp
#pragma once
#include <algorithm>
#include <cmath>
#include <cstdint>
#include <cstring>
#include <vector>

namespace pcore {
namespace streams {

struct F4 {
    float x, y, z, w;
};
struct I4 {
    int32_t x, y, z, w;
};

struct Built {
    std::vector<F4> sverts;
    std::vector<uint32_t> stris;
    std::vector<uint32_t> sorig;
    std::vector<I4> streams;
    long long passes = 0, steps = 0, filled = 0;
};

inline std::vector<int> locality_order(const std::vector<int>& tv, int num_verts) {
    const int T = (int)tv.size() / 3;
    std::vector<std::vector<int>> adj(num_verts);
    for (int t = 0; t < T; t++)
        for (int k = 0; k < 3; k++) adj[tv[3 * t + k]].push_back(t);
    std::vector<char> done(T, 0);
    std::vector<int> order;
    order.reserve(T);
    std::vector<int> stamp(num_verts, -1);
    int next_seed = 0;
    const int window = 96;
    std::vector<int> cand;
    while ((int)order.size() < T) {
        while (next_seed < T && done[next_seed]) next_seed++;
        int cur = next_seed;
        while (cur >= 0) {
            done[cur] = 1;
            const int pos = (int)order.size();
            order.push_back(cur);
            for (int k = 0; k < 3; k++) stamp[tv[3 * cur + k]] = pos;
            int best = -1, best_score = -1;
            const int lo = std::max(0, pos - 8);
            for (int q = pos; q >= lo; q--) {
                const int t = order[q];
                for (int k = 0; k < 3; k++)
                    for (int u : adj[tv[3 * t + k]]) {
                        if (done[u]) continue;
                        int score = 0;
                        for (int kk = 0; kk < 3; kk++) {
                            const int sv = stamp[tv[3 * u + kk]];
                            score += (sv >= 0 && pos - sv <= window) ? 1 : 0;
                        }
                        if (score > best_score || (score == best_score && u < best)) {
                            best_score = score;
                            best = u;
                        }
                    }
                if (best_score == 3) break;
            }
            cur = best;
        }
    }
    return order;
}

inline std::vector<int> sweep_order(const std::vector<int>& tv, const std::vector<float>& vxyz) {
    const int T = (int)tv.size() / 3;
    std::vector<int> bin(T);
    std::vector<float> cx(T), cy(T), cz(T);
    for (int t = 0; t < T; t++) {
        const float* a = &vxyz[3 * tv[3 * t]];
        const float* b = &vxyz[3 * tv[3 * t + 1]];
        const float* c = &vxyz[3 * tv[3 * t + 2]];
        const double ux = b[0] - a[0], uy = b[1] - a[1], uz = b[2] - a[2];
        const double vx = c[0] - a[0], vy = c[1] - a[1], vz = c[2] - a[2];
        const double nx = uy * vz - uz * vy, ny = uz * vx - ux * vz, nz = ux * vy - uy * vx;
        const double ax = std::fabs(nx), ay = std::fabs(ny), az = std::fabs(nz);
        int bb;
        if (!(ax == ax && ay == ay && az == az)) bb = 6;
        else if (ax >= ay && ax >= az) bb = nx >= 0 ? 0 : 1;
        else if (ay >= az) bb = ny >= 0 ? 2 : 3;
        else bb = nz >= 0 ? 4 : 5;
        bin[t] = bb;
        cx[t] = (a[0] + b[0] + c[0]) / 3.0f; cy[t] = (a[1] + b[1] + c[1]) / 3.0f; cz[t] = (a[2] + b[2] + c[2]) / 3.0f;
        if (!(cx[t] == cx[t] && cy[t] == cy[t] && cz[t] == cz[t])) { cx[t] = cy[t] = cz[t] = 0.0f; bin[t] = 6; }
    }
    std::vector<int> order;
    order.reserve(T);
    for (int bb = 0; bb < 7; bb++) {
        std::vector<int> ts;
        for (int t = 0; t < T; t++) if (bin[t] == bb) ts.push_back(t);
        if (ts.empty()) continue;
        double m[3] = {0, 0, 0};
        for (int t : ts) { m[0] += cx[t]; m[1] += cy[t]; m[2] += cz[t]; }
        for (double& v : m) v /= ts.size();
        double C[3][3] = {{0}};
        for (int t : ts) {
            const double d[3] = {cx[t] - m[0], cy[t] - m[1], cz[t] - m[2]};
            for (int i = 0; i < 3; i++) for (int j = 0; j < 3; j++) C[i][j] += d[i] * d[j];
        }
        double e[3] = {1.0, 0.7, 0.4};
        for (int it = 0; it < 50; it++) {
            double f[3] = {0, 0, 0};
            for (int i = 0; i < 3; i++) for (int j = 0; j < 3; j++) f[i] += C[i][j] * e[j];
            const double n = std::sqrt(f[0] * f[0] + f[1] * f[1] + f[2] * f[2]);
            if (!(n > 0)) break;
            for (int i = 0; i < 3; i++) e[i] = f[i] / n;
        }
        std::vector<std::pair<double, int>> key;
        for (int t : ts) key.push_back({cx[t] * e[0] + cy[t] * e[1] + cz[t] * e[2], t});
        std::stable_sort(key.begin(), key.end(),
                         [](const std::pair<double, int>& p, const std::pair<double, int>& q) { return p.first < q.first; });
        for (auto& k : key) order.push_back(k.second);
    }
    return order;
}

constexpr int kNever = -(1 << 20);
constexpr uint32_t kStepVertexPass = 1u << 30;
constexpr uint32_t kSlotPadding = 1u << 31;

inline void build_model_order(const std::vector<int>& tv, const std::vector<float>& vxyz, const std::vector<int>& order0,
                              int tri_base, int num_streams, int vring, int ref_passes, Built& out, int chunks) {
    const int T = (int)tv.size() / 3;
    if (T == 0) return;
    const int num_verts = (int)vxyz.size() / 3;
    const int S = std::max(1, std::min(num_streams, (T + 63) / 64));
    const int C = std::max(1, std::min(S * std::max(chunks, 1), (T + 255) / 256));
    std::vector<int> order;
    order.reserve(T);
    std::vector<int> stream_end;
    for (int sidx = 0; sidx < S; sidx++) {
        for (int c = sidx; c < C; c += S) {
            const int c0 = (int)((long long)T * c / C), c1 = (int)((long long)T * (c + 1) / C);
            order.insert(order.end(), order0.begin() + c0, order0.begin() + c1);
        }
        stream_end.push_back((int)order.size());
    }
    std::vector<int> latest(num_verts, kNever), slot(num_verts, 0);
    std::vector<char> in_new(num_verts, 0);
    std::vector<int> newv, batch;
    for (int sidx = 0; sidx < S; sidx++) {
        const int b0 = sidx == 0 ? 0 : stream_end[sidx - 1], b1 = stream_end[sidx];
        I4 sd;
        sd.x = (int)(out.stris.size() / 64);
        sd.z = (int)(out.sverts.size() / 64);
        for (int i = b0; i < b1; i++)
            for (int k = 0; k < 3; k++) latest[tv[3 * order[i] + k]] = kNever;
        int P = -1, i = b0;
        bool attached = true;
        batch.clear();
        auto emit = [&]() {
            const uint32_t vflag = attached ? 0u : kStepVertexPass;
            for (int t : batch) {
                const int v0 = tv[3 * t], v1 = tv[3 * t + 1], v2 = tv[3 * t + 2];
                out.stris.push_back((uint32_t)slot[v0] | ((uint32_t)slot[v1] << 9) | ((uint32_t)slot[v2] << 18) | vflag);
                out.sorig.push_back((uint32_t)(tri_base + t));
            }
            for (int k = (int)batch.size(); k < 64; k++) {
                out.stris.push_back(kSlotPadding | vflag);
                out.sorig.push_back(0u);
            }
            out.filled += (long long)batch.size();
            out.steps++;
            attached = true;
            batch.clear();
        };
        auto usable_after = [&](int t, int head) {
            for (int k = 0; k < 3; k++)
                if (latest[tv[3 * t + k]] <= head - ref_passes) return false;
            return true;
        };
        while (true) {
            while (i < b1 && usable_after(order[i], P)) {
                batch.push_back(order[i++]);
                if ((int)batch.size() == 64) emit();
            }
            if (i >= b1) {
                if (!batch.empty() || !attached) emit();
                break;
            }
            newv.clear();
            if (!batch.empty()) {
                bool carry = attached;
                for (int t : batch)
                    for (int k = 0; k < 3 && carry; k++) {
                        const int v = tv[3 * t + k];
                        if (latest[v] > P + 1 - ref_passes || in_new[v]) continue;
                        in_new[v] = 1;
                        newv.push_back(v);
                        carry = (int)newv.size() <= 32;
                    }
                if (!carry) {
                    for (int v : newv) in_new[v] = 0;
                    newv.clear();
                    emit();
                }
            } else if (!attached) {
                emit();
            }
            for (int j = i; j < b1; j++) {
                int miss[3], nm = 0;
                for (int k = 0; k < 3; k++) {
                    const int v = tv[3 * order[j] + k];
                    if (latest[v] > P + 1 - ref_passes || in_new[v]) continue;
                    bool dup = false;
                    for (int q = 0; q < nm; q++) dup |= miss[q] == v;
                    if (!dup) miss[nm++] = v;
                }
                if ((int)newv.size() + nm > 64) break;
                for (int q = 0; q < nm; q++) {
                    in_new[miss[q]] = 1;
                    newv.push_back(miss[q]);
                }
            }
            P++;
            for (int k = 0; k < (int)newv.size(); k++) {
                const int v = newv[k];
                in_new[v] = 0;
                latest[v] = P;
                slot[v] = (P % vring) * 64 + k;
                out.sverts.push_back(F4{vxyz[3 * v], vxyz[3 * v + 1], vxyz[3 * v + 2], 1.0f});
            }
            for (int k = (int)newv.size(); k < 64; k++) out.sverts.push_back(F4{0.0f, 0.0f, 0.0f, 0.0f});
            out.passes++;
            attached = false;
        }
        sd.y = (int)(out.stris.size() / 64);
        sd.w = (int)(out.sverts.size() / 64);
        out.streams.push_back(sd);
    }
}

inline void build_model(const std::vector<int>& tv, const std::vector<float>& vxyz, int tri_base, int num_streams,
                        int vring, int ref_passes, Built& out, int chunks = 4) {
    if (tv.empty()) return;
    Built a, b;
    build_model_order(tv, vxyz, locality_order(tv, (int)vxyz.size() / 3), tri_base, num_streams, vring, ref_passes, a,
                      chunks);
    build_model_order(tv, vxyz, sweep_order(tv, vxyz), tri_base, num_streams, vring, ref_passes, b, chunks);
    const Built& w = (b.passes < a.passes || (b.passes == a.passes && b.steps < a.steps)) ? b : a;
    const int step0 = (int)(out.stris.size() / 64), pass0 = (int)(out.sverts.size() / 64);
    out.sverts.insert(out.sverts.end(), w.sverts.begin(), w.sverts.end());
    out.stris.insert(out.stris.end(), w.stris.begin(), w.stris.end());
    out.sorig.insert(out.sorig.end(), w.sorig.begin(), w.sorig.end());
    for (I4 sd : w.streams) {
        sd.x += step0;
        sd.y += step0;
        sd.z += pass0;
        sd.w += pass0;
        out.streams.push_back(sd);
    }
    out.passes += w.passes;
    out.steps += w.steps;
    out.filled += w.filled;
}

}
}
```

Baseline: 35.93 million poses/s.

## Tune stream ordering, hoist sparse-projection test, drop half factors in barycentrics

Several changes ship together. Barycentrics in the fast-divide raster path no longer apply the redundant 0.5 factors. The sparse-projection check moves into pose_window and is carried in SampleWin instead of being recomputed per pose in the raster loop. The host-side mesh stream builder now tries look-ahead batching over many band orderings and keeps whichever gives fewer passes and steps. A debug render-cloud API and a bary_check tool are also added. Dropping the 0.5 factors may change rounding at triangle edges.

```diff
diff --git a/include/pcore.h b/include/pcore.h
--- a/include/pcore.h
+++ b/include/pcore.h
@@ -124,6 +124,10 @@
                            float fx, float fy, float cx, float cy, const pcore_p2p_icp_params* icp, float* d_out_T,
                            float* d_out_fitness, float* d_out_rmse, int32_t* d_out_iters, pcore_stream stream);
 
+int pcore_debug_render_clouds(pcore_ctx* ctx, const float* d_poses, const int32_t* d_pose_model,
+                              const int32_t* d_pose_label, int32_t num_poses, const pcore_eval_params* params,
+                              float* d_out_xyzw, int32_t* d_out_count, pcore_stream stream);
+
 int pcore_render(pcore_ctx* ctx, const float* d_poses, const int32_t* d_pose_model, const int32_t* d_pose_label,
                  int32_t num_poses, float occlusion_threshold, int32_t* d_out_depth, uint8_t* d_out_color,
                  pcore_stream stream);
diff --git a/perception_amd/_native.py b/perception_amd/_native.py
--- a/perception_amd/_native.py
+++ b/perception_amd/_native.py
@@ -27,7 +27,7 @@
     "pcore_count_within", "pcore_state_poses", "pcore_evaluate_select", "pcore_get_tile_info", "pcore_debug_lm_solve",
     "pcore_debug_covariances", "pcore_debug_covariances_cloud", "pcore_debug_gicp_help_stats", "pcore_depth_to_cloud_ex",
     "pcore_icp_planar", "pcore_debug_planar_step",
-    "pcore_scene_projective",
+    "pcore_scene_projective", "pcore_debug_render_clouds",
 )
 EXPORTED_SYMBOLS_WITH_DIGITS = ("pcore_icp_point2plane", "pcore_debug_p2p_clouds")
 
@@ -168,6 +168,8 @@
                                             ctypes.POINTER(P2pIcpParams), vp, vp, vp, vp, vp, vp]
         L.pcore_debug_p2p_clouds.argtypes = [vp, vp, i32, i32, vp, vp, i32, i32, f32, f32, f32, f32,
                                              ctypes.POINTER(P2pIcpParams), vp, vp, vp, vp, vp]
+    if hasattr(L, "pcore_debug_render_clouds"):
+        L.pcore_debug_render_clouds.argtypes = [vp, vp, vp, vp, i32, ctypes.POINTER(EvalParams), vp, vp, vp]
     L.pcore_select.argtypes = [vp, vp, vp, vp, i32, i64, i32, vp, vp]
     L.pcore_pose_distances.argtypes = [vp, vp, i32, vp, vp, i32, vp, vp, vp]
     L.pcore_set_observation_colors.argtypes = [vp, vp, i32, vp]
diff --git a/perception_amd/build.py b/perception_amd/build.py
--- a/perception_amd/build.py
+++ b/perception_amd/build.py
@@ -70,7 +70,7 @@
     out_dir = os.path.join(root, "tools", "bin")
     os.makedirs(out_dir, exist_ok=True)
     built = []
-    for name in ("fdiv_check",):
+    for name in ("fdiv_check", "bary_check"):
         src = os.path.join(root, "tools", name + ".hip")
         out = os.path.join(out_dir, name)
         cmd = [hipcc(), f"--offload-arch={ARCH}", "-O3", "-std=c++17", "-ffp-contract=off", "-fno-fast-math", src,
diff --git a/perception_amd/core.py b/perception_amd/core.py
--- a/perception_amd/core.py
+++ b/perception_amd/core.py
@@ -314,6 +314,22 @@
                                    sensor_resolution=sensor_resolution, occlusion_threshold=occlusion_threshold,
                                    color_distance_threshold=color_distance_threshold, stream=stream)
         return adj, iters, rc, oc, df, fitness, rmse
+
+    def render_clouds(self, poses: torch.Tensor, pose_model: torch.Tensor, pose_label: Optional[torch.Tensor] = None,
+                      stride: int = 8, depth_factor: float = 100.0, occlusion_threshold: float = 1.0, stream=None
+                      ) -> Tuple[torch.Tensor, torch.Tensor]:
+        n = int(poses.shape[0])
+        w, h = self.width, self.height
+        nsamp = (w // stride) * ((h + stride - 1) // stride)
+        xyzw = torch.zeros((n, nsamp, 4), dtype=torch.float32, device=poses.device)
+        cnt = torch.zeros(n, dtype=torch.int32, device=poses.device)
+        p = EvalParams(_native.COST_DEPTH_6DOF, 0, int(stride), float(depth_factor), 0.0, float(occlusion_threshold),
+                       0.0)
+        self._check(self.lib.pcore_debug_render_clouds(
+            self._h, _ptr(poses, torch.float32, "poses"), _ptr(pose_model, torch.int32, "pose_model"),
+            _ptr(pose_label, torch.int32, "pose_label"), n, ctypes.byref(p), _ptr(xyzw, torch.float32, "xyzw"),
+            _ptr(cnt, torch.int32, "count"), _stream(stream)))
+        return xyzw, cnt
 
     def render(self, poses: torch.Tensor, pose_model: torch.Tensor, pose_label: Optional[torch.Tensor],
                occlusion_threshold: float = 1.0, out: Optional[torch.Tensor] = None, color: bool = False,
diff --git a/perception_amd/csrc/pcore_api.hip b/perception_amd/csrc/pcore_api.hip
--- a/perception_amd/csrc/pcore_api.hip
+++ b/perception_amd/csrc/pcore_api.hip
@@ -1377,6 +1377,45 @@
     return launch_p2p_icp(g, num_segs, (hipStream_t)stream) == hipSuccess ? PCORE_OK : PCORE_E_HIP;
 }
 
+int pcore_debug_render_clouds(pcore_ctx* c, const float* d_poses, const int32_t* d_pose_model,
+                              const int32_t* d_pose_label, int32_t num_poses, const pcore_eval_params* p,
+                              float* d_out_xyzw, int32_t* d_out_count, pcore_stream stream) {
+    if (!c) return PCORE_E_INVALID_ARG;
+    if (!p) return fail(c, PCORE_E_INVALID_ARG, "debug_render_clouds: null parameters");
+    if (!c->have_mesh || !c->have_cam || !c->have_obs)
+        return fail(c, PCORE_E_STATE, "debug_render_clouds: meshes, camera and observation must be set first");
+    if (num_poses < 0 || (num_poses > 0 && (!d_poses || !d_pose_model || !d_out_xyzw || !d_out_count)))
+        return fail(c, PCORE_E_INVALID_ARG, "debug_render_clouds: null pose / output pointer");
+    if (d_pose_label && !c->obs_has_mask)
+        return fail(c, PCORE_E_INVALID_ARG, "debug_render_clouds: pose labels need a source mask");
+    const int W = c->cam.width, H = c->cam.height;
+    if (p->stride <= 0 || W % p->stride != 0)
+        return fail(c, PCORE_E_INVALID_ARG, "debug_render_clouds: width must be a multiple of stride");
+    const int ws = W / p->stride, hs = (H + p->stride - 1) / p->stride;
+    if (ws > 4095 || hs > 4095) return fail(c, PCORE_E_INVALID_ARG, "debug_render_clouds: sampled image too large");
+    if (fused_lds_bytes(ws * hs, c->bitmap_words, false) > (size_t)c->prop.sharedMemPerBlock)
+        return fail(c, PCORE_E_INVALID_ARG, "debug_render_clouds: sampled z-buffer does not fit in LDS");
+    if (num_poses == 0) return PCORE_OK;
+    HIPC(c, hipSetDevice(c->device));
+    hipStream_t s = (hipStream_t)stream;
+    int rc = ensure_sampled(c, p->stride, s);
+    if (rc != PCORE_OK) return rc;
+    FusedArgs a{};
+    fill_fused_args(c, p, a);
+    a.poses = d_poses;
+    a.pose_model = d_pose_model;
+    a.pose_label = d_pose_label;
+    a.num_poses = num_poses;
+    a.cloud_out = (float4*)d_out_xyzw;
+    a.cloud_count = d_out_count;
+    a.cloud_cap = ws * hs;
+    a.tcap = fused_tier_samples(0, a.ws, a.hs, 0, false, c->dinfo);
+    if (const char* e = getenv("PCORE_FUSED_TCAP")) a.tcap = std::min(std::max(atoi(e), 1), a.ws * a.hs);
+    if (a.tcap <= 0) a.tcap = a.ws * a.hs;
+    HIPC(c, launch_render_cloud(a, s));
+    return PCORE_OK;
+}
+
 int pcore_render(pcore_ctx* c, const float* d_poses, const int32_t* d_pose_model, const int32_t* d_pose_label,
                  int32_t num_poses, float occlusion_threshold, int32_t* d_out_depth, uint8_t* d_out_color,
                  pcore_stream stream) {
diff --git a/perception_amd/csrc/pcore_fdiv.h b/perception_amd/csrc/pcore_fdiv.h
--- a/perception_amd/csrc/pcore_fdiv.h
+++ b/perception_amd/csrc/pcore_fdiv.h
@@ -46,6 +46,21 @@
     return umin >= (87u << 23) && umax < (168u << 23);
 }
 
+template <bool NOHALF>
+__device__ __forceinline__ void frag_barycentrics(float A0, float A1, float B0, float B1, float C0, float C1, float P0,
+                                                  float P1, float& beta, float& gamma) {
+    if constexpr (NOHALF) {
+        const float base_inv = 1.0f / ((C0 - A0) * (B1 - A1) - (B0 - A0) * (C1 - A1));
+        beta = ((C0 - A0) * (P1 - A1) - (P0 - A0) * (C1 - A1)) * base_inv;
+        gamma = ((P0 - A0) * (B1 - A1) - (B0 - A0) * (P1 - A1)) * base_inv;
+    } else {
+        const float area = 0.5f * ((C0 - A0) * (B1 - A1) - (B0 - A0) * (C1 - A1));
+        const float base_inv = 1.0f / area;
+        beta = 0.5f * ((C0 - A0) * (P1 - A1) - (P0 - A0) * (C1 - A1)) * base_inv;
+        gamma = 0.5f * ((P0 - A0) * (B1 - A1) - (B0 - A0) * (P1 - A1)) * base_inv;
+    }
+}
+
 __device__ __forceinline__ int32_t frag_depth_ieee(float alpha, float beta, float gamma, float z0, float z1, float z2) {
     const float ox = alpha / z0, oy = beta / z1, oz = gamma / z2;
     return cvt_i32_rz_sat((alpha + beta + gamma) / (ox + oy + oz) + 0.5f);
diff --git a/perception_amd/csrc/pcore_kernels.hip b/perception_amd/csrc/pcore_kernels.hip
--- a/perception_amd/csrc/pcore_kernels.hip
+++ b/perception_amd/csrc/pcore_kernels.hip
@@ -15,6 +15,12 @@
 #endif
 #ifndef PCORE_STEP_UNROLL
 #define PCORE_STEP_UNROLL 1
+#endif
+#ifndef PCORE_FRAG_NOHALF
+#define PCORE_FRAG_NOHALF 1
+#endif
+#ifndef PCORE_WIN_SPARSE
+#define PCORE_WIN_SPARSE 1
 #endif
 
 namespace pcore {
@@ -81,12 +87,11 @@
     return lo <= hi;
 }
 
+template <bool NOHALF = false>
 __device__ __forceinline__ bool fragment(float A0, float A1, float B0, float B1, float C0, float C1, float z0,
                                          float z1, float z2, float P0, float P1, int32_t& depth, bool z_ok = false) {
-    const float area = 0.5f * ((C0 - A0) * (B1 - A1) - (B0 - A0) * (C1 - A1));
-    const float base_inv = 1.0f / area;
-    const float beta = 0.5f * ((C0 - A0) * (P1 - A1) - (P0 - A0) * (C1 - A1)) * base_inv;
-    const float gamma = 0.5f * ((P0 - A0) * (B1 - A1) - (B0 - A0) * (P1 - A1)) * base_inv;
+    float beta, gamma;
+    frag_barycentrics<NOHALF && PCORE_FRAG_NOHALF>(A0, A1, B0, B1, C0, C1, P0, P1, beta, gamma);
     const float alpha = 1.0f - beta - gamma;
     float mn, mx;
     asm("v_min3_f32 %0, %1, %2, %3" : "=v"(mn) : "v"(alpha), "v"(beta), "v"(gamma));
@@ -163,15 +168,17 @@
 struct SampleWin {
     int x0, y0, nx, ny;
     int fastdiv;
+    int sparse;
 };
 
-template <bool IDPASS = false>
+template <bool IDPASS = false, bool NOHALF = false>
 __device__ __forceinline__ void raster_sample(const TriRec& r, int kx, int ky, int s, int H, const SampleWin& w,
                                               int32_t* zbuf, int32_t* cid = nullptr, uint32_t id = 0) {
     const float P0 = (float)(kx * s);
     const float P1 = (float)(H - 1 - ky * s);
     int32_t d;
-    const bool in = fragment(r.a0, r.a1, r.b0, r.b1, r.c0, r.c1, r.z0, r.z1, r.z2, P0, P1, d, w.fastdiv != 0);
+    const bool in = fragment<NOHALF>(r.a0, r.a1, r.b0, r.b1, r.c0, r.c1, r.z0, r.z1, r.z2, P0, P1, d,
+                                     w.fastdiv != 0);
     const int k = (int)__umul24((uint32_t)(ky - w.y0), (uint32_t)w.nx) + (kx - w.x0);
     if constexpr (IDPASS) {
         if (in && d == zbuf[k]) atomicMin(&cid[k], (int32_t)id);
@@ -296,6 +303,7 @@
                                              int32_t* cid, FProf& fp) {
     SampleWin sw = sw_in;
     if constexpr (FD >= 0) sw.fastdiv = FD;
+    constexpr bool kNoHalf = FD == 1 && !IDPASS;
     const int tid = threadIdx.x;
     const int wave = __builtin_amdgcn_readfirstlane(tid >> 6);
     const int lane = tid & 63;
@@ -306,6 +314,9 @@
     const float m10 = P[4], m11 = P[5], m12 = P[6], m13 = P[7];
     const float m20 = P[8], m21 = P[9], m22 = P[10], m23 = P[11];
     const int model = a.pose_model[pose];
+#if PCORE_WIN_SPARSE
+    const bool proj_sparse = sw.sparse != 0;
+#else
     bool proj_sparse = false;
     if (a.proj_sparse && model >= 0 && model < a.num_models) {
         const float4 lo = a.model_box[2 * model], hi = a.model_box[2 * model + 1];
@@ -315,6 +326,7 @@
         const float By = fabsf(m10) * ax + fabsf(m11) * ay + fabsf(m12) * az + fabsf(m13);
         proj_sparse = lo.w != 0.0f && Bx < 1.0e30f && By < 1.0e30f;
     }
+#endif
     __syncthreads();
 
     const float Wf = (float)W, Hf = (float)H;
@@ -360,7 +372,8 @@
 #ifdef PCORE_FLUSH_STATS
                     atomicAdd(&pcore_flush_stats[2], 1ull);
 #endif
-                    raster_sample<IDPASS>(r, (int)(rec.y & 0xffffu), (int)(rec.y >> 16), s, H, sw, sm.zbuf, cid, id);
+                    raster_sample<IDPASS, kNoHalf>(r, (int)(rec.y & 0xffffu), (int)(rec.y >> 16), s, H, sw, sm.zbuf,
+                                                   cid, id);
                 }
             }
         }
@@ -532,7 +545,7 @@
                         for (int q = lane; q < bnk; q += kWave) {
                             int iy = (int)(((float)q + 0.5f) * inv_nx), ix = q - iy * bnx;
                             if (ix < 0) { iy--; ix += bnx; } else if (ix >= bnx) { iy++; ix -= bnx; }
-                            raster_sample<IDPASS>(rb, bkx0 + ix, bky0 + iy, s, H, sw, sm.zbuf, cid, bid);
+                            raster_sample<IDPASS, kNoHalf>(rb, bkx0 + ix, bky0 + iy, s, H, sw, sm.zbuf, cid, bid);
                         }
                     } while (big);
                 }
@@ -591,8 +604,14 @@
 }
 
 __device__ SampleWin pose_window(const FusedArgs& a, int model, const float (&m)[12], int s) {
-    const SampleWin whole = {0, 0, a.ws, a.hs, 0};
     const float4 lo = a.model_box[2 * model], hi = a.model_box[2 * model + 1];
+    const float ax = fmaxf(fabsf(lo.x), fabsf(hi.x)), ay = fmaxf(fabsf(lo.y), fabsf(hi.y));
+    const float az = fmaxf(fabsf(lo.z), fabsf(hi.z));
+    const float Bx = fabsf(m[0]) * ax + fabsf(m[1]) * ay + fabsf(m[2]) * az + fabsf(m[3]);
+    const float By = fabsf(m[4]) * ax + fabsf(m[5]) * ay + fabsf(m[6]) * az + fabsf(m[7]);
+    const float Bz = fabsf(m[8]) * ax + fabsf(m[9]) * ay + fabsf(m[10]) * az + fabsf(m[11]);
+    const int sparse = (a.proj_sparse && lo.w != 0.0f && Bx < 1.0e30f && By < 1.0e30f) ? 1 : 0;
+    const SampleWin whole = {0, 0, a.ws, a.hs, 0, sparse};
     const int c = lane_id() & 7;
     const float x = (c & 1) ? hi.x : lo.x, y = (c & 2) ? hi.y : lo.y, z = (c & 4) ? hi.z : lo.z;
     const float Wf = (float)a.width, Hf = (float)a.height;
@@ -616,11 +635,6 @@
     auto uni = [](float v) { return __int_as_float(__builtin_amdgcn_readfirstlane(__float_as_int(v))); };
     lzmin = uni(lzmin); sx0 = uni(sx0); sx1 = uni(sx1); sy0 = uni(sy0); sy1 = uni(sy1);
     if ((__ballot(bad) & 0xffull) || lo.w == 0.0f) return whole;
-    const float ax = fmaxf(fabsf(lo.x), fabsf(hi.x)), ay = fmaxf(fabsf(lo.y), fabsf(hi.y));
-    const float az = fmaxf(fabsf(lo.z), fabsf(hi.z));
-    const float Bx = fabsf(m[0]) * ax + fabsf(m[1]) * ay + fabsf(m[2]) * az + fabsf(m[3]);
-    const float By = fabsf(m[4]) * ax + fabsf(m[5]) * ay + fabsf(m[6]) * az + fabsf(m[7]);
-    const float Bz = fabsf(m[8]) * ax + fabsf(m[9]) * ay + fabsf(m[10]) * az + fabsf(m[11]);
     if (!(lzmin > 0.05f * Bz)) return whole;
     const float eps = 5.9604645e-8f;
     const float Pbx = fabsf(a.p00) * Bx + fabsf(a.p01) * By + fabsf(a.p02) * Bz + fabsf(a.p03);
@@ -633,7 +647,7 @@
     const int X0 = max(0, (int)floorf((xlo - 1.0f) / sf)), X1 = min(a.ws - 1, (int)floorf(xhi / sf));
     const int Y0 = max(0, (int)floorf((Hf - 1.0f - yhi) / sf)), Y1 = min(a.hs - 1, (int)floorf((Hf - ylo) / sf));
     const bool fastdiv = lzmin - 1.0e-5f * Bz >= 1.0f && Bz < 0x1p40f && Pbx < 0x1p40f && Pby < 0x1p40f;
-    return SampleWin{X0, Y0, max(0, X1 - X0 + 1), max(0, Y1 - Y0 + 1), fastdiv ? 1 : 0};
+    return SampleWin{X0, Y0, max(0, X1 - X0 + 1), max(0, Y1 - Y0 + 1), fastdiv ? 1 : 0, sparse};
 }
 
 __device__ __forceinline__ int64_t select_key(float rc, float oc, int m, int num_models, int64_t gidx) {
@@ -814,7 +828,8 @@
         for (int r0 = 0; r0 < pw.ny; r0 += ch)
             for (int c0 = 0; c0 < pw.nx; c0 += cw) {
                 if (r0 > 0 || c0 > 0) __syncthreads();
-                chunk(SampleWin{pw.x0 + c0, pw.y0 + r0, min(cw, pw.nx - c0), min(ch, pw.ny - r0), pw.fastdiv});
+                chunk(SampleWin{pw.x0 + c0, pw.y0 + r0, min(cw, pw.nx - c0), min(ch, pw.ny - r0), pw.fastdiv,
+                                pw.sparse});
             }
     }
     __syncthreads();
@@ -892,7 +907,7 @@
     const FusedSmem sm = carve_smem(smem_raw, a.tcap, a.bitmap_words, COLOUR);
     if (threadIdx.x < kWave) {
         const int model = a.pose_model[pose];
-        SampleWin w = {0, 0, 0, 0, 0};
+        SampleWin w = {0, 0, 0, 0, 0, 0};
         if (model >= 0 && model < a.num_models) {
             float m[12];
             load_pose_rows(a.poses, pose, m);
@@ -904,12 +919,14 @@
             sm.counters[6] = w.nx;
             sm.counters[7] = w.ny;
             sm.counters[8] = w.fastdiv;
+            sm.counters[9] = w.sparse;
         }
     }
     __syncthreads();
     const SampleWin sw = {__builtin_amdgcn_readfirstlane(sm.counters[4]), __builtin_amdgcn_readfirstlane(sm.counters[5]),
                           __builtin_amdgcn_readfirstlane(sm.counters[6]), __builtin_amdgcn_readfirstlane(sm.counters[7]),
-                          __builtin_amdgcn_readfirstlane(sm.counters[8])};
+                          __builtin_amdgcn_readfirstlane(sm.counters[8]),
+                          __builtin_amdgcn_readfirstlane(sm.counters[9])};
     const int tn = sw.nx * sw.ny;
     if (threadIdx.x == 0) {
         const int par = a.fb_par;
@@ -980,7 +997,7 @@
     const int cap = a.tcap > 0 && a.tcap < nsamp ? a.tcap : nsamp;
     const FusedSmem sm = carve_smem(smem_raw, cap, 0);
     const int model = a.pose_model[pose];
-    SampleWin sw = {0, 0, 0, 0, 0};
+    SampleWin sw = {0, 0, 0, 0, 0, 0};
     if (model >= 0 && model < a.num_models) {
         float m[12];
         load_pose_rows(a.poses, pose, m);
@@ -1039,7 +1056,8 @@
         const int cw = min(sw.nx, cap), ch = max(1, cap / max(cw, 1));
         for (int r0 = 0; r0 < sw.ny; r0 += ch)
             for (int c0 = 0; c0 < sw.nx; c0 += cw)
-                chunk(SampleWin{sw.x0 + c0, sw.y0 + r0, min(cw, sw.nx - c0), min(ch, sw.ny - r0), sw.fastdiv});
+                chunk(SampleWin{sw.x0 + c0, sw.y0 + r0, min(cw, sw.nx - c0), min(ch, sw.ny - r0), sw.fastdiv,
+                                sw.sparse});
     }
     if (tid == 0) a.cloud_count[pose] = carry_s < a.cloud_cap ? carry_s : a.cloud_cap;
     if (a.cloud_cov) {
diff --git a/perception_amd/csrc/pcore_streams.h b/perception_amd/csrc/pcore_streams.h
--- a/perception_amd/csrc/pcore_streams.h
+++ b/perception_amd/csrc/pcore_streams.h
@@ -120,12 +120,69 @@
     return order;
 }
 
+inline std::vector<int> band_order(const std::vector<int>& tv, const std::vector<float>& vxyz, int axis, int bands) {
+    const int T = (int)tv.size() / 3, NV = (int)vxyz.size() / 3;
+    const int u = (axis + 1) % 3, v = (axis + 2) % 3;
+    double lo[3] = {0, 0, 0}, hi[3] = {0, 0, 0};
+    bool any = false;
+    for (int i = 0; i < NV; i++) {
+        const float* p = &vxyz[3 * i];
+        if (!(std::isfinite(p[0]) && std::isfinite(p[1]) && std::isfinite(p[2]))) continue;
+        for (int k = 0; k < 3; k++) {
+            lo[k] = any ? std::min(lo[k], (double)p[k]) : p[k];
+            hi[k] = any ? std::max(hi[k], (double)p[k]) : p[k];
+        }
+        any = true;
+    }
+    const double cu = 0.5 * (lo[u] + hi[u]), cv = 0.5 * (lo[v] + hi[v]);
+    const double h0 = lo[axis], hspan = hi[axis] - lo[axis];
+    const bool caps_along_u = hi[u] - lo[u] >= hi[v] - lo[v];
+    struct Key {
+        int bin;
+        double k;
+        int t;
+    };
+    std::vector<Key> key(T);
+    for (int t = 0; t < T; t++) {
+        const float* a = &vxyz[3 * tv[3 * t]];
+        const float* b = &vxyz[3 * tv[3 * t + 1]];
+        const float* c = &vxyz[3 * tv[3 * t + 2]];
+        const double e1[3] = {(double)b[0] - a[0], (double)b[1] - a[1], (double)b[2] - a[2]};
+        const double e2[3] = {(double)c[0] - a[0], (double)c[1] - a[1], (double)c[2] - a[2]};
+        const double n[3] = {e1[1] * e2[2] - e1[2] * e2[1], e1[2] * e2[0] - e1[0] * e2[2],
+                             e1[0] * e2[1] - e1[1] * e2[0]};
+        const double ctr[3] = {((double)a[0] + b[0] + c[0]) / 3.0, ((double)a[1] + b[1] + c[1]) / 3.0,
+                               ((double)a[2] + b[2] + c[2]) / 3.0};
+        const double nn = n[0] * n[0] + n[1] * n[1] + n[2] * n[2];
+        Key& q = key[t];
+        q.t = t;
+        if (!(std::isfinite(nn) && std::isfinite(ctr[0]) && std::isfinite(ctr[1]) && std::isfinite(ctr[2]))) {
+            q.bin = bands + 2;
+            q.k = 0.0;
+        } else if (2.0 * n[axis] * n[axis] > nn) {
+            q.bin = n[axis] < 0.0 ? 0 : bands + 1;
+            q.k = caps_along_u ? ctr[u] : ctr[v];
+        } else {
+            int bi = hspan > 0.0 ? (int)((ctr[axis] - h0) / hspan * bands) : 0;
+            q.bin = 1 + std::max(0, std::min(bands - 1, bi));
+            q.k = std::atan2(ctr[v] - cv, ctr[u] - cu);
+        }
+    }
+    std::stable_sort(key.begin(), key.end(),
+                     [](const Key& p, const Key& q) { return p.bin != q.bin ? p.bin < q.bin : p.k < q.k; });
+    std::vector<int> order(T);
+    for (int t = 0; t < T; t++) order[t] = key[t].t;
+    return order;
+}
+
+constexpr int kAhead = 192;
 constexpr int kNever = -(1 << 20);
 constexpr uint32_t kStepVertexPass = 1u << 30;
 constexpr uint32_t kSlotPadding = 1u << 31;
 
 inline void build_model_order(const std::vector<int>& tv, const std::vector<float>& vxyz, const std::vector<int>& order0,
-                              int tri_base, int num_streams, int vring, int ref_passes, Built& out, int chunks) {
+                              int tri_base, int num_streams, int vring, int ref_passes, Built& out, int chunks,
+                              int ahead = 0) {
     const int T = (int)tv.size() / 3;
     if (T == 0) return;
     const int num_verts = (int)vxyz.size() / 3;
@@ -143,7 +200,8 @@
     }
     std::vector<int> latest(num_verts, kNever), slot(num_verts, 0);
     std::vector<char> in_new(num_verts, 0);
-    std::vector<int> newv, batch;
+    std::vector<int> newv, batch, cand;
+    std::vector<char> taken(ahead > 0 ? T : 0, 0);
     for (int sidx = 0; sidx < S; sidx++) {
         const int b0 = sidx == 0 ? 0 : stream_end[sidx - 1], b1 = stream_end[sidx];
         I4 sd;
@@ -176,9 +234,34 @@
             return true;
         };
         while (true) {
-            while (i < b1 && usable_after(order[i], P)) {
-                batch.push_back(order[i++]);
-                if ((int)batch.size() == 64) emit();
+            if (ahead <= 0) {
+                while (i < b1 && usable_after(order[i], P)) {
+                    batch.push_back(order[i++]);
+                    if ((int)batch.size() == 64) emit();
+                }
+            } else {
+                cand.assign(batch.begin(), batch.end());
+                batch.clear();
+                int waiting = 0;
+                for (int j = i; j < b1 && waiting <= ahead; j++) {
+                    if (taken[j]) continue;
+                    if (usable_after(order[j], P)) {
+                        taken[j] = 1;
+                        cand.push_back(order[j]);
+                    } else {
+                        waiting++;
+                    }
+                }
+                while (i < b1 && taken[i]) i++;
+                std::stable_partition(cand.begin(), cand.end(), [&](int t) {
+                    for (int k = 0; k < 3; k++)
+                        if (latest[tv[3 * t + k]] <= P + 1 - ref_passes) return true;
+                    return false;
+                });
+                for (int t : cand) {
+                    batch.push_back(t);
+                    if ((int)batch.size() == 64) emit();
+                }
             }
             if (i >= b1) {
                 if (!batch.empty() || !attached) emit();
@@ -204,6 +287,7 @@
                 emit();
             }
             for (int j = i; j < b1; j++) {
+                if (ahead > 0 && taken[j]) continue;
                 int miss[3], nm = 0;
                 for (int k = 0; k < 3; k++) {
                     const int v = tv[3 * order[j] + k];
@@ -212,7 +296,10 @@
                     for (int q = 0; q < nm; q++) dup |= miss[q] == v;
                     if (!dup) miss[nm++] = v;
                 }
-                if ((int)newv.size() + nm > 64) break;
+                if ((int)newv.size() + nm > 64) {
+                    if (ahead <= 0 || (int)newv.size() >= 64 || j - i > 2 * ahead) break;
+                    continue;
+                }
                 for (int q = 0; q < nm; q++) {
                     in_new[miss[q]] = 1;
                     newv.push_back(miss[q]);
@@ -236,14 +323,30 @@
     }
 }
 
+#ifndef PCORE_STREAM_CANDIDATES
+#define PCORE_STREAM_CANDIDATES 1
+#endif
 inline void build_model(const std::vector<int>& tv, const std::vector<float>& vxyz, int tri_base, int num_streams,
                         int vring, int ref_passes, Built& out, int chunks = 4) {
     if (tv.empty()) return;
-    Built a, b;
-    build_model_order(tv, vxyz, locality_order(tv, (int)vxyz.size() / 3), tri_base, num_streams, vring, ref_passes, a,
-                      chunks);
-    build_model_order(tv, vxyz, sweep_order(tv, vxyz), tri_base, num_streams, vring, ref_passes, b, chunks);
-    const Built& w = (b.passes < a.passes || (b.passes == a.passes && b.steps < a.steps)) ? b : a;
+    const std::vector<int> grow = locality_order(tv, (int)vxyz.size() / 3), sweep = sweep_order(tv, vxyz);
+    Built w, b;
+    build_model_order(tv, vxyz, grow, tri_base, num_streams, vring, ref_passes, w, chunks);
+    build_model_order(tv, vxyz, sweep, tri_base, num_streams, vring, ref_passes, b, chunks);
+    if (b.passes < w.passes || (b.passes == w.passes && b.steps < w.steps)) std::swap(w, b);
+#if PCORE_STREAM_CANDIDATES
+    const long long base_passes = w.passes, base_steps = w.steps;
+    auto offer = [&](const std::vector<int>& order) {
+        Built c;
+        build_model_order(tv, vxyz, order, tri_base, num_streams, vring, ref_passes, c, chunks, kAhead);
+        if (c.passes <= base_passes && c.steps <= base_steps && 2 * c.passes + c.steps < 2 * w.passes + w.steps)
+            std::swap(w, c);
+    };
+    offer(grow);
+    offer(sweep);
+    for (int axis = 0; axis < 3; axis++)
+        for (int bands : {1, 2, 3, 4, 6, 8}) offer(band_order(tv, vxyz, axis, bands));
+#endif
     const int step0 = (int)(out.stris.size() / 64), pass0 = (int)(out.sverts.size() / 64);
     out.sverts.insert(out.sverts.end(), w.sverts.begin(), w.sverts.end());
     out.stris.insert(out.stris.end(), w.stris.begin(), w.stris.end());
```

New measurement: 37.18 million poses/s, median of 6. 3.5% higher.
